# gcorso/disco-diffdock

Measured on AMD Instinct MI355X. Metric: complexes/sec, 20-step 40-sample inference, higher is better.
Workload: dtype f32

## Files before the change

disco_diffdock_amd/csrc/ddk_capi.hip:

```cpp
#include <math.h>
#include <algorithm>
#include <cmath>
#include <string.h>

#include "model.h"
#include "k_conv_common.h"

using namespace ddk;

namespace ddk {


int fail(ddk_ctx* ctx, int code, const std::string& msg) {
  if (ctx) ctx->err = msg;
  return code;
}

int hip_fail(ddk_ctx* ctx, hipError_t e, const char* what) {
  return fail(ctx, DDK_ERR_HIP, std::string(what) + ": " + hipGetErrorString(e));
}

hipError_t ctx_malloc(ddk_ctx* ctx, void** p, size_t bytes) {
  *p = nullptr;
  if (ctx->alloc_limit > 0 && ctx->dev_bytes + (int64_t)bytes > ctx->alloc_limit) { ctx->alloc_refusals++; return hipErrorOutOfMemory; }
// ... 501 lines not shown
      float* b2 = b2x_all.data() + g * b2sz;
      for (int t = 0; t < L.n_tiles; ++t) {
        for (int s_ = 0; s_ < 36; ++s_)
          for (int lane = 0; lane < 64; ++lane) {
            const int row = rmx[(size_t)t * 32 + (lane & 31)], hh = lane >> 5;
            w2[(((size_t)t * 9 + s_ / 4) * 64 + lane) * 4 + (s_ & 3)] = row >= 0 ? W2->data[(size_t)row * ne + hid_of(s_, hh)] * rsx[(size_t)t * 32 + (lane & 31)] : 0.f;
          }
        for (int hh = 0; hh < 2; ++hh)
          for (int r = 0; r < 16; ++r) {
            const int row = rmx[(size_t)t * 32 + d_row(r, hh)];
            b2[((size_t)t * 2 + hh) * 16 + r] = row >= 0 ? B2->data[row] * rsx[(size_t)t * 32 + d_row(r, hh)] : 0.f;
          }
      }
    }
    if ((rc = pack_x3(ctx, L, NG, w1all, w2x_all, b2x_all))) return rc;
  }
  if (!ctx->host_only) {
    std::vector<float> w2rec((size_t)NG * L.n_tiles * W2_TILE_FLOATS);
    for (int g = 0; g < NG; ++g)
      for (int t = 0; t < L.n_tiles; ++t) {
        float* rec = w2rec.data() + ((size_t)g * L.n_tiles + t) * W2_TILE_FLOATS;
        memcpy(rec, w2all.data() + g * w2sz + (size_t)t * 2304, 2304 * sizeof(float));
        memcpy(rec + 2304, b2all.data() + g * b2sz + (size_t)t * 32, 32 * sizeof(float));
        memcpy(rec + 2336, &tiles[t], 2 * sizeof(int32_t));
      }
    float* d1 = dev_upload(ctx, w1all);
    float* db1 = dev_upload(ctx, b1all);
    float* d2 = dev_upload(ctx, w2rec);
    if (mode == 0) { L.wn = dev_upload(ctx, L.h_wn); L.bnp = dev_upload(ctx, L.h_bnp); if (!L.wn || !L.bnp) return fail(ctx, DDK_ERR_NOMEM, "device allocation failed while packing conv weights"); }
    L.bn_mean = dev_upload(ctx, L.h_bn_mean);
    L.bn_scale = dev_upload(ctx, L.h_bn_scale);
    L.bn_bias = dev_upload(ctx, L.h_bn_bias);
    if (!d1 || !db1 || !d2 || !L.bn_mean || !L.bn_scale || !L.bn_bias)
      return fail(ctx, DDK_ERR_NOMEM, "device allocation failed while packing conv weights");
    L.w1p[0] = d1; L.b1p[0] = db1; L.w2r[0] = d2;
    for (int g = 1; g < 4; ++g) {
      L.w1p[g] = d1 + g * w1sz;
      L.b1p[g] = db1 + g * b1sz;
      L.w2r[g] = d2 + (size_t)g * L.n_tiles * W2_TILE_FLOATS;
    }
  }
  return DDK_OK;
}

int build_head_layer(ddk_ctx* ctx, int mode, ConvLayerDev& L) {
  std::vector<int> rowmap;
  std::vector<float> rowscale;
  std::vector<TileDesc> tiles;
  int rc = build_layout(ctx, mode, 3, L, rowmap, rowscale, tiles);
  if (rc) return rc;
  L.n_groups = 1;
  const std::string pre = mode == 2 ? "tor_bond_conv.fc" : "final_conv.fc";
  const int kin = mode == 2 ? NE : 2 * NS;
  const HostTensor* W1 = find_w(ctx, pre + ".0.weight", {kin, kin});
  const HostTensor* B1 = find_w(ctx, pre + ".0.bias", {kin});
  const HostTensor* W2 = find_w(ctx, pre + ".4.weight", {L.W, kin});
  const HostTensor* B2 = find_w(ctx, pre + ".4.bias", {L.W});
  if (!W1 || !B1 || !W2 || !B2) return DDK_ERR_INVALID;
  L.has_weights = true;
  std::vector<float> w1(3 * 9 * 64 * 4, 0.f), b1(3 * 2 * 16, 0.f), w2((size_t)L.n_tiles * 9 * 64 * 4, 0.f), b2((size_t)L.n_tiles * 32, 0.f);
  for (int T = 0; T < 3; ++T) {
    for (int s = 0; s < 36; ++s)
      for (int lane = 0; lane < 64; ++lane) {
        const int hidden = 32 * T + (lane & 31), k = kin_of(s, lane >> 5);
        w1[(((size_t)T * 9 + s / 4) * 64 + lane) * 4 + (s & 3)] = (hidden < kin && k < kin) ? W1->data[(size_t)hidden * kin + k] : 0.f;
      }
    for (int hh = 0; hh < 2; ++hh)
      for (int r = 0; r < 16; ++r) {
        const int hidden = 32 * T + d_row(r, hh);
        b1[(T * 2 + hh) * 16 + r] = hidden < kin ? B1->data[hidden] : 0.f;
      }
  }
  for (int t = 0; t < L.n_tiles; ++t) {
    for (int s = 0; s < 36; ++s)
      for (int lane = 0; lane < 64; ++lane) {
        const int row = rowmap[(size_t)t * 32 + (lane & 31)], hd = hid_of(s, lane >> 5);
        w2[(((size_t)t * 9 + s / 4) * 64 + lane) * 4 + (s & 3)] =
            (row >= 0 && hd < kin) ? W2->data[(size_t)row * kin + hd] * rowscale[(size_t)t * 32 + (lane & 31)] : 0.f;
      }
    for (int hh = 0; hh < 2; ++hh)
      for (int r = 0; r < 16; ++r) {
        const int row = rowmap[(size_t)t * 32 + d_row(r, hh)];
        b2[((size_t)t * 2 + hh) * 16 + r] = row >= 0 ? B2->data[row] * rowscale[(size_t)t * 32 + d_row(r, hh)] : 0.f;
      }
  }
  L.h_w1p.assign(1, w1); L.h_b1p.assign(1, b1); L.h_w2p.assign(1, w2); L.h_b2p.assign(1, b2);
  L.h_bn_mean.assign(XW, 0.f); L.h_bn_scale.assign(XW, 1.f); L.h_bn_bias.assign(XW, 0.f);
  if (ctx->cfg.conv_kernel != 1 && (rc = pack_x3(ctx, L, 1, w1, w2, b2))) return rc;
  if (ctx->host_only) return DDK_OK;
  std::vector<float> w2rec((size_t)L.n_tiles * W2_TILE_FLOATS);
  for (int t = 0; t < L.n_tiles; ++t) {
    float* rec = w2rec.data() + (size_t)t * W2_TILE_FLOATS;
    memcpy(rec, w2.data() + (size_t)t * 2304, 2304 * sizeof(float));
    memcpy(rec + 2304, b2.data() + (size_t)t * 32, 32 * sizeof(float));
    memcpy(rec + 2336, &tiles[t], 2 * sizeof(int32_t));
  }
  L.w1p[0] = dev_upload(ctx, w1); L.b1p[0] = dev_upload(ctx, b1); L.w2r[0] = dev_upload(ctx, w2rec);
  if (!L.w1p[0] || !L.b1p[0] || !L.w2r[0]) return fail(ctx, DDK_ERR_NOMEM, "device allocation failed while packing the head weights");
  return DDK_OK;
}

int model_finalize(ddk_ctx* ctx);
int conf_model_finalize(ddk_ctx* ctx);
void conf_model_destroy(ddk_ctx* ctx);
void model_destroy(ddk_ctx* ctx);

}

extern "C" {

const char* ddk_version(void) { return "ddk 0.8 (gfx950)"; }

int ddk_create(const ddk_config* cfg, ddk_ctx** out) {
  if (!cfg || !out) return DDK_ERR_INVALID;
  ddk_ctx* ctx = new ddk_ctx();
  ctx->cfg = *cfg;
  *out = ctx;
  if (cfg->ns != NS || cfg->nv != NV)
    return fail(ctx, DDK_ERR_INVALID, "only ns=24, nv=6 (DiffDock-S / DisCo-DiffDock-S) is compiled in");
  if (cfg->num_conv_layers < 4 || cfg->num_conv_layers > 16)
    return fail(ctx, DDK_ERR_INVALID, "num_conv_layers must be in [4,16] (the heads and the confidence predictor assume the full 0e+1o+1e+0o irreps)");
  if (cfg->confidence_mode && cfg->all_atoms)
    return fail(ctx, DDK_ERR_INVALID, "confidence_mode selects the COARSE-GRAINED score model's confidence head; the all-atom confidence model is all_atoms = 1 alone (include/ddk.h)");
  if (cfg->sigma_embed_dim != 32 || cfg->distance_embed_dim != 32 || cfg->cross_distance_embed_dim != 32)
    return fail(ctx, DDK_ERR_INVALID, "only 32-wide sigma / distance embeddings are compiled in");
  if (cfg->deterministic && cfg->all_atoms)
    return fail(ctx, DDK_ERR_INVALID, "deterministic scatter is implemented for the score model (not with all_atoms)");
#ifdef DDK_VARIANT_CONV_Y
  if (cfg->conv_kernel < 0 || cfg->conv_kernel > 3) return fail(ctx, DDK_ERR_INVALID, "conv_kernel must be 0, 1, 2 (variant build) or 3");
#else
  if (cfg->conv_kernel < 0 || cfg->conv_kernel > 3 || cfg->conv_kernel == 2)
    return fail(ctx, DDK_ERR_INVALID, "conv_kernel must be 0 (two f16 limbs per operand, three products), 1 (fp32 MFMA) or 3 (three f16 limbs, six products); 2 (round 5's software-pipelined form) lives under tools/variants/ and is not part of libddk.so");
#endif
  if (cfg->device < 0) {
    ctx->host_only = true;
    return DDK_OK;
  }
  hipError_t e = hipSetDevice(cfg->device);
  if (e != hipSuccess) return hip_fail(ctx, e, "hipSetDevice");
  hipDeviceProp_t prop;
  e = hipGetDeviceProperties(&prop, cfg->device);
  if (e != hipSuccess) return hip_fail(ctx, e, "hipGetDeviceProperties");
  ctx->n_cu = prop.multiProcessorCount;
  e = hipStreamCreateWithFlags(&ctx->up_stream, hipStreamNonBlocking);
  if (e != hipSuccess) return hip_fail(ctx, e, "hipStreamCreate (upload stream)");
  e = hipStreamCreateWithFlags(&ctx->head_stream, hipStreamNonBlocking);
  if (e == hipSuccess) e = hipEventCreateWithFlags(&ctx->ev_fork, hipEventDisableTiming);
  if (e == hipSuccess) e = hipEventCreateWithFlags(&ctx->ev_join, hipEventDisableTiming);
  if (e != hipSuccess) return hip_fail(ctx, e, "hipStreamCreate (head stream)");
  e = conv_prepare_device();
  if (e != hipSuccess) return hip_fail(ctx, e, "hipFuncSetAttribute(dynamic LDS)");
  e = graph_prepare_device(&ctx->max_rec);
  if (e != hipSuccess) return hip_fail(ctx, e, "hipFuncSetAttribute(dynamic LDS, graph kernels)");
  ctx->ws.tile_info = (int32_t*)dev_alloc(ctx, 64 * sizeof(int32_t));
  if (!ctx->ws.tile_info) return fail(ctx, DDK_ERR_NOMEM, "hipMalloc failed");
  return DDK_OK;
}

void ddk_destroy(ddk_ctx* ctx) {
  if (!ctx) return;
  if (!ctx->host_only) {
    hipSetDevice(ctx->cfg.device);
    model_destroy(ctx);
    conf_model_destroy(ctx);
    for (auto& r : ctx->prof_recs) { hipEventDestroy(r.a); hipEventDestroy(r.b); }
    if (ctx->prof_edges) hipHostFree(ctx->prof_edges);
    for (auto& c : ctx->chunk_pool) { if (c.free_after) hipEventDestroy(c.free_after); ctx_free(ctx, c.p); }
    for (auto& b : ctx->stage_pool) { if (b.done) hipEventDestroy(b.done); hipHostFree(b.p); }
    if (ctx->up_stream) hipStreamDestroy(ctx->up_stream);
    if (ctx->head_stream) hipStreamDestroy(ctx->head_stream);
    if (ctx->ev_fork) hipEventDestroy(ctx->ev_fork);
    if (ctx->ev_join) hipEventDestroy(ctx->ev_join);
    for (void* p : ctx->dev_allocs) ctx_free(ctx, p);
    if (ctx->ws.xpad) ctx_free(ctx, ctx->ws.xpad);
    if (ctx->ws.sum) ctx_free(ctx, ctx->ws.sum);
    if (ctx->ws.deg) ctx_free(ctx, ctx->ws.deg);
  }
  delete ctx;
}

const char* ddk_last_error(ddk_ctx* ctx) { return ctx ? ctx->err.c_str() : "null context"; }

int ddk_load_weights(ddk_ctx* ctx, const char* name, const float* host_ptr, const int64_t* shape, int32_t ndim) {
  if (!ctx || !name || (!host_ptr && ndim > 0 && shape[0] != 0)) return fail(ctx, DDK_ERR_INVALID, "ddk_load_weights: null argument");
  const std::string n(name);
  if (n.find(".tp.") != std::string::npos) return DDK_OK;
  HostTensor t;
  int64_t numel = 1;
  for (int i = 0; i < ndim; ++i) {
    t.shape.push_back(shape[i]);
    numel *= shape[i];
  }
  t.data.assign(host_ptr, host_ptr + numel);
  ctx->weights[n] = std::move(t);
  ctx->finalized = false;
  return DDK_OK;
}

int ddk_finalize_weights(ddk_ctx* ctx) {
  if (!ctx) return DDK_ERR_INVALID;
  if (!ctx->host_only) hipSetDevice(ctx->cfg.device);
  ctx->conv.clear();
  ctx->conv.resize(ctx->cfg.num_conv_layers);
  for (int l = 0; l < ctx->cfg.num_conv_layers; ++l) {
    int rc = build_conv_layer(ctx, ctx->cfg.all_atoms ? 1 : 0, l, ctx->conv[l]);
    if (rc != DDK_OK) return rc;
  }
  ctx->head[0] = ConvLayerDev(); ctx->head[1] = ConvLayerDev();
  if (!ctx->cfg.all_atoms && ctx->weights.find("final_conv.fc.0.weight") != ctx->weights.end()) {
    int rch = build_head_layer(ctx, 3, ctx->head[1]);
    if (rch == DDK_OK && !ctx->cfg.no_torsion) rch = build_head_layer(ctx, 2, ctx->head[0]);
    if (rch != DDK_OK) return rch;
  }
  int rc = ctx->cfg.all_atoms ? conf_model_finalize(ctx) : model_finalize(ctx);
  if (rc != DDK_OK) return rc;
  ctx->finalized = true;
  return DDK_OK;
}

int ddk_set_score_norm_tables(ddk_ctx* ctx, const double* so3, int32_t n_so3, const double* torus, int32_t n_torus) {
  if (!ctx || !so3 || !torus) return fail(ctx, DDK_ERR_INVALID, "null table");
  if (n_so3 != 1000 || n_torus != 5001) return fail(ctx, DDK_ERR_INVALID, "expected 1000 so3 and 5001 torus entries");
  ctx->so3_table.assign(so3, so3 + n_so3);
  ctx->torus_table.assign(torus, torus + n_torus);
  return DDK_OK;
}

static int check_launchable(ddk_ctx* ctx, int32_t layer) {
  if (!ctx) return DDK_ERR_INVALID;
  if (ctx->host_only) return fail(ctx, DDK_ERR_STATE, "host-only context (device < 0) cannot launch kernels");
  if (!ctx->finalized) return fail(ctx, DDK_ERR_STATE, "weights not finalised");
  if (layer < 0 || layer >= (int)ctx->conv.size()) return fail(ctx, DDK_ERR_INVALID, "layer out of range");
  return DDK_OK;
}

int ddk_tp_forward(ddk_ctx* ctx, int32_t layer, const float* x_dst, const float* sh, const float* w, int64_t E,
                   float* out, void* stream) {
  int rc = check_launchable(ctx, layer);
  if (rc) return rc;
  hipError_t e = launch_tp_forward(ctx->conv[layer], x_dst, sh, w, E, out, (hipStream_t)stream);
  if (e == hipErrorInvalidValue)
    return fail(ctx, DDK_ERR_INVALID, "ddk_tp_forward: the layer's irreps are not one of the four conv-layer shapes of this model family (24x0e [+ 6x1o [+ 6x1e [+ 24x0o]]] -> the next entry)");
  if (e != hipSuccess) return hip_fail(ctx, e, "tp_forward launch");
  return DDK_OK;
}

int ddk_conv_forward(ddk_ctx* ctx, int32_t layer, const float* x, int64_t N, const int32_t* edge_src,
                     const int32_t* edge_dst, const int64_t* go, const float* edge_attr, const float* sh, float* out,
                     void* stream) {
  const bool aa = ctx && ctx->cfg.all_atoms;
  const int conv_k = aa ? layer % 9 : 0;
  if (aa) layer /= 9;
  int rc = check_launchable(ctx, layer);
  if (rc) return rc;
  if (!go || go[0] != 0 || go[1] < go[0] || go[2] < go[1] || go[3] < go[2] || go[4] < go[3])
    return fail(ctx, DDK_ERR_INVALID, "group_offsets must be a non-decreasing prefix starting at 0");
  if (go[4] >= (int64_t)1 << 31 || N * XW >= (int64_t)1 << 40) return fail(ctx, DDK_ERR_INVALID, "graph too large");
  hipStream_t s = (hipStream_t)stream;
  const ConvLayerDev& L = ctx->conv[layer];
  if (!L.has_weights) return fail(ctx, DDK_ERR_STATE, "conv layer has no weights loaded");
  Workspace& ws = ctx->ws;
  if ((rc = ensure(ctx, (void**)&ws.xpad, &ws.xpad_cap, (size_t)N * XW * 4))) return rc;
  if ((rc = ensure(ctx, (void**)&ws.sum, &ws.sum_cap, (size_t)N * XW * 4))) return rc;
  if ((rc = ensure(ctx, (void**)&ws.deg, &ws.deg_cap, (size_t)N * 4))) return rc;
  const int64_t E = go[4];
  CK(launch_pad_rows(x, N, L.din, ws.xpad, s), "pad_rows");
  CK(hipMemsetAsync(ws.sum, 0, (size_t)N * XW * 4, s), "memset sum");
  CK(hipMemsetAsync(ws.deg, 0, (size_t)N * 4, s), "memset deg");
  if (E > 0) {
    CK(launch_conv_setup(ws.tile_info, go, s), "conv_setup");
    CK(launch_count_deg(edge_src, E, ws.deg, s), "count_deg");
    ConvLaunch a;
    a.x = ws.xpad; a.src = edge_src; a.dst = edge_dst; a.edge_attr = edge_attr; a.sh = sh; a.sum = ws.sum;
    a.tile_info = ws.tile_info; a.counter = ws.tile_info + 10; a.gather = 0;
    if (aa) {
      CK(launch_conv_one_group(ws.tile_info + 32, 9, conv_k, E, s), "group table");
      a.mode = 1; a.n_groups = 9; a.n_active = 9; a.n_slots = 1; a.slots = 0; a.gbeg = ws.tile_info + 32; a.gend = ws.tile_info + 41;
    }
    CK(launch_conv_fused(L, a, ctx->n_cu, s), "conv_fused");
  }
  if (aa) {
    CK(launch_node_finalize(ws.sum, ws.deg, nullptr, L.bn_mean + conv_k * XW, L.bn_scale + conv_k * XW, L.bn_bias + conv_k * XW, N, L.dout, L.dout, out, s),
       "node_finalize");
    return DDK_OK;
  }
  if (E > 0)
    CK(launch_node_finalize(ws.sum, ws.deg, ws.xpad, L.bn_mean, L.bn_scale, L.bn_bias, N, L.dout, L.dout, out, s), "node_finalize");
  else
    CK(launch_node_finalize(ws.sum, ws.deg, ws.xpad, nullptr, nullptr, nullptr, N, 0, L.dout, out, s), "node_finalize");
  return DDK_OK;
}

int64_t ddk_debug_export(ddk_ctx* ctx, const char* what, void* buf, int64_t cap_words) {
  if (!ctx || !what) return DDK_ERR_INVALID;
  int l = 0, g = 0;
  char item[32] = {0};
  const void* src = nullptr;
  int64_t n = 0;
  if (sscanf(what, "conv.%d.%31[a-z0-9_].%d", &l, item, &g) >= 2) {
    const bool head = (l == 100 || l == 101) && ctx->head[l - 100].n_tiles > 0;
    if (!head && (l < 0 || l >= (int)ctx->conv.size())) return fail(ctx, DDK_ERR_INVALID, "bad export index");
    ConvLayerDev& L = head ? ctx->head[l - 100] : ctx->conv[l];
    if (g < 0 || g >= L.n_groups) return fail(ctx, DDK_ERR_INVALID, "bad export index");
    const std::string it(item);
    if (it == "w1p") { src = L.h_w1p[g].data(); n = L.h_w1p[g].size(); }
    else if (it == "b1p") { src = L.h_b1p[g].data(); n = L.h_b1p[g].size(); }
// ... 31 lines not shown
```

disco_diffdock_amd/csrc/k_graph.hip:

```cpp
#include <stdlib.h>
#include "model.h"
#include "k_node.h"

namespace ddk {


__device__ __forceinline__ bool cross_within(const float* lp, const float* rp, float c) {
#pragma clang fp contract(off)
  const float dx = rp[0] / c - lp[0] / c, dy = rp[1] / c - lp[1] / c, dz = rp[2] / c - lp[2] / c;
  return dx * dx + dy * dy + dz * dz < 1.0f;
}

__device__ __forceinline__ bool cross_within4(const float4 a, float rx, float ry, float rz) {
#pragma clang fp contract(off)
  const float dx = rx - a.x, dy = ry - a.y, dz = rz - a.z;
  return dx * dx + dy * dy + dz * dz < 1.0f;
}

__device__ __forceinline__ float dist2(const float* a, const float* b) {
#pragma clang fp contract(off)
  const float dx = a[0] - b[0], dy = a[1] - b[1], dz = a[2] - b[2];
  return dx * dx + dy * dy + dz * dz;
}

constexpr int GT = 1024;

__device__ void build_lig_adj(const float* lp, int n_lig, float r2, unsigned (*adj)[MAX_LIG / 32]) {
  const int lane = threadIdx.x & 63, wave = threadIdx.x >> 6, nw = blockDim.x >> 6;
  for (int i = wave; i < n_lig; i += nw) {
    int cnt = 0;
    if (lane < MAX_LIG / 32) adj[i][lane] = 0u;
    for (int j0 = 0; j0 < n_lig; j0 += 64) {
      const int j = j0 + lane;
      const bool in = j < n_lig && dist2(lp + 3 * i, lp + 3 * j) < r2;
      const unsigned long long m = __ballot(in);
      const bool keep = in && cnt + __popcll(m & ((1ull << lane) - 1ull)) < LIG_CAP && j != i;
      const unsigned long long kept = __ballot(keep);
      if (lane == 0) { adj[i][j0 >> 5] = (unsigned)kept; adj[i][(j0 >> 5) + 1] = (unsigned)(kept >> 32); }
      cnt += __popcll(m);
    }
  }
}

__device__ void block_exclusive_scan(int* a, int n, int* tmp) {
  const int tid = threadIdx.x, lane = tid & 63, wave = tid >> 6;
  const int nt = blockDim.x;
  const int per = (n + nt - 1) / nt;
  const int beg = min(tid * per, n), end = min(beg + per, n);
  int s = 0;
  for (int k = beg; k < end; ++k) s += a[k];
  int v = s;
#pragma unroll
  for (int d = 1; d < 64; d *= 2) {
    const int t = __shfl_up(v, d, 64);
    if (lane >= d) v += t;
  }
  if (lane == 63) tmp[wave] = v;
  __syncthreads();
  int base = v - s;
  for (int w = 0; w < wave; ++w) base += tmp[w];
  for (int k = beg; k < end; ++k) { const int t = a[k]; a[k] = base; base += t; }
  __syncthreads();
}

__device__ void propagate_levels(uint8_t* lvl, const GraphArgs& G) {
  constexpr int UC = 8;
  if (G.E_rr <= GT * UC) {
    unsigned e[UC];
#pragma unroll
    for (int u = 0; u < UC; ++u) {
      const int k = threadIdx.x + GT * u;
      e[u] = k < G.E_rr ? (unsigned)G.rr_src[k] | ((unsigned)G.rr_dst[k] << 16) : 0xffffffffu;
    }
    for (int pass = 0; pass < 2; ++pass) {
#pragma unroll
      for (int u = 0; u < UC; ++u) {
        const int r = (int)(e[u] & 0xffffu), d = (int)(e[u] >> 16);
        if (e[u] != 0xffffffffu && lvl[r] == pass && lvl[d] == 3) lvl[d] = (uint8_t)(pass + 1);
      }
      __syncthreads();
    }
    return;
  }
  constexpr int U = 8;
  for (int pass = 0; pass < 2; ++pass) {
    for (int k0 = threadIdx.x; k0 < G.E_rr; k0 += GT * U) {
      int r[U], d[U];
#pragma unroll
      for (int u = 0; u < U; ++u) {
        const int k = k0 + GT * u;
        r[u] = k < G.E_rr ? G.rr_src[k] : -1;
        d[u] = k < G.E_rr ? G.rr_dst[k] : 0;
      }
#pragma unroll
      for (int u = 0; u < U; ++u)
        if (r[u] >= 0 && lvl[r[u]] == pass && lvl[d[u]] == 3) lvl[d[u]] = (uint8_t)(pass + 1);
    }
    __syncthreads();
  }
}

__device__ void level_scan(const uint8_t* lvl, const int32_t* outdeg, int n, int* pre, int (*tmp)[4], int* tot) {
  const int tid = threadIdx.x, lane = tid & 63, wave = tid >> 6;
  const int nt = blockDim.x, nw = nt >> 6;
  const int per = (n + nt - 1) / nt;
  const int beg = min(tid * per, n), end = min(beg + per, n);
  int s0 = 0, s1 = 0, s2 = 0, s3 = 0;
  for (int k = beg; k < end; ++k) {
    const int l = lvl[k], od = outdeg[k];
    s0 += l == 0 ? od : 0; s1 += l == 1 ? od : 0; s2 += l == 2 ? od : 0; s3 += l == 3 ? od : 0;
  }
  int v0 = s0, v1 = s1, v2 = s2, v3 = s3;
#pragma unroll
  for (int d = 1; d < 64; d *= 2) {
    const int t0 = __shfl_up(v0, d, 64), t1 = __shfl_up(v1, d, 64), t2 = __shfl_up(v2, d, 64), t3 = __shfl_up(v3, d, 64);
    if (lane >= d) { v0 += t0; v1 += t1; v2 += t2; v3 += t3; }
  }
  if (lane == 63) { tmp[wave][0] = v0; tmp[wave][1] = v1; tmp[wave][2] = v2; tmp[wave][3] = v3; }
  __syncthreads();
  if (pre != nullptr) {
    int b0 = v0 - s0, b1 = v1 - s1, b2 = v2 - s2, b3 = v3 - s3;
    for (int w = 0; w < wave; ++w) { b0 += tmp[w][0]; b1 += tmp[w][1]; b2 += tmp[w][2]; b3 += tmp[w][3]; }
    for (int k = beg; k < end; ++k) {
      const int l = lvl[k], od = outdeg[k];
      pre[k] = l == 0 ? b0 : (l == 1 ? b1 : (l == 2 ? b2 : b3));
      b0 += l == 0 ? od : 0; b1 += l == 1 ? od : 0; b2 += l == 2 ? od : 0; b3 += l == 3 ? od : 0;
    }
  }
  if (tid < 4) { int t_ = 0; for (int w = 0; w < nw; ++w) t_ += tmp[w][tid]; tot[tid] = t_; }
  __syncthreads();
}

__global__ __launch_bounds__(GT) void graph_count_kernel(GraphArgs G) {
  extern __shared__ float smem[];
  float* lp = smem;
  float* rp = lp + MAX_LIG * 3;
  uint8_t* lvl = reinterpret_cast<uint8_t*>(rp + 3 * G.n_rec + G.n_rec);
  __shared__ unsigned adj[MAX_LIG][MAX_LIG / 32];
  __shared__ float4 lps[MAX_LIG];
  __shared__ int s_cnt[2], lvl_tmp[GT / 64][4], lvl_tot[4];
  const int b = blockIdx.x, tid = threadIdx.x;
  for (int i = tid; i < G.n_lig * 3; i += GT) {
    const float v = G.lig_pos[(size_t)b * G.n_lig * 3 + i];
    lp[i] = v;
    reinterpret_cast<float*>(lps)[4 * (i / 3) + i % 3] = v / G.cross_cutoff;
  }
  for (int i = tid; i < G.n_rec * 3; i += GT) rp[i] = G.rec_pos[i] / G.cross_cutoff;
  if (tid < 2) s_cnt[tid] = 0;
  __syncthreads();
  build_lig_adj(lp, G.n_lig, G.lig_r2, adj);
  __syncthreads();
  int c_ll = 0, c_lr = 0;
  for (int i = tid; i < G.n_lig; i += GT)
    for (int w = 0; w < MAX_LIG / 32; ++w) c_ll += __popc(adj[i][w]);
  for (int j = tid; j < G.n_rec; j += GT) {
    const float rx = rp[3 * j], ry = rp[3 * j + 1], rz = rp[3 * j + 2];
    int cnt = 0;
#pragma unroll 4
    for (int i = 0; i < G.n_lig; ++i) cnt += cross_within4(lps[i], rx, ry, rz) ? 1 : 0;
    c_lr += cnt;
    lvl[j] = (G.prune && cnt == 0) ? 3 : 0;
  }
#pragma unroll
  for (int d = 32; d > 0; d >>= 1) { c_ll += __shfl_down(c_ll, d, 64); c_lr += __shfl_down(c_lr, d, 64); }
  if ((tid & 63) == 0) { atomicAdd(&s_cnt[0], c_ll); atomicAdd(&s_cnt[1], c_lr); }
  __syncthreads();
  if (G.prune) propagate_levels(lvl, G);
  level_scan(lvl, G.rr_outdeg, G.n_rec, nullptr, lvl_tmp, lvl_tot);
  if (tid < 2) G.counts[CNT_STRIDE * b + tid] = s_cnt[tid];
  if (tid < 3) G.counts[CNT_STRIDE * b + 2 + tid] = lvl_tot[tid];
  for (int j = tid; j < G.n_rec; j += GT) G.levels[(size_t)b * G.n_rec + j] = lvl[j];
}

__device__ __forceinline__ void sample_prefix(const GraphArgs& G, int b, int* ex, int* tot) {
  const int lane = threadIdx.x & 63;
#pragma unroll
  for (int k = 0; k < 5; ++k) { tot[k] = 0; ex[k] = 0; }
  for (int b0 = 0; b0 < G.B; b0 += 64) {
    const int bb = b0 + lane;
    int v[5], inc[5];
#pragma unroll
    for (int k = 0; k < 5; ++k) v[k] = bb < G.B ? G.counts[CNT_STRIDE * bb + k] + (k == 0 ? G.M : 0) : 0;
#pragma unroll
    for (int k = 0; k < 5; ++k) {
      int x = v[k];
#pragma unroll
      for (int d = 1; d < 64; d *= 2) { const int t = __shfl_up(x, d, 64); if (lane >= d) x += t; }
      inc[k] = x;
    }
    if (b >= b0 && b < b0 + 64) {
#pragma unroll
      for (int k = 0; k < 5; ++k) ex[k] = tot[k] + __shfl(inc[k] - v[k], b - b0, 64);
    }
#pragma unroll
    for (int k = 0; k < 5; ++k) tot[k] += __shfl(inc[k], 63, 64);
  }
  ex[5] = b * G.E_rr - (ex[2] + ex[3] + ex[4]);
}

__device__ void write_group_tables(const GraphArgs& G, const int* tot) {
  const int ll = tot[0], lr = tot[1], ra = tot[2], rb = tot[3], rc = tot[4];
  int go[5];
  go[0] = 0; go[1] = ll; go[2] = ll + lr; go[3] = go[2] + G.B * G.E_rr; go[4] = go[3] + lr;
  const int seg[4] = {go[2], go[2] + ra, go[2] + ra + rb, go[2] + ra + rb + rc};
  const int n_shared = G.shared_rr ? G.E_rr : 0;
  int bs = 0;
  G.info[I_FB] = 0;
  for (int g = 0; g < 5; ++g) {
    bs += (g == 3 && G.cross_mirror) ? 0 : ((g < 4 ? go[g + 1] - go[g] : n_shared) + 255) / 256;
    G.info[I_FB + 1 + g] = bs;
  }
  for (int g = 0; g < 5; ++g) G.info[I_GO + g] = go[g];
  for (int k = 0; k < 8; ++k) G.info[I_CNT + k] = 0;
  for (int l = 0; l < 4; ++l) G.info[I_SEG + l] = seg[l];
  G.info[I_E] = go[4];
  G.info[I_OVF] = ((int64_t)go[4] + n_shared > G.edge_cap) ? 1 : 0;
  G.info[I_SHARED] = G.shared_rr ? go[4] : -1;
  G.info[I_HEAD] = 0; G.info[I_HEAD + 1] = G.B * G.n_lig; G.info[I_HEAD + 2] = G.B * G.n_lig; G.info[I_HEAD + 3] = G.B * G.n_lig;
  G.info[I_HEAD + 4] = 0; G.info[I_HEAD + 5] = 0;
  G.info[I_EXEC] = go[4];
  G.info[I_EXEC + 1] = go[2];
  G.info[I_EXEC + 7] = lr;
  for (int k = 0; k < N_TAB; ++k) {
    int32_t* tb = G.info + I_TAB + 8 * k;
    int tot = 0;
    for (int g = 0; g < 4; ++g) { tb[g] = go[g]; tb[4 + g] = go[g + 1]; }
    if (k == TAB_A) tb[4 + 2] = seg[1];
    if (k == TAB_B) tb[4 + 2] = seg[2];
    if (k == TAB_C) tb[4 + 2] = seg[3];
    if (k == TAB_SHARED) { tb[2] = go[4]; tb[4 + 2] = go[4] + n_shared; }
    for (int g = 0; g < 4; ++g) tot += tb[4 + g] - tb[g];
    if (k == TAB_SHARED && G.patch_off >= 0 && G.shared_rr) tot += G.info[I_PATCH];
    G.info[I_EXEC + 2 + k] = tot;
  }
  if (G.patch_off >= 0 && G.shared_rr) {
    const int np = G.info[I_PATCH];
    const int32_t* ts = G.info + I_TAB + 8 * TAB_SHARED;
    for (int g = 0; g < 4; ++g) { G.info[I_TABX + g] = ts[g]; G.info[I_TABX + 5 + g] = ts[4 + g]; }
    G.info[I_TABX + 4] = (int)G.patch_off; G.info[I_TABX + 9] = (int)G.patch_off + np;
    G.info[I_FBX] = bs + (np + 255) / 256;
  } else {
    G.info[I_FBX] = bs;
  }
}

__device__ __forceinline__ bool latent_nonzero(const float* lat, int64_t row, int ld) {
  bool nz = false;
  for (int j = 0; j < ld; ++j) nz |= lat[row * ld + j] != 0.0f;
  return nz;
}

__global__ __launch_bounds__(256) void disco_patch_count_kernel(PatchArgs A) {
  extern __shared__ unsigned char mk[];
  __shared__ int red[256];
  const int b = blockIdx.x, tid = threadIdx.x;
  for (int j = tid; j < A.n_rec; j += 256)
    mk[j] = b > 0 && (latent_nonzero(A.rec_latent, (int64_t)b * A.n_rec + j, A.latent_dim) || latent_nonzero(A.rec_latent, j, A.latent_dim));
  __syncthreads();
  int cnt = 0;
  for (int i = tid; i < A.n_rec; i += 256) {
    bool a = mk[i];
    const int k0 = A.rr_start[i], k1 = k0 + A.rr_outdeg[i];
    for (int k = k0; k < k1 && !a; ++k) a = mk[A.rr_dst[k]];
    A.rr_mask[(size_t)b * A.n_rec + i] = a;
    if (a) cnt += k1 - k0;
  }
  red[tid] = cnt;
  __syncthreads();
  for (int d = 128; d > 0; d >>= 1) { if (tid < d) red[tid] += red[tid + d]; __syncthreads(); }
  if (tid == 0) A.patch_cnt[b] = red[0];
}

__global__ void disco_patch_scan_kernel(PatchArgs A) {
  if (threadIdx.x != 0 || blockIdx.x != 0) return;
  int tot = 0;
  for (int b = 0; b < A.B; ++b) { const int c = A.patch_cnt[b]; A.patch_cnt[b] = tot; tot += c; }
  A.patch_cnt[A.B] = tot;
  A.info[I_PATCH] = tot;
}

__global__ __launch_bounds__(256) void disco_patch_fill_kernel(PatchArgs A) {
  extern __shared__ int pre_[];
  __shared__ int scan_tmp[16];
  const int b = blockIdx.x, tid = threadIdx.x;
  for (int i = tid; i < A.n_rec; i += 256) pre_[i] = A.rr_mask[(size_t)b * A.n_rec + i] ? A.rr_outdeg[i] : 0;
  __syncthreads();
  block_exclusive_scan(pre_, A.n_rec, scan_tmp);
  const int rec0 = A.B * A.n_lig + b * A.n_rec;
  const int64_t base = A.patch_off + A.patch_cnt[b];
  for (int i = tid; i < A.n_rec; i += 256) {
    if (!A.rr_mask[(size_t)b * A.n_rec + i]) continue;
    const int k0 = A.rr_start[i], n = A.rr_outdeg[i];
    for (int q = 0; q < n; ++q) {
      const int64_t pos = base + pre_[i] + q;
      A.e_src[pos] = rec0 + i; A.e_dst[pos] = rec0 + A.rr_dst[k0 + q]; A.e_aux[pos] = k0 + q;
    }
  }
}

hipError_t launch_disco_patch(const PatchArgs& a, hipStream_t s) {
  hipLaunchKernelGGL(disco_patch_count_kernel, dim3(a.B), dim3(256), (size_t)a.n_rec, s, a);
  hipLaunchKernelGGL(disco_patch_scan_kernel, dim3(1), dim3(64), 0, s, a);
  hipLaunchKernelGGL(disco_patch_fill_kernel, dim3(a.B), dim3(256), (size_t)a.n_rec * sizeof(int), s, a);
  return hipGetLastError();
}

constexpr int FILL_SLICES = 4;

__global__ __launch_bounds__(GT) void graph_fill_kernel(GraphArgs G) {
  extern __shared__ float smem[];
  float* lp = smem;
  float* rp = lp + MAX_LIG * 3;
  int* c_rl = reinterpret_cast<int*>(rp + 3 * G.n_rec);
  uint8_t* lvl = reinterpret_cast<uint8_t*>(c_rl + G.n_rec);
  unsigned long long* cmask = reinterpret_cast<unsigned long long*>(lvl + ((G.n_rec + 15) & ~15));
  const int LW = (G.n_lig + 63) >> 6;
  __shared__ unsigned adj[MAX_LIG][MAX_LIG / 32];
  __shared__ int bdeg[MAX_LIG], odeg[MAX_LIG], c_lr[MAX_LIG], ll_pre[MAX_LIG], lr_pre[MAX_LIG], scan_tmp[GT / 64], lvl_tmp[GT / 64][4], lvl_tot[4];
  constexpr int BOND_LDS = 1024;
  __shared__ short2 bond_sd[BOND_LDS];
  const int b = blockIdx.x, slice = blockIdx.y, tid = threadIdx.x, lane = tid & 63, wave = tid >> 6;
  const int n_lig = G.n_lig, n_rec = G.n_rec;
  int ex[6], tot[5];
  sample_prefix(G, b, ex, tot);
// ... 207 lines not shown
    float gs[DE];
#pragma unroll
    for (int k = 0; k < DE; ++k) {
      const float t = d - M.offset[k];
      gs[k] = expf(M.coeff * (t * t));
    }
#pragma unroll
    for (int o = 0; o < NS; ++o) h[o] = sigb[o];
#pragma unroll
    for (int k = 0; k < DE; ++k) {
#pragma unroll
      for (int o = 0; o < NS; ++o) h[o] = fmaf(M.w1d_t[k * NS + o], gs[k], h[o]);
    }
    if (g == 0 && aux >= 0) {
      const float4 ba = *reinterpret_cast<const float4*>(A.bond_attr + 4 * (size_t)aux);
#pragma unroll
      for (int o = 0; o < NS; ++o)
        h[o] += M.w1b[o * 4] * ba.x + M.w1b[o * 4 + 1] * ba.y + M.w1b[o * 4 + 2] * ba.z + M.w1b[o * 4 + 3] * ba.w;
    }
  }
  if (A.latent_dim > 0 && (g == 0 || g == 2)) {
    const float* lat = g == 0 ? A.lig_latent : A.rec_latent;
    const int off = g == 0 ? 0 : A.n_lig_total;
    const int ld = A.latent_dim;
    for (int j = 0; j < ld; ++j) {
      const float ls = lat[(size_t)(sn - off) * ld + j], ldv = lat[(size_t)(dn - off) * ld + j];
#pragma unroll
      for (int o = 0; o < NS; ++o) h[o] += M.w1l[o * 2 * ld + j] * ls + M.w1l[o * 2 * ld + ld + j] * ldv;
    }
  }
#pragma unroll
  for (int o = 0; o < NS; ++o) h[o] = fmaxf(h[o], 0.0f);
  float* out = A.e_emb + (size_t)e * NS;
  float* out2 = (g == 1 && A.cross_mirror) ? A.e_emb + (size_t)aux * NS : nullptr;
  const float uncw = (A.latent_dim > 0 && M.unc != nullptr) ? A.unconditional : 0.0f;
  float y[NS];
#pragma unroll
  for (int o = 0; o < NS; ++o) y[o] = M.b2[o];
#pragma unroll
  for (int k = 0; k < NS; ++k) {
#pragma unroll
    for (int o = 0; o < NS; ++o) y[o] = fmaf(M.w2_t[k * NS + o], h[k], y[o]);
  }
  if (uncw != 0.0f) {
#pragma unroll
    for (int o = 0; o < NS; ++o) y[o] += uncw * M.unc[o];
  }
#pragma unroll
  for (int o4 = 0; o4 < NS / 4; ++o4) {
    const float4 rv = make_float4(y[4 * o4], y[4 * o4 + 1], y[4 * o4 + 2], y[4 * o4 + 3]);
    *reinterpret_cast<float4*>(out + 4 * o4) = rv;
    if (out2) *reinterpret_cast<float4*>(out2 + 4 * o4) = rv;
  }
  *reinterpret_cast<float4*>(A.e_sh + 4 * (size_t)e) = shv;
  if (out2) *reinterpret_cast<float4*>(A.e_sh + 4 * (size_t)aux) = shv;
}

__global__ __launch_bounds__(256) void edge_features_kernel(EdgeFeatArgs A) { edge_features_body(A, (int)blockIdx.x, (int)threadIdx.x); }

__global__ __launch_bounds__(PRE_W) void edge_features_node_kernel(EdgeFeatArgs A, NodePreArgs P, NodeEmbedArgs E, int node_blocks) {
  if ((int)blockIdx.x < node_blocks) { node_finalize_pre_body<2>(P, E, (int)blockIdx.x, node_blocks); return; }
  if (threadIdx.x < 256) edge_features_body(A, (int)blockIdx.x - node_blocks, (int)threadIdx.x);
}

__global__ void node_embed_kernel(NodeEmbedArgs A) {
  const int64_t i = (int64_t)blockIdx.x * blockDim.x + threadIdx.x;
  const int64_t n_l = (int64_t)A.B * A.n_lig, n = n_l + (int64_t)A.B * A.n_rec;
  if (i >= n * XW) return;
  const int64_t node = i / XW;
  const int c = (int)(i % XW);
  float v = 0.0f;
  if (c < NS) {
    const bool lig = node < n_l;
    if (lig) v = A.lig_static[(node % A.n_lig) * NS + c] + A.sp.lig_node_sig[c];
    else v = A.rec_static[((node - n_l) % A.n_rec) * NS + c] + A.sp.rec_node_sig[c];
    if (A.latent_dim > 0) {
      const float* lat = lig ? A.lig_latent + node * A.latent_dim : A.rec_latent + (node - n_l) * A.latent_dim;
      const float* w = (lig ? A.lig_w_lat : A.rec_w_lat) + c * A.latent_dim;
      for (int j = 0; j < A.latent_dim; ++j) v += w[j] * lat[j];
      const float* u = lig ? A.lig_unc : A.rec_unc;
      if (u != nullptr) v += A.unconditional * u[c];
    }
  }
  A.x[i] = v;
}

constexpr int RNS_SLICES = 10;
__global__ __launch_bounds__(RNS_SLICES * NS) void rec_node_static_kernel(RecStaticArgs A) {
  __shared__ double part[RNS_SLICES][NS];
  const int o = threadIdx.x % NS, sl = threadIdx.x / NS, j = blockIdx.x;
  const float* xr = A.rec_x + (size_t)j * A.feat_dim;
  double a = 0.0;
  if (sl == 0) {
    const float* emb = A.rec_table + (size_t)(int)xr[0] * NS;
    a = A.b[o];
    for (int k = 0; k < NS; ++k) a += (double)A.w_emb[o * NS + k] * emb[k];
  }
  const int per = (A.lm + RNS_SLICES - 1) / RNS_SLICES, k0 = sl * per, k1 = min(A.lm, k0 + per);
  for (int k = k0; k < k1; ++k) a += (double)A.w_lm_t[(size_t)k * NS + o] * (double)xr[1 + k];
  part[sl][o] = a;
  __syncthreads();
  if (sl == 0) {
#pragma unroll
    for (int q = 1; q < RNS_SLICES; ++q) a += part[q][o];
    A.out[(size_t)j * NS + o] = (float)a;
  }
}

__global__ __launch_bounds__(256) void rec_edge_static_kernel(const int32_t* rr_src, const int32_t* rr_dst, const float* rec_pos, int E, EdgeMlpDev m,
                                                              float* pre1) {
  const int gid = blockIdx.x * blockDim.x + threadIdx.x;
  const int k = gid / (NS / 4), o4 = gid % (NS / 4);
  if (k >= E) return;
  const int a = rr_src[k], b = rr_dst[k];
  const float vx = rec_pos[3 * b] - rec_pos[3 * a], vy = rec_pos[3 * b + 1] - rec_pos[3 * a + 1], vz = rec_pos[3 * b + 2] - rec_pos[3 * a + 2];
  const float dist = sqrtf(vx * vx + vy * vy + vz * vz);
  float gs[DE];
#pragma unroll
  for (int q = 0; q < DE; ++q) { const float t = dist - m.offset[q]; gs[q] = expf(m.coeff * (t * t)); }
  float r[4];
#pragma unroll
  for (int i = 0; i < 4; ++i) {
    const int o = 4 * o4 + i;
    float a2 = 0.0f;
#pragma unroll
    for (int q = 0; q < DE; ++q) a2 += m.w1d[o * DE + q] * gs[q];
    r[i] = a2;
  }
  *reinterpret_cast<float4*>(pre1 + (size_t)k * NS + 4 * o4) = make_float4(r[0], r[1], r[2], r[3]);
}

__global__ void zero_fill_kernel(float4* p, int64_t n4, float* tail, int n_tail) {
  const int64_t i = (int64_t)blockIdx.x * blockDim.x + threadIdx.x;
  if (i < n4) p[i] = make_float4(0.f, 0.f, 0.f, 0.f);
  if (i < n_tail) tail[i] = 0.0f;
}
hipError_t launch_zero_fill(void* p, size_t bytes, hipStream_t s) {
  if (bytes == 0) return hipSuccess;
  if ((reinterpret_cast<uintptr_t>(p) & 15) || (bytes & 3)) return hipMemsetAsync(p, 0, bytes, s);
  const int64_t n4 = (int64_t)(bytes / 16);
  const int n_tail = (int)((bytes % 16) / 4);
  hipLaunchKernelGGL(zero_fill_kernel, dim3((unsigned)((n4 + 255) / 256 + 1)), dim3(256), 0, s, reinterpret_cast<float4*>(p), n4,
                     reinterpret_cast<float*>(p) + 4 * n4, n_tail);
  return hipGetLastError();
}

hipError_t launch_complex_static(const RecStaticArgs& R, const int32_t* rr_src, const int32_t* rr_dst, const float* rec_pos, int E, const EdgeMlpDev& m,
                                 float* pre1, hipStream_t s) {
  if (R.n_rec > 0) hipLaunchKernelGGL(rec_node_static_kernel, dim3(R.n_rec), dim3(RNS_SLICES * NS), 0, s, R);
  if (E > 0) hipLaunchKernelGGL(rec_edge_static_kernel, dim3((E * (NS / 4) + 255) / 256), dim3(256), 0, s, rr_src, rr_dst, rec_pos, E, m, pre1);
  return hipGetLastError();
}

static inline size_t graph_lds_bytes(int n_rec) {
  return (size_t)(MAX_LIG * 3 + n_rec * 3) * 4 + (size_t)n_rec * 4 + (((size_t)n_rec + 15) & ~(size_t)15);
}

static size_t g_graph_dyn[64] = {};
static inline size_t graph_lds_bytes_mirror(int n_rec, int n_lig) { return graph_lds_bytes(n_rec) + (size_t)n_rec * ((n_lig + 63) / 64) * 8; }
int graph_cross_mirror_fits(int n_lig, int n_rec) {
  static const bool off = getenv("DDK_NO_CROSS_MIRROR") != nullptr;
  if (off) return 0;
  int dev = 0;
  if (hipGetDevice(&dev) != hipSuccess || dev < 0 || dev >= 64) return 0;
  return g_graph_dyn[dev] > 0 && graph_lds_bytes_mirror(n_rec, n_lig) <= g_graph_dyn[dev];
}

hipError_t graph_prepare_device(int* max_rec) {
  hipFuncAttributes a1, a2;
  hipError_t e = hipFuncGetAttributes(&a1, reinterpret_cast<const void*>(&graph_count_kernel));
  if (e == hipSuccess) e = hipFuncGetAttributes(&a2, reinterpret_cast<const void*>(&graph_fill_kernel));
  if (e != hipSuccess) return e;
  const size_t st = a1.sharedSizeBytes > a2.sharedSizeBytes ? a1.sharedSizeBytes : a2.sharedSizeBytes;
  const size_t dyn = 160 * 1024 - st;
  e = hipFuncSetAttribute(reinterpret_cast<const void*>(&graph_count_kernel), hipFuncAttributeMaxDynamicSharedMemorySize, (int)(160 * 1024 - a1.sharedSizeBytes));
  if (e == hipSuccess) e = hipFuncSetAttribute(reinterpret_cast<const void*>(&graph_fill_kernel), hipFuncAttributeMaxDynamicSharedMemorySize, (int)(160 * 1024 - a2.sharedSizeBytes));
  if (e != hipSuccess) return e;
  int n = MAX_REC;
  while (n > 1 && graph_lds_bytes(n) > dyn) --n;
  *max_rec = n;
  int dev = 0;
  if (hipGetDevice(&dev) == hipSuccess && dev >= 0 && dev < 64) g_graph_dyn[dev] = 160 * 1024 - a2.sharedSizeBytes;
  return hipSuccess;
}

hipError_t launch_graph(const GraphArgs& G, int64_t edge_cap, hipStream_t s) {
  const size_t lds = graph_lds_bytes(G.n_rec);
  GraphArgs Gc = G;
  Gc.edge_cap = edge_cap;
  hipLaunchKernelGGL(graph_count_kernel, dim3(G.B), dim3(GT), lds, s, Gc);
  hipLaunchKernelGGL(graph_fill_kernel, dim3(G.B, FILL_SLICES), dim3(GT), G.cross_mirror ? graph_lds_bytes_mirror(G.n_rec, G.n_lig) : lds, s, Gc);
  return hipGetLastError();
}

__global__ __launch_bounds__(GT) void det_ranges_kernel(GraphArgs G, int kind, int len_uniform, int32_t* out, int nr) {
  extern __shared__ int nb_s[];
  __shared__ int scan_tmp[GT / 64];
  const int tid = threadIdx.x, lane = tid & 63, wave = tid >> 6;
  int32_t* beg_o = out + nr + 1;
  int32_t* end_o = beg_o + nr;
  int32_t* grp_o = end_o + nr;
  auto put = [&](int r, int beg, int end, int g) {
    if (lane == 0) { beg_o[r] = beg; end_o[r] = end; grp_o[r] = g; nb_s[r] = (end - beg + 255) / 256; }
  };
  if (kind == 6) {
    for (int r = tid; r < nr; r += GT) { beg_o[r] = r * len_uniform; end_o[r] = (r + 1) * len_uniform; grp_o[r] = 0; nb_s[r] = (len_uniform + 255) / 256; }
  } else {
    const int nseg = kind == 5 ? 0 : kind;
    for (int b = wave; b < G.B; b += GT / 64) {
      int ex[6], tot[5];
      sample_prefix(G, b, ex, tot);
      const int g1 = tot[0], g2 = tot[0] + tot[1], g3 = g2 + G.B * G.E_rr;
      const int cnt0 = G.counts[CNT_STRIDE * b] + G.M, cnt1 = G.counts[CNT_STRIDE * b + 1];
      const int ca = G.counts[CNT_STRIDE * b + 2], cb = G.counts[CNT_STRIDE * b + 3], cc = G.counts[CNT_STRIDE * b + 4];
      put(b, ex[0], ex[0] + cnt0, 0);
      put(G.B + b, g1 + ex[1], g1 + ex[1] + cnt1, 1);
      if (kind == 0) continue;
      int r = 2 * G.B;
      const int segbeg[4] = {g2 + ex[2], g2 + tot[2] + ex[3], g2 + tot[2] + tot[3] + ex[4], g2 + tot[2] + tot[3] + tot[4] + ex[5]};
      const int seglen[4] = {ca, cb, cc, G.E_rr - ca - cb - cc};
      for (int l = 0; l < nseg; ++l) { put(r + b, segbeg[l], segbeg[l] + seglen[l], 2); r += G.B; }
      if (kind == 5) {
        const int g4 = g3 + tot[1];
        if (b == 0) put(r, g4, g4 + G.E_rr, 2);
        r += 1;
      }
      put(r + b, g3 + ex[1], g3 + ex[1] + cnt1, 3);
    }
  }
  __syncthreads();
  block_exclusive_scan(nb_s, nr, scan_tmp);
  for (int r = tid; r < nr; r += GT) out[r] = nb_s[r];
  if (tid == 0) out[nr] = nb_s[nr - 1] + (end_o[nr - 1] - beg_o[nr - 1] + 255) / 256;
}

int det_ranges_count(int kind, int B) { return kind == 0 ? 2 * B : (kind == 5 ? 3 * B + 1 : (kind == 6 ? B : (3 + kind) * B)); }

hipError_t launch_det_ranges(const GraphArgs& G, int kind, int len_uniform, int32_t* out, hipStream_t s) {
  const int nr = det_ranges_count(kind, G.B);
  hipLaunchKernelGGL(det_ranges_kernel, dim3(1), dim3(GT), (size_t)(nr + 1) * sizeof(int), s, G, kind, len_uniform, out, nr);
  return hipGetLastError();
}

hipError_t launch_edge_features(const EdgeFeatArgs& A, int64_t edge_cap, hipStream_t s) {
  const unsigned blocks = (unsigned)((edge_cap + 255) / 256 + 5);
  hipLaunchKernelGGL(edge_features_kernel, dim3(blocks), dim3(256), 0, s, A);
  return hipGetLastError();
}

hipError_t launch_edge_features_node(const EdgeFeatArgs& A, int64_t edge_cap, const NodePreArgs& P, const NodeEmbedArgs& E, hipStream_t s) {
  const unsigned blocks = (unsigned)((edge_cap + 255) / 256 + 5);
  const int nb = node_pre_tiles(P);
  hipLaunchKernelGGL(edge_features_node_kernel, dim3(blocks + nb), dim3(PRE_W), 0, s, A, P, E, nb);
  return hipGetLastError();
}

hipError_t launch_node_embed(const NodeEmbedArgs& a, hipStream_t s) {
  const int64_t tot = (int64_t)a.B * (a.n_lig + a.n_rec) * XW;
  hipLaunchKernelGGL(node_embed_kernel, dim3((unsigned)((tot + 255) / 256)), dim3(256), 0, s, a);
  return hipGetLastError();
}

}
```

disco_diffdock_amd/csrc/k_heads.hip:

```cpp
#include "model.h"

namespace ddk {

constexpr int EPB = 32;
__device__ __forceinline__ void edge_embed8(const EdgeMlpDev& m, const float* b1, float d, float (*act)[DE + 1], int el, int p, float* e3) {
#pragma unroll
  for (int q = 0; q < 4; ++q) {
    const float t = d - m.offset[4 * p + q];
    act[el][4 * p + q] = expf(m.coeff * (t * t));
  }
  __syncthreads();
  float h3[3];
#pragma unroll
  for (int q = 0; q < 3; ++q) {
    const int o = 3 * p + q;
    float a = b1[o];
#pragma unroll
    for (int k = 0; k < DE; ++k) a += m.w1d[o * DE + k] * act[el][k];
    h3[q] = fmaxf(a, 0.0f);
  }
  __syncthreads();
#pragma unroll
  for (int q = 0; q < 3; ++q) act[el][3 * p + q] = h3[q];
  __syncthreads();
#pragma unroll
  for (int q = 0; q < 3; ++q) {
    const int o = 3 * p + q;
    float a = m.b2[o];
#pragma unroll
    for (int k = 0; k < NS; ++k) a += m.w2[o * NS + k] * act[el][k];
    e3[q] = a;
  }
  __syncthreads();
}

__global__ __launch_bounds__(256) void heads_pre_kernel(HeadArgs A, int n_tor_blocks) {
  __shared__ float lp[MAX_LIG * 3];
  __shared__ float act[EPB][DE + 1];
  __shared__ int nb[BOND_CAP];
  __shared__ int s_cnt, s_base;
  __shared__ float ctr[3];
  const int tid = threadIdx.x, n = A.n_lig;
  const int el = tid >> 3, p = tid & 7;
  const bool tor = (int)blockIdx.x < n_tor_blocks;
  const int b = tor ? blockIdx.x / A.R : blockIdx.x - n_tor_blocks;
  for (int i = tid; i < n * 3; i += 256) lp[i] = A.lig_pos[(size_t)b * n * 3 + i];
  __syncthreads();
  if (!tor) {
    if (tid < 3) {
      float s = 0.0f;
      for (int i = 0; i < n; ++i) s += lp[3 * i + tid];
      ctr[tid] = s / (float)n;
    }
    __syncthreads();
    for (int a0 = 0; a0 < n; a0 += EPB) {
      const int i = a0 + el;
      const bool live = i < n;
      const int ii = live ? i : n - 1;
      const float vx = lp[3 * ii] - ctr[0], vy = lp[3 * ii + 1] - ctr[1], vz = lp[3 * ii + 2] - ctr[2];
      const float d = sqrtf(vx * vx + vy * vy + vz * vz);
      float e3[3];
      edge_embed8(A.md.center_edge, A.sp.center_edge_sigb, d, act, el, p, e3);
      if (live) {
        const int e = b * n + i;
        float* at = A.h_attr + (size_t)e * NE;
        const float* xr = A.x + ((size_t)b * n + i) * XW;
#pragma unroll
        for (int q = 0; q < 3; ++q) {
          at[3 * p + q] = e3[q];
          at[NS + 3 * p + q] = xr[3 * p + q];
          at[2 * NS + 3 * p + q] = 0.0f;
        }
        if (p == 0) {
          const float inv = 1.7320508075688772f / fmaxf(d, 1e-12f);
          *reinterpret_cast<float4*>(A.h_sh + (size_t)e * 4) = make_float4(1.0f, vx * inv, vy * inv, vz * inv);
          A.h_src[e] = b;
          A.h_dst[e] = b * n + i;
        }
      }
    }
    return;
  }
  const int r = blockIdx.x - b * A.R;
  const int u = A.rot_u[r], v = A.rot_v[r];
  const float cx = (lp[3 * u] + lp[3 * v]) * 0.5f, cy = (lp[3 * u + 1] + lp[3 * v + 1]) * 0.5f, cz = (lp[3 * u + 2] + lp[3 * v + 2]) * 0.5f;
  if (tid < 64) {
    int cnt = 0;
    for (int k0 = 0; k0 < n; k0 += 64) {
      const int k = k0 + tid;
      bool in = false;
      if (k < n) {
        const float dx = lp[3 * k] - cx, dy = lp[3 * k + 1] - cy, dz = lp[3 * k + 2] - cz;
        in = dx * dx + dy * dy + dz * dz < A.lig_r2;
      }
      const unsigned long long mask = __ballot(in);
      const int rank = cnt + __popcll(mask & ((1ull << tid) - 1ull));
      if (in && rank < BOND_CAP) nb[rank] = k;
      cnt += __popcll(mask);
    }
    if (tid == 0) {
      s_cnt = cnt < BOND_CAP ? cnt : BOND_CAP;
      if (A.deterministic) {
        s_base = A.B * n + (int)blockIdx.x * BOND_CAP;
        if (blockIdx.x == 0) A.h_info[3] = A.B * n + n_tor_blocks * BOND_CAP;
      } else {
        s_base = atomicAdd(A.h_info + 3, s_cnt);
      }
      A.h_deg[blockIdx.x] = s_cnt;
    }
  }
  __syncthreads();
  const int ne = s_cnt;
  const bool live = el < ne;
  const int k = ne > 0 ? nb[live ? el : 0] : u;
  const float vx = lp[3 * k] - cx, vy = lp[3 * k + 1] - cy, vz = lp[3 * k + 2] - cz;
  const float d = sqrtf(vx * vx + vy * vy + vz * vz);
  float e3[3];
  edge_embed8(A.md.final_edge, A.md.final_edge_b1, d, act, el, p, e3);
  const int e = s_base + el;
  float* at = A.h_attr + (size_t)e * NE;
  if (!live) {
    if (A.deterministic) {
#pragma unroll
      for (int q = 0; q < 9; ++q) at[9 * p + q] = 0.0f;
      if (p == 0) {
        *reinterpret_cast<float4*>(A.h_sh + (size_t)e * 4) = make_float4(0.f, 0.f, 0.f, 0.f);
        A.h_src[e] = A.B + n_tor_blocks;
        A.h_dst[e] = b * n + u;
      }
    }
    return;
  }
  const float* xk = A.x + ((size_t)b * n + k) * XW;
  const float* xu = A.x + ((size_t)b * n + u) * XW;
  const float* xv = A.x + ((size_t)b * n + v) * XW;
#pragma unroll
  for (int q = 0; q < 3; ++q) {
    const int o = 3 * p + q;
    at[o] = e3[q];
    at[NS + o] = xk[o];
    at[2 * NS + o] = xu[o] + xv[o];
  }
  if (p != 0) return;
  const float inv = 1.7320508075688772f / fmaxf(d, 1e-12f);
  const float s1[3] = {vx * inv, vy * inv, vz * inv};
  float bx = lp[3 * v] - lp[3 * u], by = lp[3 * v + 1] - lp[3 * u + 1], bz = lp[3 * v + 2] - lp[3 * u + 2];
  const float bn = fmaxf(sqrtf(bx * bx + by * by + bz * bz), 1e-12f);
  bx /= bn; by /= bn; bz /= bn;
  const float s3 = 1.7320508075688772f, s5 = 2.2360679774997897f;
  const float y0 = s5 * s3 * bx * bz, y1 = s5 * s3 * bx * by, y2 = s5 * (by * by - 0.5f * (bx * bx + bz * bz)),
              y3 = s5 * s3 * by * bz, y4 = s5 * (s3 * 0.5f) * (bz * bz - bx * bx);
  const float ca = 0.31622776601683794f, cb = 0.18257418583505536f;
  const float T0 = s3 * (-cb * s1[0] * y2 - ca * s1[0] * y4 + ca * s1[1] * y1 + ca * s1[2] * y0);
  const float T1 = s3 * (ca * s1[0] * y1 + 2.0f * cb * s1[1] * y2 + ca * s1[2] * y3);
  const float T2 = s3 * (ca * s1[0] * y0 + ca * s1[1] * y3 - cb * s1[2] * y2 + ca * s1[2] * y4);
  *reinterpret_cast<float4*>(A.h_sh + (size_t)e * 4) = make_float4(1.0f, T0, T1, T2);
  A.h_src[e] = A.B + (int)blockIdx.x;
  A.h_dst[e] = b * n + k;
}

__global__ __launch_bounds__(64) void heads_post_kernel(HeadArgs A, int n_tor_blocks) {
  __shared__ float v48[2 * NS], hid[NS], g12[12];
  const int tid = threadIdx.x;
  if (A.prof_out != nullptr && blockIdx.x == gridDim.x - 1 && tid < PROF_INTS) A.prof_out[tid] = A.exec_info[tid];
  if ((int)blockIdx.x < n_tor_blocks) {
    float* row = A.h_sum + (size_t)(A.B + blockIdx.x) * XW;
    const int ne = A.h_deg[blockIdx.x];
    if (tid < 2 * NS) {
      const float s = row[tid] / (float)(ne > 1 ? ne : 1);
      row[tid] = 0.0f;
      v48[tid] = (s - A.md.tb_bn_mean[tid]) * A.md.tb_bn_scale[tid] + A.md.tb_bn_bias[tid];
    }
    __syncthreads();
    if (tid < NS) {
      float a = 0.0f;
      for (int j = 0; j < 2 * NS; ++j) a += A.md.tf_w0[tid * 2 * NS + j] * v48[j];
      hid[tid] = A.md.tf_w3[tid] * tanhf(a);
    }
    __syncthreads();
    if (tid == 0) {
      float o = 0.0f;
      for (int j = 0; j < NS; ++j) o += hid[j];
      if (A.scale_by_sigma) o *= A.sp.torus_norm_sqrt;
      A.tor_out[blockIdx.x] = o;
    }
    return;
  }
  const int b = blockIdx.x - n_tor_blocks;
  float* row = A.h_sum + (size_t)b * XW;
  if (tid < 12) {
    g12[tid] = (row[tid] / (float)A.n_lig) * A.md.fc_bn_scale[tid / 3];
    row[tid] = 0.0f;
  }
  __syncthreads();
  if (tid < 2) {
    const int o = 3 * tid;
    const float px = g12[o] + g12[6 + o], py = g12[o + 1] + g12[7 + o], pz = g12[o + 2] + g12[8 + o];
    const float nrm = sqrtf(px * px + py * py + pz * pz);
    const float* w0n = tid == 0 ? A.md.tr_w0n : A.md.rot_w0n;
    const float* w3 = tid == 0 ? A.md.tr_w3 : A.md.rot_w3;
    const float* sb = tid == 0 ? A.sp.tr_sigb : A.sp.rot_sigb;
    float s = tid == 0 ? A.md.tr_b3 : A.md.rot_b3;
    for (int k = 0; k < NS; ++k) s += w3[k] * fmaxf(w0n[k] * nrm + sb[k], 0.0f);
    float f = s / nrm;
    if (A.scale_by_sigma) f = tid == 0 ? f / A.sp.tr_sigma : f * A.sp.so3_norm;
    float* out = (tid == 0 ? A.tr_out : A.rot_out) + 3 * (size_t)b;
    out[0] = px * f; out[1] = py * f; out[2] = pz * f;
  }
}

hipError_t launch_heads_pre(const HeadArgs& A, bool torsion, hipStream_t s) {
  const int n_tor = (torsion && A.R > 0) ? A.B * A.R : 0;
  hipLaunchKernelGGL(heads_pre_kernel, dim3(n_tor + A.B), dim3(256), 0, s, A, n_tor);
  return hipGetLastError();
}

hipError_t launch_heads_post(const HeadArgs& A, bool torsion, hipStream_t s) {
  const int n_tor = (torsion && A.R > 0) ? A.B * A.R : 0;
  hipLaunchKernelGGL(heads_post_kernel, dim3(n_tor + A.B), dim3(64), 0, s, A, n_tor);
  return hipGetLastError();
}

}
```

disco_diffdock_amd/csrc/k_se3.hip:

```cpp
#include "model.h"

namespace ddk {


__device__ void axis_angle_to_matrix_dev(float ax, float ay, float az, float* R) {
  const float ang = sqrtf(ax * ax + ay * ay + az * az);
  const float half = 0.5f * ang;
  const float s = fabsf(ang) < 1e-6f ? 0.5f - ang * ang / 48.0f : sinf(half) / ang;
  const float qr = cosf(half), qi = ax * s, qj = ay * s, qk = az * s;
  const float two_s = 2.0f / (qr * qr + qi * qi + qj * qj + qk * qk);
  R[0] = 1 - two_s * (qj * qj + qk * qk); R[1] = two_s * (qi * qj - qk * qr); R[2] = two_s * (qi * qk + qj * qr);
  R[3] = two_s * (qi * qj + qk * qr); R[4] = 1 - two_s * (qi * qi + qk * qk); R[5] = two_s * (qj * qk - qi * qr);
  R[6] = two_s * (qi * qk - qj * qr); R[7] = two_s * (qj * qk + qi * qr); R[8] = 1 - two_s * (qi * qi + qj * qj);
}

__device__ void horn_rotation(const double* S, float* R) {
  double N[4][4] = {
      {S[0] + S[4] + S[8], S[5] - S[7], S[6] - S[2], S[1] - S[3]},
      {S[5] - S[7], S[0] - S[4] - S[8], S[1] + S[3], S[6] + S[2]},
      {S[6] - S[2], S[1] + S[3], -S[0] + S[4] - S[8], S[5] + S[7]},
      {S[1] - S[3], S[6] + S[2], S[5] + S[7], -S[0] - S[4] + S[8]}};
  double V[4][4] = {{1, 0, 0, 0}, {0, 1, 0, 0}, {0, 0, 1, 0}, {0, 0, 0, 1}};
  for (int sweep = 0; sweep < 30; ++sweep) {
    double off = 0, dg = 0;
#pragma unroll
    for (int p = 0; p < 4; ++p) {
      dg += N[p][p] * N[p][p];
#pragma unroll
      for (int q = p + 1; q < 4; ++q) off += N[p][q] * N[p][q];
    }
    if (off <= 1e-32 * dg || off < 1e-300) break;
#pragma unroll
    for (int p = 0; p < 4; ++p)
#pragma unroll
      for (int q = p + 1; q < 4; ++q) {
        const double x = N[p][q];
        if (fabs(x) <= 8.7e-19 * (fabs(N[p][p]) + fabs(N[q][q]))) continue;
        const double d = 0.5 * (N[q][q] - N[p][p]);
        const double r = d + (d >= 0 ? 1.0 : -1.0) * sqrt(d * d + x * x);
        const double inv = rsqrt(r * r + x * x);
        const double c = fabs(r) * inv, s = (r >= 0 ? x : -x) * inv;
        const double app = N[p][p], aqq = N[q][q], cc = c * c, ss = s * s, cs2 = 2.0 * c * s * x;
        N[p][p] = cc * app - cs2 + ss * aqq;
        N[q][q] = ss * app + cs2 + cc * aqq;
        N[p][q] = 0.0; N[q][p] = 0.0;
#pragma unroll
        for (int k = 0; k < 4; ++k) {
          if (k == p || k == q) continue;
          const double a = N[k][p], b = N[k][q];
          const double np_ = c * a - s * b, nq_ = s * a + c * b;
          N[k][p] = np_; N[p][k] = np_; N[k][q] = nq_; N[q][k] = nq_;
        }
#pragma unroll
        for (int k = 0; k < 4; ++k) {
          const double a = V[k][p], b = V[k][q];
          V[k][p] = c * a - s * b; V[k][q] = s * a + c * b;
        }
      }
  }
  double top = N[0][0], w = V[0][0], x = V[1][0], y = V[2][0], z = V[3][0];
#pragma unroll
  for (int k = 1; k < 4; ++k)
    if (N[k][k] > top) { top = N[k][k]; w = V[0][k]; x = V[1][k]; y = V[2][k]; z = V[3][k]; }
  const double nn = w * w + x * x + y * y + z * z, s2 = 2.0 / nn;
  R[0] = (float)(1 - s2 * (y * y + z * z)); R[1] = (float)(s2 * (x * y - z * w)); R[2] = (float)(s2 * (x * z + y * w));
  R[3] = (float)(s2 * (x * y + z * w)); R[4] = (float)(1 - s2 * (x * x + z * z)); R[5] = (float)(s2 * (y * z - x * w));
  R[6] = (float)(s2 * (x * z - y * w)); R[7] = (float)(s2 * (y * z + x * w)); R[8] = (float)(1 - s2 * (x * x + y * y));
}

__device__ void kabsch_block(const float* a, const float* bpts, int n, float* cA, float* cB, double* S, float* Rk, float* tk) {
  const int tid = threadIdx.x;
  if (tid < 3) {
    float sa = 0.0f, sb = 0.0f;
    for (int i = 0; i < n; ++i) { sa += a[3 * i + tid]; sb += bpts[3 * i + tid]; }
    cA[tid] = sa / (float)n; cB[tid] = sb / (float)n;
  }
  __syncthreads();
  if (tid < 9) {
    const int r = tid / 3, c = tid % 3;
    double s = 0.0;
    for (int i = 0; i < n; ++i) s += (double)(a[3 * i + r] - cA[r]) * (double)(bpts[3 * i + c] - cB[c]);
    S[tid] = s;
  }
  __syncthreads();
  if (tid == 0) {
    horn_rotation(S, Rk);
    for (int k = 0; k < 3; ++k) tk[k] = -(Rk[3 * k] * cA[0] + Rk[3 * k + 1] * cA[1] + Rk[3 * k + 2] * cA[2]) + cB[k];
  }
  __syncthreads();
}

__global__ __launch_bounds__(256) void debug_kabsch_kernel(const float* A, const float* Bp, int n, float* R_out, float* t_out) {
  __shared__ float a[MAX_LIG * 3], bb[MAX_LIG * 3], cA[3], cB[3], Rk[9], tk[3];
  __shared__ double S[9];
  const int b = blockIdx.x, tid = threadIdx.x;
  for (int i = tid; i < n * 3; i += 256) { a[i] = A[(size_t)b * n * 3 + i]; bb[i] = Bp[(size_t)b * n * 3 + i]; }
  __syncthreads();
  kabsch_block(a, bb, n, cA, cB, S, Rk, tk);
  if (tid < 9) R_out[9 * b + tid] = Rk[tid];
  if (tid < 3) t_out[3 * b + tid] = tk[tid];
}

__global__ void debug_axis_angle_kernel(const float* aa, int n, float* R_out) {
  const int i = blockIdx.x * blockDim.x + threadIdx.x;
  if (i < n) axis_angle_to_matrix_dev(aa[3 * i], aa[3 * i + 1], aa[3 * i + 2], R_out + 9 * i);
}

hipError_t launch_debug_kabsch(const float* A, const float* Bp, int B, int n, float* R_out, float* t_out, hipStream_t s) {
  hipLaunchKernelGGL(debug_kabsch_kernel, dim3(B), dim3(256), 0, s, A, Bp, n, R_out, t_out);
  return hipGetLastError();
}

hipError_t launch_debug_axis_angle(const float* aa, int n, float* R_out, hipStream_t s) {
  hipLaunchKernelGGL(debug_axis_angle_kernel, dim3((n + 63) / 64), dim3(64), 0, s, aa, n, R_out);
  return hipGetLastError();
}

template <bool POST, bool REC>
__global__ __launch_bounds__(256) void se3_update_kernel(Se3Args A, HeadArgs H) {
  __shared__ float rig[MAX_LIG * 3], flx_a[MAX_LIG * 3], flx2[MAX_LIG * 3];
  __shared__ float upd[6], ctr[3], Rm[9], cA[3], cB[3], Rk[9], tk[3], rot_th[64];
  __shared__ int2 rot_uv[64];
  __shared__ double S[9];
  float* flx = flx_a;
  const int b = blockIdx.x, tid = threadIdx.x, n = A.n_lig, R = A.R;
  if constexpr (POST) {
    __shared__ float v48[64][2 * NS], hid[64][NS], g12[12];
    if (H.prof_out != nullptr && b == (int)gridDim.x - 1 && tid < PROF_INTS) H.prof_out[tid] = H.exec_info[tid];
    if (A.tor != nullptr && R > 0) {
      for (int r0 = 0; r0 < R; r0 += 64) {
        const int chunk = min(64, R - r0);
        for (int i = tid; i < chunk * 2 * NS; i += 256) {
          const int rr = i / (2 * NS), c = i - rr * 2 * NS;
          const int bond = b * R + r0 + rr;
          float* row = H.h_sum + (size_t)(H.B + bond) * XW;
          const int ne = H.h_deg[bond];
          const float sv = row[c] / (float)(ne > 1 ? ne : 1);
          row[c] = 0.0f;
          v48[rr][c] = (sv - H.md.tb_bn_mean[c]) * H.md.tb_bn_scale[c] + H.md.tb_bn_bias[c];
        }
        __syncthreads();
        for (int i = tid; i < chunk * NS; i += 256) {
          const int rr = i / NS, k = i - rr * NS;
          float a = 0.0f;
          for (int j = 0; j < 2 * NS; ++j) a += H.md.tf_w0[k * 2 * NS + j] * v48[rr][j];
          hid[rr][k] = H.md.tf_w3[k] * tanhf(a);
        }
        __syncthreads();
        if (tid < chunk) {
          float o = 0.0f;
          for (int j = 0; j < NS; ++j) o += hid[tid][j];
          if (H.scale_by_sigma) o *= H.sp.torus_norm_sqrt;
          H.tor_out[(size_t)b * R + r0 + tid] = o;
        }
        __syncthreads();
      }
    }
    float* row = H.h_sum + (size_t)b * XW;
    if (tid < 12) {
      g12[tid] = (row[tid] / (float)H.n_lig) * H.md.fc_bn_scale[tid / 3];
      row[tid] = 0.0f;
    }
    __syncthreads();
    if (tid < 2) {
      const int o = 3 * tid;
      const float px = g12[o] + g12[6 + o], py = g12[o + 1] + g12[7 + o], pz = g12[o + 2] + g12[8 + o];
      const float nrm = sqrtf(px * px + py * py + pz * pz);
      const float* w0n = tid == 0 ? H.md.tr_w0n : H.md.rot_w0n;
      const float* w3 = tid == 0 ? H.md.tr_w3 : H.md.rot_w3;
      const float* sb = tid == 0 ? H.sp.tr_sigb : H.sp.rot_sigb;
      float sv = tid == 0 ? H.md.tr_b3 : H.md.rot_b3;
      for (int k = 0; k < NS; ++k) sv += w3[k] * fmaxf(w0n[k] * nrm + sb[k], 0.0f);
      float f = sv / nrm;
      if (H.scale_by_sigma) f = tid == 0 ? f / H.sp.tr_sigma : f * H.sp.so3_norm;
      float* out = (tid == 0 ? H.tr_out : H.rot_out) + 3 * (size_t)b;
      out[0] = px * f; out[1] = py * f; out[2] = pz * f;
    }
    __syncthreads();
  }
  const float* nz = A.noise ? A.noise + (size_t)b * (6 + R) : nullptr;
  for (int i = tid; i < n * 3; i += 256) rig[i] = A.pos[(size_t)b * n * 3 + i];
  if (tid < 6) {
    const int k = tid / 3;
    const float sc = (tid < 3 ? A.tr : A.rot)[3 * b + tid % 3];
    const float u = A.sc[k] * sc + (nz ? A.nc[k] * nz[tid] : 0.0f);
    upd[tid] = u;
    if constexpr (REC) {
      if (A.rec_scores != nullptr) A.rec_scores[(size_t)b * (6 + R) + tid] = sc;
      if (A.rec_perturb != nullptr) A.rec_perturb[(size_t)b * (6 + R) + tid] = u;
    }
  }
  if constexpr (REC) {
    if (A.rec_edges != nullptr && b == 0 && tid < 4) A.rec_edges[tid] = A.info[I_GO + 1 + tid] - A.info[I_GO + tid];
  }
  __syncthreads();
  if (tid < 3) {
    float s = 0.0f;
    for (int i = 0; i < n; ++i) s += rig[3 * i + tid];
    ctr[tid] = s / (float)n;
  }
  if (tid == 32) axis_angle_to_matrix_dev(upd[3], upd[4], upd[5], Rm);
  __syncthreads();
  if (tid < n) {
    const float x = rig[3 * tid] - ctr[0], y = rig[3 * tid + 1] - ctr[1], z = rig[3 * tid + 2] - ctr[2];
    const float rx = Rm[0] * x + Rm[1] * y + Rm[2] * z + upd[0] + ctr[0];
    const float ry = Rm[3] * x + Rm[4] * y + Rm[5] * z + upd[1] + ctr[1];
    const float rz = Rm[6] * x + Rm[7] * y + Rm[8] * z + upd[2] + ctr[2];
    rig[3 * tid] = rx; rig[3 * tid + 1] = ry; rig[3 * tid + 2] = rz;
    flx[3 * tid] = rx; flx[3 * tid + 1] = ry; flx[3 * tid + 2] = rz;
  }
  __syncthreads();
  if (A.tor == nullptr || R == 0) {
    for (int i = tid; i < n * 3; i += 256) {
      A.pos_out[(size_t)b * n * 3 + i] = rig[i];
      if constexpr (REC) if (A.rec_pos != nullptr) A.rec_pos[(size_t)b * n * 3 + i] = rig[i];
    }
    if constexpr (REC)
      for (int r = tid; r < R; r += 256) {
        if (A.rec_scores != nullptr) A.rec_scores[(size_t)b * (6 + R) + 6 + r] = 0.0f;
        if (A.rec_perturb != nullptr) A.rec_perturb[(size_t)b * (6 + R) + 6 + r] = 0.0f;
      }
    return;
  }
  float* cur = flx;
  float* nxt = flx2;
  for (int r0 = 0; r0 < R; r0 += 64) {
    const int chunk = min(64, R - r0);
    if (tid < chunk) {
      const int r = r0 + tid;
      rot_uv[tid] = make_int2(A.rot_u[r], A.rot_v[r]);
      const float ts = A.tor[(size_t)b * R + r];
      const float th = A.sc[2] * ts + (nz ? A.nc[2] * nz[6 + r] : 0.0f);
      rot_th[tid] = th;
      if constexpr (REC) {
        if (A.rec_scores != nullptr) A.rec_scores[(size_t)b * (6 + R) + 6 + r] = ts;
        if (A.rec_perturb != nullptr) A.rec_perturb[(size_t)b * (6 + R) + 6 + r] = th;
      }
    }
    unsigned long long mbits = 0ull;
    if (tid < n)
      for (int k = 0; k < chunk; ++k) mbits |= (unsigned long long)(A.mask_rotate[(size_t)(r0 + k) * n + tid] != 0) << k;
    __syncthreads();
    for (int k = 0; k < chunk; ++k) {
      if (tid < n) {
        const int2 uv = rot_uv[k];
        const float th = rot_th[k];
        const float px = cur[3 * uv.y], py = cur[3 * uv.y + 1], pz = cur[3 * uv.y + 2];
        float x = cur[3 * tid], y = cur[3 * tid + 1], z = cur[3 * tid + 2];
        if ((mbits >> k) & 1ull) {
          const float ax = cur[3 * uv.x] - px, ay = cur[3 * uv.x + 1] - py, az = cur[3 * uv.x + 2] - pz;
          const float nn = sqrtf(ax * ax + ay * ay + az * az);
          float Rl[9];
          axis_angle_to_matrix_dev(ax / nn * th, ay / nn * th, az / nn * th, Rl);
          x -= px; y -= py; z -= pz;
          const float nx = Rl[0] * x + Rl[1] * y + Rl[2] * z + px, ny = Rl[3] * x + Rl[4] * y + Rl[5] * z + py, nz_ = Rl[6] * x + Rl[7] * y + Rl[8] * z + pz;
          x = nx; y = ny; z = nz_;
        }
        nxt[3 * tid] = x; nxt[3 * tid + 1] = y; nxt[3 * tid + 2] = z;
      }
      __syncthreads();
      float* t_ = cur; cur = nxt; nxt = t_;
    }
  }
  flx = cur;
  kabsch_block(flx, rig, n, cA, cB, S, Rk, tk);
  if (tid < n) {
    const float x = flx[3 * tid], y = flx[3 * tid + 1], z = flx[3 * tid + 2];
    float* o = A.pos_out + ((size_t)b * n + tid) * 3;
    const float ox = Rk[0] * x + Rk[1] * y + Rk[2] * z + tk[0];
    const float oy = Rk[3] * x + Rk[4] * y + Rk[5] * z + tk[1];
    const float oz = Rk[6] * x + Rk[7] * y + Rk[8] * z + tk[2];
    o[0] = ox; o[1] = oy; o[2] = oz;
    if constexpr (REC)
      if (A.rec_pos != nullptr) {
        float* q = A.rec_pos + ((size_t)b * n + tid) * 3;
        q[0] = ox; q[1] = oy; q[2] = oz;
      }
  }
}

__global__ __launch_bounds__(256) void randomize_kernel(RandPosArgs A) {
  __shared__ float p[MAX_LIG * 3];
  __shared__ float Rt[9], piv[3], ctr[3];
  __shared__ int skip;
  const int b = blockIdx.x, tid = threadIdx.x, n = A.n_lig, R = A.R;
  for (int i = tid; i < n * 3; i += 256) p[i] = A.pos0[i];
  __syncthreads();
  if (A.tor != nullptr) {
    for (int r = 0; r < R; ++r) {
      if (tid == 0) {
        const float th = A.tor[(size_t)b * R + r];
        skip = th == 0.0f;
        const int u = A.rot_u[r], v = A.rot_v[r];
        const float ax = p[3 * u] - p[3 * v], ay = p[3 * u + 1] - p[3 * v + 1], az = p[3 * u + 2] - p[3 * v + 2];
        const float nn = sqrtf(ax * ax + ay * ay + az * az);
        axis_angle_to_matrix_dev(ax / nn * th, ay / nn * th, az / nn * th, Rt);
        piv[0] = p[3 * v]; piv[1] = p[3 * v + 1]; piv[2] = p[3 * v + 2];
      }
      __syncthreads();
      if (!skip && tid < n && A.mask_rotate[(size_t)r * n + tid]) {
        const float x = p[3 * tid] - piv[0], y = p[3 * tid + 1] - piv[1], z = p[3 * tid + 2] - piv[2];
        p[3 * tid] = Rt[0] * x + Rt[1] * y + Rt[2] * z + piv[0];
        p[3 * tid + 1] = Rt[3] * x + Rt[4] * y + Rt[5] * z + piv[1];
        p[3 * tid + 2] = Rt[6] * x + Rt[7] * y + Rt[8] * z + piv[2];
      }
      __syncthreads();
    }
  }
  if (tid < 3) {
    float s = 0.0f;
    for (int i = 0; i < n; ++i) s += p[3 * i + tid];
    ctr[tid] = s / (float)n;
  }
  __syncthreads();
  if (tid < n) {
    const float* M = A.rot + (size_t)b * 9;
    const float x = p[3 * tid] - ctr[0], y = p[3 * tid + 1] - ctr[1], z = p[3 * tid + 2] - ctr[2];
    float ox = M[0] * x + M[1] * y + M[2] * z, oy = M[3] * x + M[4] * y + M[5] * z, oz = M[6] * x + M[7] * y + M[8] * z;
    if (A.tr != nullptr) { ox += A.tr[3 * b]; oy += A.tr[3 * b + 1]; oz += A.tr[3 * b + 2]; }
    float* o = A.pos_out + ((size_t)b * n + tid) * 3;
    o[0] = ox; o[1] = oy; o[2] = oz;
  }
}

hipError_t launch_randomize(const RandPosArgs& A, hipStream_t s) {
  hipLaunchKernelGGL(randomize_kernel, dim3(A.B), dim3(256), 0, s, A);
  return hipGetLastError();
}

__global__ __launch_bounds__(256) void pose_metrics_kernel(const float* pos, const float* ref, const uint8_t* mask, const int32_t* perms, int n_perms,
                                                           const float* rec_pos, int n_lig, int n_rec, float* out) {
  __shared__ float p[MAX_LIG * 3], rf[MAX_LIG * 3];
  __shared__ unsigned char keep[MAX_LIG];
  __shared__ float red[4][256];
  const int b = blockIdx.x, tid = threadIdx.x;
  for (int i = tid; i < n_lig * 3; i += 256) { p[i] = pos[(size_t)b * n_lig * 3 + i]; rf[i] = ref[i]; }
  for (int i = tid; i < n_lig; i += 256) keep[i] = mask ? (mask[i] != 0) : 1;
  __syncthreads();
  float cnt = 0.f, cx = 0.f, cy = 0.f, cz = 0.f, rx = 0.f, ry = 0.f, rz = 0.f;
  float mcross = INFINITY, mself = INFINITY;
  for (int i = tid; i < n_lig; i += 256)
    if (keep[i]) {
      cnt += 1.f;
      cx += p[3 * i]; cy += p[3 * i + 1]; cz += p[3 * i + 2];
      rx += rf[3 * i]; ry += rf[3 * i + 1]; rz += rf[3 * i + 2];
      for (int j = 0; j < n_lig; ++j)
        if (j != i && keep[j]) {
          const float ex = p[3 * i] - p[3 * j], ey = p[3 * i + 1] - p[3 * j + 1], ez = p[3 * i + 2] - p[3 * j + 2];
          mself = fminf(mself, ex * ex + ey * ey + ez * ez);
        }
    }
  float best = INFINITY;
  const int K = perms ? n_perms : 1;
  for (int k = tid; k < K; k += 256) {
    float s2 = 0.f;
    for (int i = 0; i < n_lig; ++i)
      if (keep[i]) {
        const int j = perms ? perms[(size_t)k * n_lig + i] : i;
        if ((unsigned)j >= (unsigned)n_lig) { s2 = INFINITY; break; }
        const float dx = p[3 * j] - rf[3 * i], dy = p[3 * j + 1] - rf[3 * i + 1], dz = p[3 * j + 2] - rf[3 * i + 2];
        s2 += dx * dx + dy * dy + dz * dz;
      }
    best = fminf(best, s2);
  }
  for (int r = tid; r < n_rec; r += 256) {
    const float qx = rec_pos[3 * r], qy = rec_pos[3 * r + 1], qz = rec_pos[3 * r + 2];
    for (int i = 0; i < n_lig; ++i)
      if (keep[i]) {
        const float ex = qx - p[3 * i], ey = qy - p[3 * i + 1], ez = qz - p[3 * i + 2];
        mcross = fminf(mcross, ex * ex + ey * ey + ez * ez);
      }
  }
  float vals[7] = {cnt, cx, cy, cz, rx, ry, rz};
  float sums[7];
  for (int k = 0; k < 7; ++k) {
    red[0][tid] = vals[k];
    __syncthreads();
    for (int o = 128; o > 0; o >>= 1) { if (tid < o) red[0][tid] += red[0][tid + o]; __syncthreads(); }
    sums[k] = red[0][0];
    __syncthreads();
  }
  red[1][tid] = mcross; red[2][tid] = mself; red[3][tid] = best;
  __syncthreads();
  for (int o = 128; o > 0; o >>= 1) {
    if (tid < o) {
      red[1][tid] = fminf(red[1][tid], red[1][tid + o]); red[2][tid] = fminf(red[2][tid], red[2][tid + o]);
      red[3][tid] = fminf(red[3][tid], red[3][tid + o]);
    }
    __syncthreads();
  }
  if (tid == 0) {
    const float n = fmaxf(sums[0], 1.f);
    const float dx = (sums[1] - sums[4]) / n, dy = (sums[2] - sums[5]) / n, dz = (sums[3] - sums[6]) / n;
    out[4 * b + 0] = sqrtf(red[3][0] / n);
    out[4 * b + 1] = sqrtf(dx * dx + dy * dy + dz * dz);
    out[4 * b + 2] = sqrtf(red[1][0]);
    out[4 * b + 3] = sqrtf(red[2][0]);
  }
}

hipError_t launch_pose_metrics(const float* pos, const float* ref, const uint8_t* mask, const int32_t* perms, int n_perms, const float* rec_pos,
                               int B, int n_lig, int n_rec, float* out, hipStream_t s) {
  hipLaunchKernelGGL(pose_metrics_kernel, dim3(B), dim3(256), 0, s, pos, ref, mask, perms, n_perms, rec_pos, n_lig, n_rec, out);
  return hipGetLastError();
}

__global__ void cfg_combine_kernel(float* score, const float* uncond, float w, int64_t n) {
  const int64_t i = (int64_t)blockIdx.x * blockDim.x + threadIdx.x;
  if (i < n) score[i] = score[i] + w * (score[i] - uncond[i]);
}

hipError_t launch_cfg_combine(float* score, const float* uncond, float weight, int64_t n, hipStream_t s) {
  if (n == 0) return hipSuccess;
  hipLaunchKernelGGL(cfg_combine_kernel, dim3((unsigned)((n + 255) / 256)), dim3(256), 0, s, score, uncond, weight, n);
  return hipGetLastError();
}

hipError_t launch_se3(const Se3Args& A, hipStream_t s, const HeadArgs* post) {
  const bool rec = A.rec_pos != nullptr || A.rec_scores != nullptr || A.rec_perturb != nullptr || A.rec_edges != nullptr;
  HeadArgs H0 = {};
  const HeadArgs& H = post ? *post : H0;
  if (post && rec) hipLaunchKernelGGL((se3_update_kernel<true, true>), dim3(A.B), dim3(256), 0, s, A, H);
  else if (post) hipLaunchKernelGGL((se3_update_kernel<true, false>), dim3(A.B), dim3(256), 0, s, A, H);
  else if (rec) hipLaunchKernelGGL((se3_update_kernel<false, true>), dim3(A.B), dim3(256), 0, s, A, H);
  else hipLaunchKernelGGL((se3_update_kernel<false, false>), dim3(A.B), dim3(256), 0, s, A, H);
  return hipGetLastError();
}

}
```

disco_diffdock_amd/csrc/model.h:

```cpp
#pragma once
#include <stdio.h>
#include <stdlib.h>
#include <thread>

#include "ddk_internal.h"

namespace ddk {

constexpr int SIG = 32;
constexpr int DE = 32;
constexpr int MAX_LIG = 256;
constexpr int MAX_REC = 8192;
constexpr int LIG_CAP = 33;
constexpr int BOND_CAP = 32;
constexpr int LIG_DIMS[16] = {119, 4, 12, 12, 8, 10, 6, 6, 2, 8, 2, 2, 2, 2, 2, 2};
constexpr int REC_DIM = 38;

enum InfoSlot : int {
  I_GO = 5,
  I_CNT = 10,
  I_FB = 18,
  I_E = 24,
  I_OVF = 25,
  I_MISMATCH = 31,
// ... 39 lines not shown
  const float* final_edge_b1;
  const float *lig_w_lat, *rec_w_lat;
  const float *lig_node_unc, *rec_node_unc;
  int latent_dim;
  const float *fc_w0, *fc_b0, *fc_w4, *fc_b4;
  float fc_bn_scale[4];
  const float *tr_w0n, *tr_w3, *rot_w0n, *rot_w3;
  float tr_b3, rot_b3;
  const float *tb_w0, *tb_b0, *tb_w4, *tb_b4;
  const float *tb_bn_scale, *tb_bn_mean, *tb_bn_bias;
  const float *tf_w0, *tf_w3;
  const float *rec_table, *rec_w_emb, *rec_w_lm_t, *rec_b;
};

constexpr int AR_H = 128;
constexpr int AR_NS_MAX = 24;
struct ArMlpDev { const float *w0, *b0, *w4, *b4, *w8; float b8; };
struct ArArgs {
  const float* x;
  ArMlpDev s, r;
  int ar_ns, H;
  int n_lig_total, n_rec_total, n_lig, n_rec;
  float* logits;
};
struct ArDecodeArgs {
  const float* logits;
  const float* uniforms;
  float temperature;
  int n_lig, n_rec, idx, latent_dim;
  float* lig_latent;
  float* rec_latent;
  int32_t* choices;
};
hipError_t launch_ar_logits(const ArArgs& A, hipStream_t s);
hipError_t launch_ar_decode(const ArDecodeArgs& A, int B, hipStream_t s);

struct ModelHost {
  std::vector<float> lig_tables;
  std::vector<int> lig_table_off;
  std::vector<float> lig_w_emb, lig_w_sig, lig_b;
  std::vector<float> rec_table, rec_w_emb, rec_w_esm, rec_w_sig, rec_b;
  std::vector<float> le_w1s, le_b1, re_w1s, re_b1, ce_w1s, ce_b1, cen_w1s, cen_b1;
  std::vector<float> re_w1d;
  std::vector<float> tr_w0s, tr_b0, rot_w0s, rot_b0;
  float rec_coeff = 0.f;
  std::vector<float> rec_offset;
  bool ready = false;
};

struct ConfPredictorDev {
  float *w0 = nullptr, *s0 = nullptr, *t0 = nullptr, *w4 = nullptr, *s4 = nullptr, *t4 = nullptr, *w8 = nullptr, *b8 = nullptr;
  int n_out = 1;
};
int conf_predictor_load(ddk_ctx* ctx, ConfPredictorDev& P);
hipError_t launch_conf_head(const ConfPredictorDev& P, const float* x, int B, int n_lig, float* out, const int32_t* ovf, hipStream_t s);

struct Model {
  ModelDev dev;
  ModelHost host;
  bool confidence_mode = false;
  ConfPredictorDev pred;
  bool has_ar = false;
  ArMlpDev ar_s, ar_r;
  int ar_ns = 0, ar_H = 0;
};


struct GraphArgs {
  const float* lig_pos;
  const float* rec_pos;
  const int32_t* bond_src;
  const int32_t* bond_dst;
  const int32_t* rr_src;
  const int32_t* rr_dst;
  const int32_t* rr_outdeg;
  int B, n_lig, n_rec, M, E_rr;
  float lig_r2;
  float cross_cutoff;
  const int32_t* rr_start;
  int32_t* counts;
  int32_t* offs;
  int32_t* info;
  uint8_t* levels;
  int prune = 0;
  int shared_rr = 0;
  int32_t* e_src;
  int32_t* e_dst;
  int32_t* e_aux;
  int32_t* deg;
  int rec_node_base = -1;
  int64_t patch_off = -1;
  int64_t edge_cap = 0;
  int cross_mirror = 0;
};

int det_ranges_count(int kind, int B);
hipError_t launch_det_ranges(const GraphArgs& G, int kind, int len_uniform, int32_t* out, hipStream_t s);

struct PatchArgs {
  const float* rec_latent;
  const int32_t* rr_start;
  const int32_t* rr_outdeg;
  const int32_t* rr_dst;
  int B, n_lig, n_rec, E_rr, latent_dim;
  int64_t patch_off;
  uint8_t* rr_mask;
  int32_t* patch_cnt;
  int32_t* info;
  int32_t *e_src, *e_dst, *e_aux;
};
hipError_t launch_disco_patch(const PatchArgs& a, hipStream_t s);

struct EdgeFeatArgs {
  const float* lig_pos;
  const float* rec_pos;
  const float* bond_attr;
  const float* rr_pre1;
  const float* rr_sh;
  const int32_t* e_src;
  const int32_t* e_dst;
  const int32_t* e_aux;
  const int32_t* info;
  float* e_emb;
  float* e_sh;
  EdgeMlpDev lig, rec, cross;
  StepParams sp;
  int n_lig_total;
  int rec_node_base = -1;
  int n_rec;
  int n_shared = 0;
  int cross_mirror = 0;
  int g2_live_only = 0;
  int64_t patch_off = -1;
  const float* lig_latent;
  const float* rec_latent;
  float unconditional;
  int latent_dim;
};

struct HeadArgs {
  const float* lig_pos;
  const float* x;
  ModelDev md;
  StepParams sp;
  int B, n_lig, R;
  int scale_by_sigma;
  const int32_t* rot_u;
  const int32_t* rot_v;
  float lig_r2;
  float* tr_out;
  float* rot_out;
  float* tor_out;
  int32_t *h_src, *h_dst, *h_deg, *h_info;
  float *h_attr, *h_sh, *h_sum;
  int32_t* prof_out = nullptr;
  const int32_t* exec_info = nullptr;
  int deterministic;
};

struct Se3Args {
  const float* pos;
  const float* tr;
  const float* rot;
  const float* tor;
  const float* noise;
  float sc[3], nc[3];
  const int32_t* rot_u;
  const int32_t* rot_v;
  const uint8_t* mask_rotate;
  int B, n_lig, R;
  float* pos_out;
  float* rec_pos = nullptr;
  float* rec_scores = nullptr;
  float* rec_perturb = nullptr;
  int32_t* rec_edges = nullptr;
  const int32_t* info = nullptr;
};

struct RandPosArgs {
  const float* pos0;
  const float* tor;
  const float* rot;
  const float* tr;
  const int32_t* rot_u;
  const int32_t* rot_v;
  const uint8_t* mask_rotate;
  int B, n_lig, R;
  float* pos_out;
};
hipError_t launch_randomize(const RandPosArgs& A, hipStream_t s);
hipError_t launch_debug_kabsch(const float* A, const float* Bp, int B, int n, float* R_out, float* t_out, hipStream_t s);
hipError_t launch_debug_axis_angle(const float* aa, int n, float* R_out, hipStream_t s);
hipError_t launch_pose_metrics(const float* pos, const float* ref, const uint8_t* mask, const int32_t* perms, int n_perms, const float* rec_pos,
                               int B, int n_lig, int n_rec, float* out, hipStream_t s);

int conf_model_finalize(ddk_ctx* ctx);
void conf_complex_free(ddk_complex* cx);
void conf_model_destroy(ddk_ctx* ctx);
struct ConfComplex;

hipError_t launch_graph(const GraphArgs& G, int64_t edge_cap, hipStream_t s);
GraphArgs graph_args(const ddk_ctx* ctx, const ddk_complex* cx, int B, const float* lig_pos, float cross_cutoff);
int graph_cross_mirror_fits(int n_lig, int n_rec);
hipError_t launch_edge_features(const EdgeFeatArgs& A, int64_t edge_cap, hipStream_t s);
hipError_t launch_edge_features_node(const EdgeFeatArgs& A, int64_t edge_cap, const NodePreArgs& P, const NodeEmbedArgs& E, hipStream_t s);
struct NodeEmbedArgs {
  const float* lig_static; const float* rec_static; StepParams sp; int B, n_lig, n_rec; float* x;
  const float *lig_latent, *rec_latent, *lig_w_lat, *rec_w_lat, *lig_unc, *rec_unc; float unconditional; int latent_dim;
};
hipError_t launch_node_embed(const NodeEmbedArgs& a, hipStream_t s);
struct RecStaticArgs { const float* rec_x; int n_rec, feat_dim, lm; const float *rec_table, *w_emb, *w_lm_t, *b; float* out; };
hipError_t launch_complex_static(const RecStaticArgs& R, const int32_t* rr_src, const int32_t* rr_dst, const float* rec_pos, int E, const EdgeMlpDev& m,
                                 float* pre1, hipStream_t s);
hipError_t launch_zero_fill(void* p, size_t bytes, hipStream_t s);
hipError_t launch_heads_pre(const HeadArgs& A, bool torsion, hipStream_t s);
hipError_t launch_heads_post(const HeadArgs& A, bool torsion, hipStream_t s);
hipError_t launch_se3(const Se3Args& A, hipStream_t s, const HeadArgs* post = nullptr);
hipError_t launch_cfg_combine(float* score, const float* uncond, float weight, int64_t n, hipStream_t s);

}

struct ddk_complex {
  int n_lig = 0, n_rec = 0, M = 0, R = 0, E_rr = 0, max_batch = 0;
  int32_t *bond_src = nullptr, *bond_dst = nullptr, *rot_u = nullptr, *rot_v = nullptr, *rot_bond = nullptr;
  float* bond_attr = nullptr;
  uint8_t* mask_rotate = nullptr;
  float *rec_pos = nullptr, *lig_node_static = nullptr, *rec_node_static = nullptr;
  int32_t *rr_src = nullptr, *rr_dst = nullptr, *rr_outdeg = nullptr, *rr_start = nullptr;
  float *rr_pre1 = nullptr, *rr_sh = nullptr;
  int64_t edge_cap = 0;
  int32_t *e_src = nullptr, *e_dst = nullptr, *e_aux = nullptr, *deg = nullptr, *counts = nullptr, *offs = nullptr, *info = nullptr;
  uint8_t* levels = nullptr;
  float *e_emb = nullptr, *e_sh = nullptr, *xa = nullptr, *xb = nullptr, *sum = nullptr;
  float* scores = nullptr;
  const float *lig_latent = nullptr, *rec_latent = nullptr;
  float unconditional = 0.0f;
  int64_t patch_off = -1;
  uint8_t* rr_mask = nullptr;
  int32_t* patch_cnt = nullptr;
  bool latent_dirty = true;
  int patch_B = 0;
  float cfg_weight = 0.0f, cfg_start = 1.0f, cfg_end = 0.0f;
  float *zero_lat = nullptr, *scores2 = nullptr;
  float* part = nullptr;
  int32_t* det_rng = nullptr;
  float* sum_rr0 = nullptr;
  int32_t *h_src = nullptr, *h_dst = nullptr, *h_deg = nullptr;
  float *h_attr = nullptr, *h_sh = nullptr, *h_sum = nullptr;
  float* pre = nullptr;
  float* x_last = nullptr;
  int last_B = 0;
  bool sum_clean = false;
  bool keep_rec = false, last_full = false;
  ddk::ConfComplex* conf = nullptr;
  ddk_ctx* owner = nullptr;
  struct Chunk { void* p; size_t cap; };
  std::vector<Chunk> allocs;
  char* chunk = nullptr;
  size_t chunk_cap = 0, chunk_off = 0, reserve_hint = 0;
  bool oom = false;
  int stage_idx = -1;
  size_t stage_off = 0;
  struct CopyRec { void* dst; size_t off, bytes; };
  std::vector<CopyRec> pending;
  hipEvent_t ready = nullptr;
  bool ready_pending = false;
  hipStream_t last_stream = nullptr;
  std::vector<hipStream_t> streams;
  bool used = false;
  struct Canary { char* tail; size_t bytes; };
  std::vector<Canary> canaries;
  std::vector<int32_t> h_rr;
  std::vector<float> h_rec_pos;
};

#define GET(var, name, ...) const HostTensor* var = find_w(ctx, name, {__VA_ARGS__}); if (!var) return DDK_ERR_INVALID
#define CK(x, what) do { hipError_t ck_e = (x); if (ck_e != hipSuccess) return hip_fail(ctx, ck_e, what); } while (0)

namespace ddk {
const HostTensor* find_w(ddk_ctx* ctx, const std::string& name, std::initializer_list<int64_t> shape);
std::vector<float> cols(const HostTensor* t, int c0, int c1);
std::vector<float> transpose_rm(const std::vector<float>& w, int rows, int cols_);

template <typename F>
inline void host_parallel_for(int n, F&& body) {
  unsigned nt = std::thread::hardware_concurrency();
  nt = nt < 1 ? 1 : (nt > 8 ? 8 : nt);
  if (n < 512 || nt == 1) {
    for (int i = 0; i < n; ++i) body(i);
    return;
  }
  std::vector<std::thread> th;
  const int per = (n + (int)nt - 1) / (int)nt;
  for (unsigned t = 0; t < nt; ++t) {
    const int lo = (int)t * per, hi = lo + per < n ? lo + per : n;
    if (lo >= hi) break;
    th.emplace_back([lo, hi, &body]() { for (int i = lo; i < hi; ++i) body(i); });
  }
  for (auto& x : th) x.join();
}


void* cx_new_chunk(ddk_complex* cx, size_t cap);
int cx_stage_begin(ddk_ctx* ctx, ddk_complex* cx, size_t bytes);
bool cx_put(ddk_complex* cx, void* dst, const void* src, size_t bytes);
int cx_stage_flush(ddk_ctx* ctx, ddk_complex* cx);
hipError_t cx_wait_ready(ddk_complex* cx, hipStream_t s);
inline void cx_reserve(ddk_complex* cx, size_t bytes) { cx->reserve_hint = bytes; }
inline bool cx_canary_on() { static const bool on = getenv("DDK_CANARY") != nullptr; return on; }
inline void* cx_alloc(ddk_complex* cx, size_t bytes) {
  const size_t need = (((bytes ? bytes : 4) + 255) & ~(size_t)255) + (cx_canary_on() ? 4096 : 0);
  if (!cx->chunk || cx->chunk_off + need > cx->chunk_cap) {
    size_t cap = need > cx->reserve_hint ? need : cx->reserve_hint;
    if (cap < ((size_t)1 << 20)) cap = (size_t)1 << 20;
    void* p = cx_new_chunk(cx, cap);
    if (!p) { cx->oom = true; return nullptr; }
    cx->chunk = (char*)p; cx->chunk_off = 0; cx->reserve_hint = 0;
  }
  void* r = cx->chunk + cx->chunk_off;
  cx->chunk_off += need;
  if (cx_canary_on()) {
    char* tail = (char*)r + (need - 4096);
    if (hipMemset(tail, 0xA5, 4096) != hipSuccess) { cx->oom = true; return nullptr; }
    cx->canaries.push_back({tail, bytes});
  }
  {
    static const bool trace = getenv("DDK_TRACE_ALLOC") != nullptr;
    if (trace && bytes >= 4096) fprintf(stderr, "[ddk alloc] cx %p ctx %p  %p .. %p  (%zu B, chunk %p + %zu of %zu)\n", (void*)cx, (void*)cx->owner, r, (void*)((char*)r + bytes), bytes,
                                        (void*)cx->chunk, cx->chunk_off - need, cx->chunk_cap);
  }
  return r;
}
template <typename T>
inline T* cx_upload(ddk_complex* cx, const T* src, size_t n) {
  T* p = (T*)cx_alloc(cx, n * sizeof(T));
  if (!p || (n && src && !cx_put(cx, p, src, n * sizeof(T)))) return nullptr;
  return p;
}
}
```

disco_diffdock_amd/csrc/model.hip:

```cpp
#include <math.h>
#include <string.h>

#include <algorithm>
#include <thread>

#include "model.h"

namespace ddk {

std::vector<float> cols(const HostTensor* t, int c0, int c1) {
  const int rows = (int)t->shape[0], nc = (int)t->shape[1];
  std::vector<float> o((size_t)rows * (c1 - c0));
  for (int r = 0; r < rows; ++r)
    for (int c = c0; c < c1; ++c) o[(size_t)r * (c1 - c0) + (c - c0)] = t->data[(size_t)r * nc + c];
  return o;
}

static bool smearing(ddk_ctx* ctx, const char* name, float stop, EdgeMlpDev& m, std::vector<float>* host_off, float* host_coeff) {
  std::vector<float> off(DE);
  auto it = ctx->weights.find(std::string(name) + "_distance_expansion.offset");
  if (it != ctx->weights.end() && it->second.data.size() == (size_t)DE) off = it->second.data;
  else for (int k = 0; k < DE; ++k) off[k] = stop * (float)k / (float)(DE - 1);
  const double d = (double)(off[1] - off[0]);
  m.coeff = (float)(-0.5 / (d * d));
// ... 251 lines not shown
  {
    float idx = (log10f(sp.rot_sigma) - (float)log10(0.01)) / (float)(log10(2.0) - log10(0.01)) * 1000.0f;
    long i = lrintf(idx);
    i = i < 0 ? 0 : (i > 999 ? 999 : i);
    sp.so3_norm = (float)ctx->so3_table[i];
  }
  {
    float s = logf(sp.tor_sigma / (float)M_PI);
    s = (s - (float)log(3e-3)) / (float)(log(2.0) - log(3e-3)) * 5000.0f;
    s = s < 0.f ? 0.f : (s > 5000.f ? 5000.f : s);
    const long i = lrintf(s);
    sp.torus_norm_sqrt = sqrtf((float)ctx->torus_table[i]);
  }
  return DDK_OK;
}

constexpr size_t CHUNK_POOL_MAX_CHUNKS = 1024;
constexpr size_t CHUNK_POOL_MAX_BYTES = (size_t)96 << 30;

size_t pool_evict_idle(ddk_ctx* ctx, bool wait) {
  size_t freed = 0;
  for (size_t i = 0; i < ctx->chunk_pool.size();) {
    ddk_ctx::PoolChunk& c = ctx->chunk_pool[i];
    const bool idle = !c.free_after || hipEventQuery(c.free_after) == hipSuccess;
    if (!idle && !wait) { ++i; continue; }
    if (!idle) hipEventSynchronize(c.free_after);
    if (c.free_after) hipEventDestroy(c.free_after);
    ctx_free(ctx, c.p);
    freed += c.cap;
    ctx->chunk_pool_bytes -= c.cap;
    ctx->pool_frees++;
    ctx->chunk_pool.erase(ctx->chunk_pool.begin() + i);
  }
  return freed;
}

void* cx_new_chunk(ddk_complex* cx, size_t cap) {
  ddk_ctx* ctx = cx->owner;
  {
    size_t c2 = (size_t)1 << 20;
    while (c2 < cap) c2 = (c2 & (c2 - 1)) ? (c2 / 3) * 4 : c2 + c2 / 2;
    cap = c2;
  }
  int best = -1;
  for (int i = 0; i < (int)ctx->chunk_pool.size(); ++i) {
    const auto& c = ctx->chunk_pool[i];
    if (c.free_after && hipEventQuery(c.free_after) != hipSuccess) continue;
    if (c.cap >= cap && c.cap <= 2 * cap && (best < 0 || c.cap < ctx->chunk_pool[best].cap)) best = i;
  }
  void* p = nullptr;
  if (best >= 0) {
    ddk_ctx::PoolChunk c = ctx->chunk_pool[best];
    ctx->chunk_pool.erase(ctx->chunk_pool.begin() + best);
    ctx->chunk_pool_bytes -= c.cap;
    if (c.free_after) hipEventDestroy(c.free_after);
    p = c.p; cap = c.cap;
    ctx->pool_reuses++;
  } else {
    if (ctx_malloc(ctx, &p, cap) != hipSuccess) {
      if (pool_evict_idle(ctx, false) == 0 || ctx_malloc(ctx, &p, cap) != hipSuccess)
        if (pool_evict_idle(ctx, true) == 0 || ctx_malloc(ctx, &p, cap) != hipSuccess) {
          ctx->err = "out of device memory: a complex asked for a chunk of " + std::to_string(cap) + " B (context holds " + std::to_string(ctx->dev_bytes) + " B" +
                     (ctx->alloc_limit > 0 ? ", debug limit " + std::to_string(ctx->alloc_limit) + " B" : std::string()) + "); retry with a smaller batch";
          return nullptr;
        }
    }
    ctx->pool_mallocs++;
  }
  ctx->pool_bytes_out += (int64_t)cap;
  if (ctx->pool_bytes_out > ctx->pool_bytes_out_peak) ctx->pool_bytes_out_peak = ctx->pool_bytes_out;
  cx->allocs.push_back({p, cap});
  cx->chunk_cap = cap;
  return p;
}

int cx_stage_begin(ddk_ctx* ctx, ddk_complex* cx, size_t bytes) {
  bytes = (bytes + 4095) & ~(size_t)4095;
  int idx = -1;
  for (int i = 0; i < (int)ctx->stage_pool.size(); ++i) {
    auto& b = ctx->stage_pool[i];
    if (b.in_flight && hipEventQuery(b.done) == hipSuccess) b.in_flight = false;
    if (!b.in_flight && b.cap >= bytes && (idx < 0 || b.cap < ctx->stage_pool[idx].cap)) idx = i;
  }
  if (idx < 0) {
    ddk_ctx::StageBuf b;
    b.cap = bytes < ((size_t)8 << 20) ? ((size_t)8 << 20) : bytes;
    if (hipHostMalloc((void**)&b.p, b.cap) != hipSuccess) return fail(ctx, DDK_ERR_NOMEM, "hipHostMalloc failed (staging buffer)");
    if (hipEventCreateWithFlags(&b.done, hipEventDisableTiming) != hipSuccess) return fail(ctx, DDK_ERR_HIP, "event create failed");
    ctx->stage_pool.push_back(b);
    idx = (int)ctx->stage_pool.size() - 1;
  }
  ctx->stage_pool[idx].in_flight = true;
  cx->stage_idx = idx; cx->stage_off = 0; cx->pending.clear();
  return DDK_OK;
}

bool cx_put(ddk_complex* cx, void* dst, const void* src, size_t bytes) {
  if (!dst || !bytes) return dst != nullptr;
  ddk_ctx* ctx = cx->owner;
  if (cx->stage_idx >= 0) {
    auto& b = ctx->stage_pool[cx->stage_idx];
    const size_t off = (cx->stage_off + 255) & ~(size_t)255;
    if (off + bytes <= b.cap) {
      memcpy(b.p + off, src, bytes);
      cx->stage_off = off + bytes;
      if (!cx->pending.empty()) {
        auto& l = cx->pending.back();
        const size_t gap = off - l.off;
        if ((char*)l.dst + gap == (char*)dst && gap >= l.bytes && gap - l.bytes < 256) { l.bytes = gap + bytes; return true; }
      }
      cx->pending.push_back({dst, off, bytes});
      return true;
    }
  }
  if (hipMemcpyAsync(dst, src, bytes, hipMemcpyHostToDevice, ctx->up_stream) != hipSuccess) return false;
  return hipStreamSynchronize(ctx->up_stream) == hipSuccess;
}

int cx_stage_flush(ddk_ctx* ctx, ddk_complex* cx) {
  hipError_t e = hipSuccess;
  if (cx->stage_idx >= 0) {
    auto& b = ctx->stage_pool[cx->stage_idx];
    for (const auto& r : cx->pending)
      if (e == hipSuccess) e = hipMemcpyAsync(r.dst, b.p + r.off, r.bytes, hipMemcpyHostToDevice, ctx->up_stream);
    if (e == hipSuccess) e = hipEventRecord(b.done, ctx->up_stream);
    cx->pending.clear();
    cx->stage_idx = -1;
  }
  if (e == hipSuccess && !cx->ready) e = hipEventCreateWithFlags(&cx->ready, hipEventDisableTiming);
  if (e == hipSuccess) e = hipEventRecord(cx->ready, ctx->up_stream);
  if (e != hipSuccess) return hip_fail(ctx, e, "complex upload");
  cx->ready_pending = true;
  return DDK_OK;
}

hipError_t cx_wait_ready(ddk_complex* cx, hipStream_t s) {
  cx->last_stream = s; cx->used = true;
  if (std::find(cx->streams.begin(), cx->streams.end(), s) == cx->streams.end()) cx->streams.push_back(s);
  if (!cx->ready_pending) return hipSuccess;
  if (hipEventQuery(cx->ready) == hipSuccess) { cx->ready_pending = false; return hipSuccess; }
  return hipStreamWaitEvent(s, cx->ready, 0);
}

GraphArgs graph_args(const ddk_ctx* ctx, const ddk_complex* cx, int B, const float* lig_pos, float cross_cutoff) {
  GraphArgs G;
  G.lig_pos = lig_pos; G.rec_pos = cx->rec_pos; G.bond_src = cx->bond_src; G.bond_dst = cx->bond_dst;
  G.rr_src = cx->rr_src; G.rr_dst = cx->rr_dst; G.rr_outdeg = cx->rr_outdeg; G.rr_start = cx->rr_start;
  G.B = B; G.n_lig = cx->n_lig; G.n_rec = cx->n_rec; G.M = cx->M; G.E_rr = cx->E_rr;
  G.lig_r2 = ctx->cfg.lig_max_radius * ctx->cfg.lig_max_radius; G.cross_cutoff = cross_cutoff; G.counts = cx->counts; G.offs = cx->offs; G.info = cx->info; G.levels = cx->levels;
  return G;
}

static hipError_t build_graph(ddk_ctx* ctx, ddk_complex* cx, int B, const float* lig_pos, float cross_cutoff, bool prune, bool shared_rr,
                              hipStream_t s, int64_t patch_off = -1, int cross_mirror = 0) {
  GraphArgs G = graph_args(ctx, cx, B, lig_pos, cross_cutoff);
  G.cross_mirror = cross_mirror; G.prune = prune ? 1 : 0; G.shared_rr = shared_rr ? 1 : 0; G.patch_off = patch_off;
  G.e_src = cx->e_src; G.e_dst = cx->e_dst; G.e_aux = cx->e_aux; G.deg = cx->deg;
  return launch_graph(G, cx->edge_cap, s);
}

static int score_forward_impl(ddk_ctx* ctx, ddk_complex* cx, int B, const float* lig_pos, const StepParams& sp,
                              float* tr_out, float* rot_out, float* tor_out, hipStream_t s, HeadArgs* defer_post = nullptr) {
  const ddk_config& c = ctx->cfg;
  Model* M = (Model*)ctx->model;
  const int n_lig = cx->n_lig, n_rec = cx->n_rec;
  const int64_t N = (int64_t)B * (n_lig + n_rec);
  const bool patched = c.latent_dim > 0 && ctx->layer0_dedup && !c.deterministic && cx->patch_off >= 0 && cx->pre != nullptr &&
                       ctx->conv[0].wn != nullptr && c.num_conv_layers > 1;
  const bool dedup = ((c.latent_dim == 0 && ctx->layer0_dedup) || patched) && B > 1 && cx->E_rr > 0;
  if (c.latent_dim > 0 && (!cx->lig_latent || !cx->rec_latent))
    return fail(ctx, DDK_ERR_STATE, "latent-conditioned model: call ddk_set_latents before the forward");
  if (dedup && patched && (cx->latent_dirty || cx->patch_B != B)) {
    PatchArgs P;
    P.rec_latent = cx->rec_latent; P.rr_start = cx->rr_start; P.rr_outdeg = cx->rr_outdeg; P.rr_dst = cx->rr_dst;
    P.B = B; P.n_lig = n_lig; P.n_rec = n_rec; P.E_rr = cx->E_rr; P.latent_dim = c.latent_dim; P.patch_off = cx->patch_off;
    P.rr_mask = cx->rr_mask; P.patch_cnt = cx->patch_cnt; P.info = cx->info; P.e_src = cx->e_src; P.e_dst = cx->e_dst; P.e_aux = cx->e_aux;
    CK(launch_disco_patch(P, s), "layer-0 patch group");
    cx->latent_dirty = false; cx->patch_B = B;
  }
  const bool prune = ctx->prune && !cx->keep_rec && cx->E_rr > 0;
  const int mirror = graph_cross_mirror_fits(n_lig, n_rec);
  CK(build_graph(ctx, cx, B, lig_pos, sp.cross_cutoff, prune, dedup, s, (dedup && patched) ? cx->patch_off : -1, mirror), "graph build");
  EdgeFeatArgs F;
  F.cross_mirror = mirror;
  F.lig_pos = lig_pos; F.rec_pos = cx->rec_pos; F.bond_attr = cx->bond_attr; F.rr_pre1 = cx->rr_pre1; F.rr_sh = cx->rr_sh;
  F.e_src = cx->e_src; F.e_dst = cx->e_dst; F.e_aux = cx->e_aux; F.info = cx->info; F.e_emb = cx->e_emb; F.e_sh = cx->e_sh;
  F.lig = M->dev.lig_edge; F.rec = M->dev.rec_edge; F.cross = M->dev.cross_edge; F.sp = sp;
  F.n_lig_total = B * n_lig; F.n_rec = n_rec; F.n_shared = dedup ? cx->E_rr : 0;
  F.g2_live_only = (dedup && prune && c.num_conv_layers == 5) ? 1 : 0;
  F.patch_off = (dedup && patched) ? cx->patch_off : -1;
  F.latent_dim = c.latent_dim; F.lig_latent = cx->lig_latent; F.rec_latent = cx->rec_latent; F.unconditional = cx->unconditional;
  const int64_t cap_b = (int64_t)B * ((int64_t)cx->M + (int64_t)n_lig * LIG_CAP + 2LL * n_lig * n_rec + cx->E_rr) + cx->E_rr;
  const int64_t feat_cap = (cap_b < cx->edge_cap ? cap_b : cx->edge_cap) + (F.patch_off >= 0 ? (int64_t)B * cx->E_rr + 256 : 0);
  float* xin = cx->xa;
  float* xout = cx->xb;
  NodeEmbedArgs NE_;
  NE_.lig_static = cx->lig_node_static; NE_.rec_static = cx->rec_node_static; NE_.sp = sp; NE_.B = B; NE_.n_lig = n_lig; NE_.n_rec = n_rec;
  NE_.x = xin; NE_.lig_latent = cx->lig_latent; NE_.rec_latent = cx->rec_latent; NE_.lig_w_lat = M->dev.lig_w_lat; NE_.rec_w_lat = M->dev.rec_w_lat;
  NE_.lig_unc = M->dev.lig_node_unc; NE_.rec_unc = M->dev.rec_node_unc; NE_.unconditional = cx->unconditional; NE_.latent_dim = c.latent_dim;
  const bool split = ctx->conv[0].wn != nullptr && cx->pre != nullptr;
  if (split) {
    NodePreArgs PA = {};
    PA.x_out = xin; PA.n_lig_total = B * n_lig; PA.n_rec_total = B * n_rec; PA.n_rec = n_rec;
    PA.wn = ctx->conv[0].wn; PA.bnp = ctx->conv[0].bnp; PA.pre = cx->pre; PA.n_slots = 1; PA.lig_roles = 15; PA.rec_roles = 15;
    CK(launch_edge_features_node(F, feat_cap, PA, NE_, s), "edge features + node embed + node_pre");
  } else {
    CK(launch_edge_features(F, feat_cap, s), "edge features");
    CK(launch_node_embed(NE_, s), "node embed");
  }
  if (!cx->sum_clean) {
    CK(hipMemsetAsync(cx->sum, 0, (size_t)cx->max_batch * (n_lig + n_rec) * XW * sizeof(float) * (c.deterministic ? 2 : 1), s), "memset sum");
    CK(hipMemsetAsync(cx->sum_rr0, 0, (size_t)n_rec * XW * sizeof(float), s), "memset sum_rr0");
  }
  cx->sum_clean = false;
  bool rr0_dirty = false;
  const int NL = c.num_conv_layers;
  int32_t* prof_slot = nullptr;
  if (ctx->prof && ctx->prof_slots + 1 <= ctx->prof_cap) prof_slot = ctx->prof_edges + (size_t)PROF_INTS * ctx->prof_slots;
  for (int l = 0; l < NL; ++l) {
    const ConvLayerDev& L = ctx->conv[l];
    ConvLaunch a;
    a.x = xin; a.src = cx->e_src; a.dst = cx->e_dst; a.edge_attr = cx->e_emb; a.sh = cx->e_sh; a.sum = cx->sum;
    a.tile_info = cx->info; a.counter = cx->info + I_CNT + (l % 8); a.gather = 1;
    a.pre = split ? cx->pre : nullptr;
    const bool lig_only = (l == NL - 1 && !cx->keep_rec);
    const bool shared0 = dedup && l == 0;
    int tab = TAB_ALL;
    if (shared0) tab = TAB_SHARED;
    else if (prune && l == NL - 2) tab = TAB_A;
    else if (prune && l == NL - 3) tab = TAB_B;
    else if (prune && l == NL - 4) tab = TAB_C;
    a.gbeg = cx->info + I_TAB + 8 * tab; a.gend = a.gbeg + 4;
    a.n_groups = 4; a.n_active = lig_only ? 2 : 4; a.n_slots = 1; a.slots = 0;
    if (shared0 && patched) {
      a.gbeg = cx->info + I_TABX; a.gend = a.gbeg + 5; a.n_groups = 5; a.n_active = 5; a.wmap = 0x23210ull;
    }
    if (c.deterministic) {
      a.n_slots = 2; a.slots = (0u) | (1u << 2) | (0u << 4) | (1u << 6);
      a.part = cx->part; a.edge_bound = cap_b;
      const int kind = lig_only ? 0 : (shared0 ? 5 : (tab == TAB_A ? 1 : (tab == TAB_B ? 2 : (tab == TAB_C ? 3 : 4))));
      GraphArgs Gd = {};
      Gd.counts = cx->counts; Gd.B = B; Gd.M = cx->M; Gd.E_rr = cx->E_rr;
      CK(launch_det_ranges(Gd, kind, 0, cx->det_rng, s), "deterministic ranges");
      a.det_rng = cx->det_rng; a.det_nr = det_ranges_count(kind, B);
    }
    if (shared0) {
      rr0_dirty = true;
      a.sum_g2 = cx->sum_rr0; a.g2_node_off = B * n_lig;
    }
    if (l >= 8) CK(hipMemsetAsync(cx->info + I_CNT + (l % 8), 0, sizeof(int32_t), s), "counter reset");
    ddk_ctx::ProfRec pr;
    if (prof_slot) {
      CK(hipEventCreate(&pr.a), "event"); CK(hipEventCreate(&pr.b), "event");
      pr.layer = l; pr.slot = ctx->prof_slots; pr.tab = tab; pr.lig_only = lig_only; pr.r01_skipped = shared0 ? (patched ? -1 : (int64_t)(B - 1) * cx->E_rr) : 0;
      CK(hipEventRecord(pr.a, s), "event record");
    }
    a.use_y = ctx->cfg.conv_kernel == 2;
    if (ctx->conv_trace != nullptr && ctx->conv_trace_layer == l) { a.trace = ctx->conv_trace; a.trace_coarse = ctx->conv_trace_coarse; }
    CK(launch_conv_fused(L, a, ctx->n_cu, s), "conv_fused");
    if (prof_slot) {
      CK(hipEventRecord(pr.b, s), "event record");
      ctx->prof_recs.push_back(pr);
    }
    const bool clear_rr0 = rr0_dirty && !shared0;
    if (split && l + 1 < NL) {
      NodePreArgs PA = {};
      PA.sum = cx->sum; PA.deg = cx->deg; PA.x_in = xin; PA.bn_mean = L.bn_mean; PA.bn_scale = L.bn_scale; PA.bn_bias = L.bn_bias;
      PA.dout = L.dout; PA.x_out = xout; PA.sum_rr0 = shared0 ? cx->sum_rr0 : nullptr; PA.n_lig_total = B * n_lig; PA.n_rec_total = B * n_rec;
      PA.rr0_mask = (shared0 && patched) ? cx->rr_mask : nullptr;
      PA.n_rec = n_rec; PA.zero_extra = clear_rr0 ? cx->sum_rr0 : nullptr; PA.n_extra = clear_rr0 ? (int64_t)n_rec * XW : 0;
      PA.wn = ctx->conv[l + 1].wn; PA.bnp = ctx->conv[l + 1].bnp; PA.pre = cx->pre; PA.n_slots = c.deterministic ? 2 : 1;
      const bool next_lig_only = (l + 1 == NL - 1) && !cx->keep_rec;
      PA.lig_roles = next_lig_only ? 0x7 : 0xF; PA.rec_roles = next_lig_only ? 0x4 : 0xF;
      PA.levels = prune ? cx->levels : nullptr; PA.max_level = l == NL - 2 ? 0 : (l == NL - 3 ? 1 : (l == NL - 4 ? 2 : 3));
      CK(launch_node_finalize_pre(PA, true, s), "node_finalize_pre");
    } else
    CK(launch_node_finalize(cx->sum, cx->deg, xin, L.bn_mean, L.bn_scale, L.bn_bias, lig_only ? (int64_t)B * n_lig : N, L.dout, XW, xout, s,
                            shared0 ? cx->sum_rr0 : nullptr, (int64_t)B * n_lig, n_rec, 1, clear_rr0 ? cx->sum_rr0 : nullptr,
                            clear_rr0 ? (int64_t)n_rec * XW : 0, c.deterministic ? 2 : 1, (shared0 && patched) ? cx->rr_mask : nullptr), "node_finalize");
    if (clear_rr0) rr0_dirty = false;
    float* t = xin; xin = xout; xout = t;
  }
  cx->x_last = xin;
  cx->last_B = B;
  cx->last_full = cx->keep_rec;
  cx->sum_clean = !rr0_dirty;
  if (M->confidence_mode) return DDK_OK;
  const bool torsion = !c.no_torsion && tor_out != nullptr && cx->R > 0;
  HeadArgs Hd;
  Hd.lig_pos = lig_pos; Hd.x = xin; Hd.md = M->dev; Hd.sp = sp; Hd.B = B; Hd.n_lig = n_lig; Hd.R = cx->R;
  Hd.scale_by_sigma = c.scale_by_sigma; Hd.rot_u = cx->rot_u; Hd.rot_v = cx->rot_v; Hd.lig_r2 = c.lig_max_radius * c.lig_max_radius;
  Hd.tr_out = tr_out; Hd.rot_out = rot_out; Hd.tor_out = tor_out;
  Hd.h_src = cx->h_src; Hd.h_dst = cx->h_dst; Hd.h_deg = cx->h_deg; Hd.h_info = cx->info + I_HEAD; Hd.h_attr = cx->h_attr; Hd.h_sh = cx->h_sh;
  Hd.h_sum = cx->h_sum; Hd.deterministic = c.deterministic;
  if (prof_slot) {
    Hd.prof_out = prof_slot; Hd.exec_info = cx->info + I_EXEC;
    ctx->prof_slots += 1;
  }
  CK(launch_heads_pre(Hd, torsion, s), "heads_pre");
  int32_t* head_rng = nullptr;
  if (c.deterministic) {
    head_rng = cx->det_rng + (4 * (7 * (size_t)cx->max_batch + 1) + 8);
    GraphArgs Gd = {};
    Gd.B = B;
    CK(launch_det_ranges(Gd, 6, n_lig, head_rng, s), "deterministic ranges (head)");
  }
  if (torsion) {
    CK(hipEventRecord(ctx->ev_fork, s), "head fork");
    CK(hipStreamWaitEvent(ctx->head_stream, ctx->ev_fork, 0), "head fork");
  }
  for (int hd = 1; hd >= (torsion ? 0 : 1); --hd) {
    ConvLaunch a;
    a.x = xin; a.src = cx->h_src; a.dst = cx->h_dst; a.edge_attr = cx->h_attr; a.sh = cx->h_sh; a.sum = cx->h_sum;
    a.tile_info = cx->info; a.counter = cx->info + I_HEAD + 4 + hd; a.gather = 0; a.pre = nullptr;
    a.n_groups = 1; a.n_active = 1; a.n_slots = 1; a.slots = 0;
    a.gbeg = cx->info + I_HEAD + (hd == 1 ? 0 : 2); a.gend = a.gbeg + 1;
    if (c.deterministic) {
      const int64_t eh = (int64_t)B * (n_lig + (int64_t)cx->R * BOND_CAP);
      a.part = cx->part + (hd == 1 ? 0 : ((size_t)B + 2) * CONV_WAVES * 2 * XW); a.edge_bound = eh;
      if (hd == 1) { a.det_rng = head_rng; a.det_nr = B; }
    }
    CK(launch_conv_fused(ctx->head[hd], a, ctx->n_cu, (hd == 1 && torsion) ? ctx->head_stream : s), "conv_fused (head)");
  }
  if (torsion) {
    CK(hipEventRecord(ctx->ev_join, ctx->head_stream), "head join");
    CK(hipStreamWaitEvent(s, ctx->ev_join, 0), "head join");
  }
  if (defer_post) *defer_post = Hd;
  else CK(launch_heads_post(Hd, torsion, s), "heads_post");
  return DDK_OK;
}

}

using namespace ddk;

static int check_model(ddk_ctx* ctx, ddk_complex* cx, int B) {
  if (!ctx) return DDK_ERR_INVALID;
  if (ctx->host_only) return fail(ctx, DDK_ERR_STATE, "host-only context (device < 0) cannot launch kernels");
  if (!ctx->finalized || !ctx->model || !((Model*)ctx->model)->host.ready)
    return fail(ctx, DDK_ERR_STATE, "score model weights not loaded / finalised");
  if (!cx) return fail(ctx, DDK_ERR_INVALID, "null complex");
  if (B < 1 || B > cx->max_batch) return fail(ctx, DDK_ERR_INVALID, "batch size exceeds the complex's max_batch");
  return DDK_OK;
}

extern "C" {

int ddk_complex_create(ddk_ctx* ctx, const ddk_complex_desc* d, int32_t max_batch, ddk_complex** out) {
  if (!ctx || !d || !out) return DDK_ERR_INVALID;
  if (ctx->host_only) return fail(ctx, DDK_ERR_STATE, "host-only context (device < 0) cannot hold device data");
  if (!ctx->finalized) return fail(ctx, DDK_ERR_STATE, "ddk_finalize_weights has not run");
  const ddk_config& c = ctx->cfg;
  const bool has_model = ctx->model != nullptr;
  static const ModelHost no_model;
  const ModelHost& H = has_model ? ((Model*)ctx->model)->host : no_model;
  if (d->n_lig < 1 || d->n_lig > MAX_LIG) return fail(ctx, DDK_ERR_INVALID, "n_lig must be in [1, 256]");
  if (d->n_rec < 1 || d->n_rec > ctx->max_rec)
    return fail(ctx, DDK_ERR_INVALID, "n_rec must be in [1, " + std::to_string(ctx->max_rec) + "]: the graph kernels keep a sample's receptor (17 B per residue) in LDS");
  if (has_model && d->rec_feat_dim != 1 + c.lm_embedding_dim) return fail(ctx, DDK_ERR_INVALID, "receptor feature width != 1 + lm_embedding_dim");
  if (max_batch < 1) return fail(ctx, DDK_ERR_INVALID, "max_batch < 1");
  hipSetDevice(c.device);
  ddk_complex* cx = new ddk_complex();
  cx->owner = ctx;
  *out = cx;
  cx->n_lig = d->n_lig; cx->n_rec = d->n_rec; cx->M = d->n_bond_edges; cx->R = d->n_rot; cx->E_rr = d->n_rec_edges;
  cx->max_batch = max_batch;
  const int n_lig = d->n_lig, n_rec = d->n_rec, M = d->n_bond_edges, lm = c.lm_embedding_dim;
  {
    const size_t E0 = (size_t)d->n_rec_edges, Bm0 = (size_t)max_batch, R0 = (size_t)(d->n_rot > 0 ? d->n_rot : 1);
    const size_t cap0 = Bm0 * ((size_t)M + (size_t)n_lig * LIG_CAP + 2 * (size_t)n_lig * n_rec + E0) + E0 + 64, N0 = Bm0 * (size_t)(n_lig + n_rec);
    size_t need = (size_t)M * 24 + R0 * 8 + R0 * n_lig + (size_t)n_rec * 12 + (size_t)(n_lig + n_rec) * NS * 4 + E0 * (8 + NS * 4 + 16) + (size_t)n_rec * 4 +
                  (size_t)n_rec * d->rec_feat_dim * 4;
    need += cap0 * (12 + NS * 4 + 16) + N0 * 4 + N0 * PRE_W * 4 + (c.deterministic ? N0 * XW * 4 + (cap0 / 32 + 128 + 8 * (7 * Bm0 + 8)) * 2 * XW * 4 + 64 * (7 * Bm0 + 8) : 0) + Bm0 * ((size_t)n_lig + R0 * BOND_CAP + 2) * (8 + NE * 4 + 16) + Bm0 * (1 + R0) * (XW * 4 + 4) + 8 * 256 + Bm0 * 2 * CNT_STRIDE * 4 + INFO_INTS * 4 + (size_t)n_rec * 4 + Bm0 * n_rec + 3 * N0 * XW * 4 + (size_t)n_rec * XW * 4 + Bm0 * n_lig * 12 + 2 * Bm0 * (6 + R0) * 4;
    if (c.latent_dim > 0) need += N0 * c.latent_dim * 4 + Bm0 * E0 * (12 + NS * 4 + 16) + Bm0 * n_rec + (Bm0 + 1) * 4 + 3 * 256;
    cx_reserve(cx, need + 64 * 256);
    const size_t staged = (size_t)M * 24 + R0 * 8 + R0 * n_lig + (size_t)n_rec * 12 + (size_t)n_lig * NS * 4 + E0 * (8 + 16) +
                          (size_t)n_rec * 8 + (size_t)n_rec * d->rec_feat_dim * 4 + 24 * 256;
    int rc0 = cx_stage_begin(ctx, cx, staged);
    if (rc0) return rc0;
  }
  std::vector<int32_t> ru, rv;
  for (int m = 0; m < M; ++m) {
    const int a = d->bond_index[m], b = d->bond_index[M + m];
    if (a < 0 || a >= n_lig || b < 0 || b >= n_lig) return fail(ctx, DDK_ERR_INVALID, "bond index out of range");
    if (d->edge_mask[m]) { ru.push_back(a); rv.push_back(b); }
  }
  if ((int)ru.size() != d->n_rot) return fail(ctx, DDK_ERR_INVALID, "edge_mask.sum() != n_rot");
  for (int r = 0; r < d->n_rot; ++r)
    if (d->mask_rotate[(size_t)r * n_lig + ru[r]] || !d->mask_rotate[(size_t)r * n_lig + rv[r]])
      return fail(ctx, DDK_ERR_INVALID, "mask_rotate orientation: u must be fixed and v rotating for every rotatable bond");
  cx->bond_src = cx_upload(cx, d->bond_index, (size_t)M);
  cx->bond_dst = cx_upload(cx, d->bond_index + M, (size_t)M);
  cx->bond_attr = cx_upload(cx, d->bond_attr, (size_t)M * 4);
  cx->rot_u = cx_upload(cx, ru.data(), ru.size());
  cx->rot_v = cx_upload(cx, rv.data(), rv.size());
  cx->mask_rotate = cx_upload(cx, d->mask_rotate, (size_t)d->n_rot * n_lig);
  cx->rec_pos = cx_upload(cx, d->rec_pos, (size_t)n_rec * 3);
  std::vector<float> ls((size_t)n_lig * NS);
  for (int i = 0; has_model && i < n_lig; ++i) {
    float emb[NS] = {0};
    for (int f = 0; f < 16; ++f) {
      const int v = d->lig_x[(size_t)i * 16 + f];
      if (v < 0 || v >= LIG_DIMS[f]) return fail(ctx, DDK_ERR_INVALID, "ligand categorical feature out of range");
      const float* row = H.lig_tables.data() + (size_t)(H.lig_table_off[f] + v) * NS;
      for (int k = 0; k < NS; ++k) emb[k] += row[k];
    }
    for (int o = 0; o < NS; ++o) {
      double a = H.lig_b[o];
      for (int k = 0; k < NS; ++k) a += (double)H.lig_w_emb[(size_t)o * NS + k] * emb[k];
      ls[(size_t)i * NS + o] = (float)a;
    }
  }
  for (int j = 0; has_model && j < n_rec; ++j) {
    const int res = (int)d->rec_x[(size_t)j * d->rec_feat_dim];
    if (res < 0 || res >= REC_DIM) return fail(ctx, DDK_ERR_INVALID, "residue id out of range");
  }
  float* rec_x_dev = has_model ? cx_upload(cx, d->rec_x, (size_t)n_rec * d->rec_feat_dim) : nullptr;
  cx->lig_node_static = cx_upload(cx, ls.data(), ls.size());
  cx->rec_node_static = cx_upload<float>(cx, nullptr, (size_t)n_rec * NS);
  const int E = d->n_rec_edges;
  std::vector<int32_t> outdeg(n_rec, 0);
  std::vector<float> sh((size_t)E * 4);
  for (int k = 0; k < E; ++k) {
    const int a = d->rec_edge_index[k], b = d->rec_edge_index[E + k];
    if (a < 0 || a >= n_rec || b < 0 || b >= n_rec) return fail(ctx, DDK_ERR_INVALID, "receptor edge index out of range");
    if (k > 0 && a < d->rec_edge_index[k - 1]) return fail(ctx, DDK_ERR_INVALID, "receptor edges must be grouped by source (process_mols.py:337-353 order)");
    outdeg[a]++;
    const float vx = d->rec_pos[3 * b] - d->rec_pos[3 * a], vy = d->rec_pos[3 * b + 1] - d->rec_pos[3 * a + 1],
                vz = d->rec_pos[3 * b + 2] - d->rec_pos[3 * a + 2];
    const float dist = sqrtf(vx * vx + vy * vy + vz * vz);
    const float inv = 1.7320508075688772f / fmaxf(dist, 1e-12f);
    sh[4 * (size_t)k] = 1.0f; sh[4 * (size_t)k + 1] = vx * inv; sh[4 * (size_t)k + 2] = vy * inv; sh[4 * (size_t)k + 3] = vz * inv;
  }
  cx->h_rr.assign(d->rec_edge_index, d->rec_edge_index + 2 * (size_t)E);
  cx->h_rec_pos.assign(d->rec_pos, d->rec_pos + 3 * (size_t)n_rec);
  cx->rr_src = cx_upload(cx, d->rec_edge_index, (size_t)E);
  cx->rr_dst = cx_upload(cx, d->rec_edge_index + E, (size_t)E);
  cx->rr_outdeg = cx_upload(cx, outdeg.data(), outdeg.size());
  std::vector<int32_t> rstart(n_rec, 0);
  for (int j = 1; j < n_rec; ++j) rstart[j] = rstart[j - 1] + outdeg[j - 1];
  cx->rr_start = cx_upload(cx, rstart.data(), rstart.size());
  cx->rr_pre1 = cx_upload<float>(cx, nullptr, (size_t)E * NS);
  cx->rr_sh = cx_upload(cx, sh.data(), sh.size());
  const int64_t Bm = max_batch;
  cx->edge_cap = Bm * ((int64_t)M + (int64_t)n_lig * LIG_CAP + 2LL * n_lig * n_rec + E) + E + 64;
  if (cx->edge_cap >= ((int64_t)1 << 31)) return fail(ctx, DDK_ERR_INVALID, "edge capacity exceeds int32 (reduce max_batch)");
  const int64_t N = Bm * (n_lig + n_rec);
  const int64_t patch_cap = (has_model && c.latent_dim > 0 && E > 0) ? Bm * (int64_t)E : 0;
  if (cx->edge_cap + patch_cap >= ((int64_t)1 << 31)) return fail(ctx, DDK_ERR_INVALID, "edge capacity exceeds int32 (reduce max_batch)");
  const int64_t e_alloc = cx->edge_cap + patch_cap;
  cx->e_src = cx_upload<int32_t>(cx, nullptr, e_alloc);
  cx->e_dst = cx_upload<int32_t>(cx, nullptr, e_alloc);
  cx->e_aux = cx_upload<int32_t>(cx, nullptr, e_alloc);
  cx->e_emb = cx_upload<float>(cx, nullptr, e_alloc * NS);
  cx->e_sh = cx_upload<float>(cx, nullptr, e_alloc * 4);
  if (patch_cap > 0) {
    cx->patch_off = cx->edge_cap;
    cx->rr_mask = cx_upload<uint8_t>(cx, nullptr, Bm * n_rec);
    cx->patch_cnt = cx_upload<int32_t>(cx, nullptr, Bm + 1);
  }
  cx->deg = cx_upload<int32_t>(cx, nullptr, N);
  cx->counts = cx_upload<int32_t>(cx, nullptr, Bm * CNT_STRIDE);
  cx->offs = cx_upload<int32_t>(cx, nullptr, Bm * CNT_STRIDE);
  cx->info = cx_upload<int32_t>(cx, nullptr, INFO_INTS);
  cx->levels = cx_upload<uint8_t>(cx, nullptr, Bm * n_rec);
  cx->xa = cx_upload<float>(cx, nullptr, N * XW);
  cx->xb = cx_upload<float>(cx, nullptr, N * XW);
  const int det = c.deterministic ? 1 : 0;
  cx->sum = cx_upload<float>(cx, nullptr, N * XW * (det ? 2 : 1));
  if (det) {
    cx->part = cx_upload<float>(cx, nullptr, (cx->edge_cap / CONV_BLOCK_EDGES + 16 + 7 * Bm + 8) * CONV_WAVES * 2 * XW);
    cx->det_rng = cx_upload<int32_t>(cx, nullptr, 2 * (4 * (7 * Bm + 1) + 8));
  }
  cx->sum_rr0 = cx_upload<float>(cx, nullptr, (int64_t)n_rec * XW);
  if (has_model) cx->pre = cx_upload<float>(cx, nullptr, N * PRE_W);
  if (has_model) {
    const int64_t Eh = Bm * ((int64_t)n_lig + (int64_t)(d->n_rot > 0 ? d->n_rot : 0) * BOND_CAP) + 64, Nh = Bm * (1 + (int64_t)(d->n_rot > 0 ? d->n_rot : 0)) + 1;
    cx->h_src = cx_upload<int32_t>(cx, nullptr, Eh);
    cx->h_dst = cx_upload<int32_t>(cx, nullptr, Eh);
    cx->h_attr = cx_upload<float>(cx, nullptr, Eh * NE);
    cx->h_sh = cx_upload<float>(cx, nullptr, Eh * 4);
    cx->h_deg = cx_upload<int32_t>(cx, nullptr, Nh);
    cx->h_sum = cx_upload<float>(cx, nullptr, Nh * XW);
    if (cx->h_sum) launch_zero_fill(cx->h_sum, (size_t)Nh * XW * sizeof(float), ctx->up_stream);
  }
  cx->scores = cx_upload<float>(cx, nullptr, Bm * (6 + (d->n_rot > 0 ? d->n_rot : 1)));
  cx->scores2 = cx_upload<float>(cx, nullptr, Bm * (6 + (d->n_rot > 0 ? d->n_rot : 1)));
  if (c.latent_dim > 0) {
    cx->zero_lat = cx_upload<float>(cx, nullptr, N * c.latent_dim);
    if (cx->zero_lat) launch_zero_fill(cx->zero_lat, (size_t)N * c.latent_dim * sizeof(float), ctx->up_stream);
  }
  if (cx->oom || !cx->bond_src || !cx->rr_sh || !cx->scores)
    return fail(ctx, DDK_ERR_NOMEM, "ddk_complex_create (max_batch " + std::to_string(max_batch) + ", " + std::to_string(n_rec) + " residues): " +
                (ctx->err.rfind("out of device memory", 0) == 0 ? ctx->err : std::string("device allocation failed")));
  hipMemsetAsync(cx->info, 0, INFO_INTS * sizeof(int32_t), ctx->up_stream);
  if (cx->sum && cx->sum_rr0) {
    launch_zero_fill(cx->sum, (size_t)N * XW * sizeof(float) * (det ? 2 : 1), ctx->up_stream);
    launch_zero_fill(cx->sum_rr0, (size_t)n_rec * XW * sizeof(float), ctx->up_stream);
    cx->sum_clean = true;
  }
  int rcf = cx_stage_flush(ctx, cx);
  if (rcf || !has_model) return rcf;
  {
    const ModelDev& MD = ((Model*)ctx->model)->dev;
    RecStaticArgs RS;
    RS.rec_x = rec_x_dev; RS.n_rec = n_rec; RS.feat_dim = d->rec_feat_dim; RS.lm = lm; RS.rec_table = MD.rec_table; RS.w_emb = MD.rec_w_emb; RS.w_lm_t = MD.rec_w_lm_t;
    RS.b = MD.rec_b; RS.out = cx->rec_node_static;
    hipError_t e = launch_complex_static(RS, cx->rr_src, cx->rr_dst, cx->rec_pos, E, MD.rec_edge, cx->rr_pre1, ctx->up_stream);
    if (e == hipSuccess) e = hipEventRecord(cx->ready, ctx->up_stream);
    if (e != hipSuccess) return hip_fail(ctx, e, "static precompute");
  }
  return DDK_OK;
}

void ddk_complex_destroy(ddk_ctx* ctx, ddk_complex* cx) {
  if (!cx) return;
  if (!ctx) ctx = cx->owner;
  hipSetDevice(ctx->cfg.device);
  if (!cx->canaries.empty()) {
    hipDeviceSynchronize();
    std::vector<unsigned char> h(4096);
    for (size_t i = 0; i < cx->canaries.size(); ++i) {
      if (hipMemcpy(h.data(), cx->canaries[i].tail, 4096, hipMemcpyDeviceToHost) != hipSuccess) continue;
      size_t bad = 0, first = 4096;
      for (size_t k = 0; k < 4096; ++k) if (h[k] != 0xA5) { ++bad; if (first == 4096) first = k; }
      if (bad) fprintf(stderr, "[ddk canary] cx %p (n_lig %d n_rec %d all_atoms %d): allocation #%zu of %zu B overrun: %zu bytes changed, first at +%zu\n", (void*)cx, cx->n_lig, cx->n_rec,
                       ctx->cfg.all_atoms, i, cx->canaries[i].bytes, bad, first);
    }
  }
  if (cx->stage_idx >= 0) { ctx->stage_pool[cx->stage_idx].in_flight = false; cx->stage_idx = -1; }
  bool joined = true;
  for (hipStream_t o : cx->streams) {
    if (o == cx->last_stream) continue;
    hipEvent_t ev = nullptr;
    bool ok = hipEventCreateWithFlags(&ev, hipEventDisableTiming) == hipSuccess;
    if (ok) ok = hipEventRecord(ev, o) == hipSuccess && hipStreamWaitEvent(cx->last_stream, ev, 0) == hipSuccess;
    if (ev) hipEventDestroy(ev);
    joined = joined && ok;
  }
  if (!joined) hipDeviceSynchronize();
  for (auto& a : cx->allocs) {
    if (!a.p) continue;
    ddk_ctx::PoolChunk c;
    c.p = a.p; c.cap = a.cap;
    ctx->pool_bytes_out -= (int64_t)a.cap;
    bool ok = hipEventCreateWithFlags(&c.free_after, hipEventDisableTiming) == hipSuccess;
    if (ok) ok = hipEventRecord(c.free_after, cx->used ? cx->last_stream : ctx->up_stream) == hipSuccess;
    if (!ok || ctx->chunk_pool_bytes + c.cap > CHUNK_POOL_MAX_BYTES || ctx->chunk_pool.size() >= CHUNK_POOL_MAX_CHUNKS) {
      if (ok) hipEventSynchronize(c.free_after); else hipDeviceSynchronize();
      if (c.free_after) hipEventDestroy(c.free_after);
      ctx_free(ctx, a.p);
      ctx->pool_frees++;
      continue;
    }
    ctx->chunk_pool.push_back(c);
    ctx->chunk_pool_bytes += c.cap;
  }
  if (cx->ready) hipEventDestroy(cx->ready);
  conf_complex_free(cx);
  delete cx;
}

int ddk_score_confidence(ddk_ctx* ctx, ddk_complex* cx, int32_t B, const float* lig_pos, float t_tr, float t_rot, float t_tor, float* out,
                         void* stream) {
  int rc = check_model(ctx, cx, B);
  if (rc) return rc;
  Model* M = (Model*)ctx->model;
  if (!M->confidence_mode) return fail(ctx, DDK_ERR_STATE, "ddk_score_confidence needs a context created with confidence_mode = 1");
  if (!lig_pos || !out) return fail(ctx, DDK_ERR_INVALID, "ddk_score_confidence: null argument");
  { hipError_t we = cx_wait_ready(cx, (hipStream_t)stream); if (we != hipSuccess) return hip_fail(ctx, we, "wait for the complex upload"); }
  StepParams sp;
  if ((rc = make_step_params(ctx, t_tr, t_rot, t_tor, sp))) return rc;
  if ((rc = score_forward_impl(ctx, cx, B, lig_pos, sp, nullptr, nullptr, nullptr, (hipStream_t)stream))) return rc;
  hipError_t e = launch_conf_head(M->pred, cx->x_last, B, cx->n_lig, out, nullptr, (hipStream_t)stream);
  return e == hipSuccess ? DDK_OK : hip_fail(ctx, e, "confidence head");
}

int ddk_score_forward(ddk_ctx* ctx, ddk_complex* cx, int32_t B, const float* lig_pos, float t_tr, float t_rot, float t_tor,
                      float* tr_out, float* rot_out, float* tor_out, void* stream) {
  int rc = check_model(ctx, cx, B);
  if (rc) return rc;
  if (((Model*)ctx->model)->confidence_mode) return fail(ctx, DDK_ERR_STATE, "a confidence_mode context has no score heads (ddk_score_confidence)");
  { hipError_t we = cx_wait_ready(cx, (hipStream_t)stream); if (we != hipSuccess) return hip_fail(ctx, we, "wait for the complex upload"); }
  StepParams sp;
  if ((rc = make_step_params(ctx, t_tr, t_rot, t_tor, sp))) return rc;
  return score_forward_impl(ctx, cx, B, lig_pos, sp, tr_out, rot_out, tor_out, (hipStream_t)stream);
}

int ddk_build_graph(ddk_ctx* ctx, ddk_complex* cx, int32_t B, const float* lig_pos, float t_tr, int32_t* edge_src_out,
                    int32_t* edge_dst_out, int64_t cap, int32_t* group_offsets_out, void* stream) {
  int rc = check_model(ctx, cx, B);
  if (rc) return rc;
  { hipError_t we = cx_wait_ready(cx, (hipStream_t)stream); if (we != hipSuccess) return hip_fail(ctx, we, "wait for the complex upload"); }
  if (!lig_pos || !edge_src_out || !edge_dst_out || !group_offsets_out) return fail(ctx, DDK_ERR_INVALID, "ddk_build_graph: null argument");
  const int64_t cap_b = (int64_t)B * ((int64_t)cx->M + (int64_t)cx->n_lig * LIG_CAP + 2LL * cx->n_lig * cx->n_rec + cx->E_rr);
  const int64_t need = cap_b < cx->edge_cap ? cap_b : cx->edge_cap;
  if (cap < need) return fail(ctx, DDK_ERR_INVALID, "ddk_build_graph: cap " + std::to_string(cap) + " is below the worst case " + std::to_string(need) + " of this batch");
  StepParams sp;
  if ((rc = make_step_params(ctx, t_tr, t_tr, t_tr, sp))) return rc;
  hipStream_t s = (hipStream_t)stream;
  hipError_t e = build_graph(ctx, cx, B, lig_pos, sp.cross_cutoff, false, false, s);
  if (e == hipSuccess) e = hipMemcpyAsync(edge_src_out, cx->e_src, (size_t)need * sizeof(int32_t), hipMemcpyDeviceToDevice, s);
  if (e == hipSuccess) e = hipMemcpyAsync(edge_dst_out, cx->e_dst, (size_t)need * sizeof(int32_t), hipMemcpyDeviceToDevice, s);
  if (e == hipSuccess) e = hipMemcpyAsync(group_offsets_out, cx->info + I_GO, 5 * sizeof(int32_t), hipMemcpyDeviceToDevice, s);
  if (e != hipSuccess) return hip_fail(ctx, e, "ddk_build_graph");
  return DDK_OK;
}

int ddk_se3_update(ddk_ctx* ctx, ddk_complex* cx, int32_t B, const float* pos, const float* tr, const float* rot,
                   const float* tor, float* pos_out, void* stream) {
  if (!ctx) return DDK_ERR_INVALID;
  if (ctx->host_only) return fail(ctx, DDK_ERR_STATE, "host-only context (device < 0) cannot launch kernels");
  if (!cx || B < 1) return fail(ctx, DDK_ERR_INVALID, "bad complex / batch");
  { hipError_t we = cx_wait_ready(cx, (hipStream_t)stream); if (we != hipSuccess) return hip_fail(ctx, we, "wait for the complex upload"); }
  Se3Args A;
  A.pos = pos; A.tr = tr; A.rot = rot; A.tor = tor; A.noise = nullptr;
  for (int k = 0; k < 3; ++k) { A.sc[k] = 1.0f; A.nc[k] = 0.0f; }
  A.rot_u = cx->rot_u; A.rot_v = cx->rot_v; A.mask_rotate = cx->mask_rotate; A.B = B; A.n_lig = cx->n_lig; A.R = cx->R;
  A.pos_out = pos_out;
  hipError_t e = launch_se3(A, (hipStream_t)stream);
  if (e != hipSuccess) return hip_fail(ctx, e, "se3_update launch");
  return DDK_OK;
}

int ddk_randomize_position(ddk_ctx* ctx, ddk_complex* cx, int32_t B, const float* pos0, const float* tor, const float* rot,
                           const float* tr, float* pos_out, void* stream) {
  if (!ctx) return DDK_ERR_INVALID;
  if (ctx->host_only) return fail(ctx, DDK_ERR_STATE, "host-only context (device < 0) cannot launch kernels");
  if (!cx || B < 1 || !pos0 || !rot || !pos_out) return fail(ctx, DDK_ERR_INVALID, "ddk_randomize_position: bad complex / batch / null argument");
  { hipError_t we = cx_wait_ready(cx, (hipStream_t)stream); if (we != hipSuccess) return hip_fail(ctx, we, "wait for the complex upload"); }
  RandPosArgs A;
  A.pos0 = pos0; A.tor = tor; A.rot = rot; A.tr = tr;
  A.rot_u = cx->rot_u; A.rot_v = cx->rot_v; A.mask_rotate = cx->mask_rotate; A.B = B; A.n_lig = cx->n_lig; A.R = cx->R;
  A.pos_out = pos_out;
  hipError_t e = launch_randomize(A, (hipStream_t)stream);
  if (e != hipSuccess) return hip_fail(ctx, e, "randomize_position launch");
  return DDK_OK;
}

int ddk_pose_metrics(ddk_ctx* ctx, ddk_complex* cx, int32_t B, const float* pos, const float* ref_pos, const uint8_t* atom_mask,
                     const int32_t* perms, int32_t n_perms, const float* rec_atom_pos, int32_t n_rec_atoms, float* out, void* stream) {
  if (!ctx) return DDK_ERR_INVALID;
  if (ctx->host_only) return fail(ctx, DDK_ERR_STATE, "host-only context (device < 0) cannot launch kernels");
  if (!cx || B < 1 || !pos || !ref_pos || !out) return fail(ctx, DDK_ERR_INVALID, "ddk_pose_metrics: bad complex / batch / null argument");
  if ((perms != nullptr) != (n_perms > 0) || (rec_atom_pos != nullptr) != (n_rec_atoms > 0))
    return fail(ctx, DDK_ERR_INVALID, "ddk_pose_metrics: perms / n_perms and rec_atom_pos / n_rec_atoms come in pairs");
  { hipError_t we = cx_wait_ready(cx, (hipStream_t)stream); if (we != hipSuccess) return hip_fail(ctx, we, "wait for the complex upload"); }
  hipError_t e = launch_pose_metrics(pos, ref_pos, atom_mask, perms, n_perms, rec_atom_pos ? rec_atom_pos : cx->rec_pos, B, cx->n_lig,
                                     rec_atom_pos ? n_rec_atoms : cx->n_rec, out, (hipStream_t)stream);
  if (e != hipSuccess) return hip_fail(ctx, e, "pose_metrics launch");
  return DDK_OK;
}

}

static int sample_impl(ddk_ctx* ctx, ddk_complex* cx, int32_t B, int32_t steps, const float* t, const float* score_coeff, const float* noise_coeff,
                       const float* noise, float* pos, const ddk_trajectory& rec, void* stream, const char* what) {
  int rc = check_model(ctx, cx, B);
  if (rc) return rc;
  if (((Model*)ctx->model)->confidence_mode) return fail(ctx, DDK_ERR_STATE, "a confidence_mode context has no score heads (ddk_score_confidence)");
  { hipError_t we = cx_wait_ready(cx, (hipStream_t)stream); if (we != hipSuccess) return hip_fail(ctx, we, "wait for the complex upload"); }
  if (steps < 1 || !t || !score_coeff || !noise_coeff || !pos) return fail(ctx, DDK_ERR_INVALID, std::string(what) + ": null argument");
  hipStream_t s = (hipStream_t)stream;
  const int R = cx->R;
  const size_t pos_row = (size_t)B * cx->n_lig * 3, sc_row = (size_t)B * (6 + R);
  if (rec.pos) {
    hipError_t e0 = hipMemcpyAsync(rec.pos, pos, pos_row * sizeof(float), hipMemcpyDeviceToDevice, s);
    if (e0 != hipSuccess) return hip_fail(ctx, e0, "trajectory start-pose copy");
  }
  float* tr = cx->scores;
  float* rot = tr + (size_t)B * 3;
  float* tor = rot + (size_t)B * 3;
  const bool torsion = !ctx->cfg.no_torsion && R > 0;
  std::vector<StepParams> sps(steps);
  for (int k = 0; k < steps; ++k)
    if ((rc = make_step_params(ctx, t[3 * k], t[3 * k + 1], t[3 * k + 2], sps[k]))) return rc;
  const size_t n_sc = (size_t)B * (6 + (torsion ? R : 0));
  for (int k = 0; k < steps; ++k) {
    const bool guided = cx->cfg_weight != 0.0f && ctx->cfg.latent_dim > 0 && t[3 * k] <= cx->cfg_start && t[3 * k] >= cx->cfg_end;
    HeadArgs post;
    if ((rc = score_forward_impl(ctx, cx, B, pos, sps[k], tr, rot, torsion ? tor : nullptr, s, guided ? nullptr : &post))) return rc;
    if (guided) {
      const float* ll = cx->lig_latent; const float* rl = cx->rec_latent; const float un = cx->unconditional;
      cx->lig_latent = cx->zero_lat; cx->rec_latent = cx->zero_lat + (size_t)B * cx->n_lig * ctx->cfg.latent_dim; cx->unconditional = 1.0f;
      float* tr2 = cx->scores2;
      float* rot2 = tr2 + (size_t)B * 3;
      float* tor2 = rot2 + (size_t)B * 3;
      rc = score_forward_impl(ctx, cx, B, pos, sps[k], tr2, rot2, torsion ? tor2 : nullptr, s);
      cx->lig_latent = ll; cx->rec_latent = rl; cx->unconditional = un;
      if (rc) return rc;
      hipError_t e2 = launch_cfg_combine(cx->scores, cx->scores2, cx->cfg_weight, (int64_t)n_sc, s);
      if (e2 != hipSuccess) return hip_fail(ctx, e2, "cfg_combine launch");
    }
    Se3Args A;
    A.pos = pos; A.tr = tr; A.rot = rot; A.tor = torsion ? tor : nullptr;
    A.noise = noise ? noise + (size_t)k * B * (6 + R) : nullptr;
    for (int j = 0; j < 3; ++j) { A.sc[j] = score_coeff[3 * k + j]; A.nc[j] = noise_coeff[3 * k + j]; }
    A.rot_u = cx->rot_u; A.rot_v = cx->rot_v; A.mask_rotate = cx->mask_rotate; A.B = B; A.n_lig = cx->n_lig; A.R = R;
    A.pos_out = pos;
    if (rec.pos) A.rec_pos = rec.pos + (size_t)(k + 1) * pos_row;
    if (rec.scores) A.rec_scores = rec.scores + (size_t)k * sc_row;
    if (rec.perturb) A.rec_perturb = rec.perturb + (size_t)k * sc_row;
    if (rec.edge_counts) { A.rec_edges = rec.edge_counts + 4 * (size_t)k; A.info = cx->info; }
    hipError_t e = launch_se3(A, s, guided ? nullptr : &post);
    if (e != hipSuccess) return hip_fail(ctx, e, "se3_update launch");
  }
  return DDK_OK;
}

extern "C" {

int ddk_sample(ddk_ctx* ctx, ddk_complex* cx, int32_t B, int32_t steps, const float* t, const float* score_coeff,
               const float* noise_coeff, const float* noise, float* pos, void* stream) {
  return sample_impl(ctx, cx, B, steps, t, score_coeff, noise_coeff, noise, pos, ddk_trajectory{}, stream, "ddk_sample");
}

int ddk_sample_trajectory(ddk_ctx* ctx, ddk_complex* cx, int32_t B, int32_t steps, const float* t, const float* score_coeff,
                          const float* noise_coeff, const float* noise, float* pos, const ddk_trajectory* rec, void* stream) {
  return sample_impl(ctx, cx, B, steps, t, score_coeff, noise_coeff, noise, pos, rec ? *rec : ddk_trajectory{}, stream, "ddk_sample_trajectory");
}

int ddk_last_graph_stats(ddk_ctx* ctx, ddk_complex* cx, int64_t* out, void* stream) {
  if (!ctx || !cx || !out) return DDK_ERR_INVALID;
  int32_t info[INFO_INTS];
  hipError_t e = hipMemcpyAsync(info, cx->info, sizeof(info), hipMemcpyDeviceToHost, (hipStream_t)stream);
  if (e == hipSuccess) e = hipStreamSynchronize((hipStream_t)stream);
  if (e != hipSuccess) return hip_fail(ctx, e, "graph stats readback");
  for (int g = 0; g < 4; ++g) out[g] = info[I_GO + 1 + g] - info[I_GO + g];
  out[4] = info[I_SHARED] >= 0 ? cx->E_rr : 0;
  out[5] = info[I_E];
  out[6] = info[I_OVF];
  out[7] = cx->edge_cap;
  out[8] = info[I_SEG + 1] - info[I_SEG]; out[9] = info[I_SEG + 2] - info[I_SEG]; out[10] = info[I_SEG + 3] - info[I_SEG];
  out[11] = info[I_MISMATCH];
  return DDK_OK;
}

int ddk_last_node_features(ddk_ctx* ctx, ddk_complex* cx, int32_t B, float* lig_out, float* rec_out, void* stream) {
  if (!ctx || !cx || !cx->x_last || B != cx->last_B) return fail(ctx, DDK_ERR_STATE, "no forward with this batch size has run");
  if (rec_out && !cx->last_full)
    return fail(ctx, DDK_ERR_STATE, "receptor rows of the last conv layer were not evaluated: call ddk_set_keep_receptor_features(on) before the forward");
  hipStream_t s = (hipStream_t)stream;
  const size_t nl = (size_t)B * cx->n_lig * XW, nr = (size_t)B * cx->n_rec * XW;
  hipError_t e = hipSuccess;
  if (lig_out) e = hipMemcpyAsync(lig_out, cx->x_last, nl * sizeof(float), hipMemcpyDeviceToDevice, s);
  if (e == hipSuccess && rec_out) e = hipMemcpyAsync(rec_out, cx->x_last + nl, nr * sizeof(float), hipMemcpyDeviceToDevice, s);
  if (e != hipSuccess) return hip_fail(ctx, e, "node feature copy");
  return DDK_OK;
}

int ddk_set_latents(ddk_ctx* ctx, ddk_complex* cx, const float* lig_latent, const float* rec_latent, float unconditional) {
  if (!ctx || !cx) return DDK_ERR_INVALID;
  if ((lig_latent == nullptr) != (rec_latent == nullptr)) return fail(ctx, DDK_ERR_INVALID, "ddk_set_latents: pass both latent arrays or neither");
  cx->lig_latent = lig_latent; cx->rec_latent = rec_latent; cx->unconditional = unconditional;
  cx->latent_dirty = true;
  return DDK_OK;
}

int ddk_set_keep_receptor_features(ddk_ctx* ctx, ddk_complex* cx, int32_t on) {
  if (!ctx || !cx) return DDK_ERR_INVALID;
  cx->keep_rec = on != 0;
  return DDK_OK;
}

int ddk_ar_logits(ddk_ctx* ctx, ddk_complex* cx, int32_t B, float* logits_out, void* stream) {
  int rc = check_model(ctx, cx, B);
  if (rc) return rc;
  Model* M = (Model*)ctx->model;
  if (!M->has_ar) return fail(ctx, DDK_ERR_STATE, "no AR predictor weights in this context (latent_s_predictor.* / latent_r_predictor.*)");
  if (!logits_out) return fail(ctx, DDK_ERR_INVALID, "ddk_ar_logits: null argument");
  if (!cx->x_last || cx->last_B != B || !cx->last_full)
    return fail(ctx, DDK_ERR_STATE, "ddk_ar_logits needs a forward of this batch size with ddk_set_keep_receptor_features(on) first");
  { hipError_t we = cx_wait_ready(cx, (hipStream_t)stream); if (we != hipSuccess) return hip_fail(ctx, we, "wait for the complex upload"); }
  ArArgs A;
  A.x = cx->x_last; A.s = M->ar_s; A.r = M->ar_r; A.ar_ns = M->ar_ns; A.H = M->ar_H;
  A.n_lig_total = B * cx->n_lig; A.n_rec_total = B * cx->n_rec; A.n_lig = cx->n_lig; A.n_rec = cx->n_rec; A.logits = logits_out;
  hipError_t e = launch_ar_logits(A, (hipStream_t)stream);
  return e == hipSuccess ? DDK_OK : hip_fail(ctx, e, "ar_logits launch");
}

int ddk_ar_decode(ddk_ctx* ctx, ddk_complex* cx, int32_t B, const float* logits, float temperature, const float* uniforms,
                  int32_t decoding_idx, int32_t latent_dim, float* lig_latent, float* rec_latent, int32_t* choices, void* stream) {
  if (!ctx) return DDK_ERR_INVALID;
  if (ctx->host_only) return fail(ctx, DDK_ERR_STATE, "host-only context (device < 0) cannot launch kernels");
  if (!cx || B < 1 || !logits || !lig_latent || !rec_latent || latent_dim < 1 || decoding_idx < 0 || decoding_idx >= latent_dim)
    return fail(ctx, DDK_ERR_INVALID, "ddk_ar_decode: bad argument");
  if (temperature < 100.0f && !uniforms) return fail(ctx, DDK_ERR_INVALID, "ddk_ar_decode: uniforms are required below temperature 100");
  { hipError_t we = cx_wait_ready(cx, (hipStream_t)stream); if (we != hipSuccess) return hip_fail(ctx, we, "wait for the complex upload"); }
  ArDecodeArgs A;
  A.logits = logits; A.uniforms = uniforms; A.temperature = temperature; A.n_lig = cx->n_lig; A.n_rec = cx->n_rec; A.idx = decoding_idx;
  A.latent_dim = latent_dim; A.lig_latent = lig_latent; A.rec_latent = rec_latent; A.choices = choices;
  cx->latent_dirty = true;
  hipError_t e = launch_ar_decode(A, B, (hipStream_t)stream);
  return e == hipSuccess ? DDK_OK : hip_fail(ctx, e, "ar_decode launch");
}

int ddk_set_receptive_field_pruning(ddk_ctx* ctx, int32_t on) {
  if (!ctx) return DDK_ERR_INVALID;
  ctx->prune = on != 0;
  return DDK_OK;
}

int ddk_set_guidance(ddk_ctx* ctx, ddk_complex* cx, float weight, float cfg_start, float cfg_end) {
  if (!ctx || !cx) return DDK_ERR_INVALID;
  if (weight != 0.0f && ctx->cfg.latent_dim <= 0) return fail(ctx, DDK_ERR_INVALID, "classifier-free guidance needs a latent-conditioned model");
  cx->cfg_weight = weight; cx->cfg_start = cfg_start; cx->cfg_end = cfg_end;
  return DDK_OK;
}

int ddk_profile_enable(ddk_ctx* ctx, int32_t on) {
  if (!ctx) return DDK_ERR_INVALID;
  if (ctx->host_only) return fail(ctx, DDK_ERR_STATE, "host-only context");
  for (auto& r : ctx->prof_recs) { hipEventDestroy(r.a); hipEventDestroy(r.b); }
  ctx->prof_recs.clear();
  ctx->prof_slots = 0;
  if (on && !ctx->prof_edges) {
    ctx->prof_cap = 32768;
    if (hipHostMalloc((void**)&ctx->prof_edges, (size_t)ctx->prof_cap * PROF_INTS * sizeof(int32_t)) != hipSuccess)
      return fail(ctx, DDK_ERR_NOMEM, "hipHostMalloc failed");
  }
  ctx->prof = on != 0;
  return DDK_OK;
}

int ddk_profile_read(ddk_ctx* ctx, double* out, int32_t n) {
  if (!ctx || !out) return DDK_ERR_INVALID;
  const int L = ctx->cfg.num_conv_layers;
  if (n < 5 * L) return fail(ctx, DDK_ERR_INVALID, "profile buffer too small");
  for (int i = 0; i < 5 * L; ++i) out[i] = 0.0;
  hipError_t e = hipDeviceSynchronize();
  if (e != hipSuccess) return hip_fail(ctx, e, "profile sync");
  for (auto& r : ctx->prof_recs) {
    float ms = 0.f;
    e = hipEventElapsedTime(&ms, r.a, r.b);
    if (e != hipSuccess) return hip_fail(ctx, e, "hipEventElapsedTime");
    const int32_t* pe = ctx->prof_edges + (size_t)PROF_INTS * r.slot;
    const double E = pe[0], E01 = pe[1];
    out[5 * r.layer] += ms;
    out[5 * r.layer + 1] += 1.0;
    out[5 * r.layer + 2] += r.lig_only ? E01 : (double)pe[2 + r.tab];
    out[5 * r.layer + 3] += r.lig_only ? E01 : (r.r01_skipped < 0 ? (double)pe[2 + r.tab] : E - (double)r.r01_skipped);
    out[5 * r.layer + 4] += E;
  }
  return DDK_OK;
}

int ddk_profile_read_forwards(ddk_ctx* ctx, double* out, int32_t max_forwards) {
  if (!ctx || !out || max_forwards < 0) return DDK_ERR_INVALID;
  hipError_t e = hipDeviceSynchronize();
  if (e != hipSuccess) return hip_fail(ctx, e, "profile sync");
  const int nf = ctx->prof_slots < max_forwards ? ctx->prof_slots : max_forwards;
  for (int i = 0; i < 4 * nf; ++i) out[i] = 0.0;
  for (auto& r : ctx->prof_recs) {
    if (r.slot >= nf) continue;
    float ms = 0.f;
    e = hipEventElapsedTime(&ms, r.a, r.b);
    if (e != hipSuccess) return hip_fail(ctx, e, "hipEventElapsedTime");
// ... 78 lines not shown
```

Measured before the change: 48.42.

## Fuse next-step graph count into SE3 update and overlap head geometry on side stream

```diff
diff --git a/disco_diffdock_amd/csrc/ddk_capi.hip b/disco_diffdock_amd/csrc/ddk_capi.hip
--- a/disco_diffdock_amd/csrc/ddk_capi.hip
+++ b/disco_diffdock_amd/csrc/ddk_capi.hip
@@ -677,6 +677,8 @@
   if (e != hipSuccess) return hip_fail(ctx, e, "hipFuncSetAttribute(dynamic LDS)");
   e = graph_prepare_device(&ctx->max_rec);
   if (e != hipSuccess) return hip_fail(ctx, e, "hipFuncSetAttribute(dynamic LDS, graph kernels)");
+  e = se3_prepare_device();
+  if (e != hipSuccess) return hip_fail(ctx, e, "hipFuncSetAttribute(dynamic LDS, update + count kernel)");
   ctx->ws.tile_info = (int32_t*)dev_alloc(ctx, 64 * sizeof(int32_t));
   if (!ctx->ws.tile_info) return fail(ctx, DDK_ERR_NOMEM, "hipMalloc failed");
   return DDK_OK;
diff --git a/disco_diffdock_amd/csrc/k_graph.hip b/disco_diffdock_amd/csrc/k_graph.hip
--- a/disco_diffdock_amd/csrc/k_graph.hip
+++ b/disco_diffdock_amd/csrc/k_graph.hip
@@ -1,175 +1,13 @@
 #include <stdlib.h>
 #include "model.h"
 #include "k_node.h"
+#include "k_graph_count.h"
 
 namespace ddk {
 
 
-__device__ __forceinline__ bool cross_within(const float* lp, const float* rp, float c) {
-#pragma clang fp contract(off)
-  const float dx = rp[0] / c - lp[0] / c, dy = rp[1] / c - lp[1] / c, dz = rp[2] / c - lp[2] / c;
-  return dx * dx + dy * dy + dz * dz < 1.0f;
-}
-
-__device__ __forceinline__ bool cross_within4(const float4 a, float rx, float ry, float rz) {
-#pragma clang fp contract(off)
-  const float dx = rx - a.x, dy = ry - a.y, dz = rz - a.z;
-  return dx * dx + dy * dy + dz * dz < 1.0f;
-}
-
-__device__ __forceinline__ float dist2(const float* a, const float* b) {
-#pragma clang fp contract(off)
-  const float dx = a[0] - b[0], dy = a[1] - b[1], dz = a[2] - b[2];
-  return dx * dx + dy * dy + dz * dz;
-}
-
-constexpr int GT = 1024;
-
-__device__ void build_lig_adj(const float* lp, int n_lig, float r2, unsigned (*adj)[MAX_LIG / 32]) {
-  const int lane = threadIdx.x & 63, wave = threadIdx.x >> 6, nw = blockDim.x >> 6;
-  for (int i = wave; i < n_lig; i += nw) {
-    int cnt = 0;
-    if (lane < MAX_LIG / 32) adj[i][lane] = 0u;
-    for (int j0 = 0; j0 < n_lig; j0 += 64) {
-      const int j = j0 + lane;
-      const bool in = j < n_lig && dist2(lp + 3 * i, lp + 3 * j) < r2;
-      const unsigned long long m = __ballot(in);
-      const bool keep = in && cnt + __popcll(m & ((1ull << lane) - 1ull)) < LIG_CAP && j != i;
-      const unsigned long long kept = __ballot(keep);
-      if (lane == 0) { adj[i][j0 >> 5] = (unsigned)kept; adj[i][(j0 >> 5) + 1] = (unsigned)(kept >> 32); }
-      cnt += __popcll(m);
-    }
-  }
-}
-
-__device__ void block_exclusive_scan(int* a, int n, int* tmp) {
-  const int tid = threadIdx.x, lane = tid & 63, wave = tid >> 6;
-  const int nt = blockDim.x;
-  const int per = (n + nt - 1) / nt;
-  const int beg = min(tid * per, n), end = min(beg + per, n);
-  int s = 0;
-  for (int k = beg; k < end; ++k) s += a[k];
-  int v = s;
-#pragma unroll
-  for (int d = 1; d < 64; d *= 2) {
-    const int t = __shfl_up(v, d, 64);
-    if (lane >= d) v += t;
-  }
-  if (lane == 63) tmp[wave] = v;
-  __syncthreads();
-  int base = v - s;
-  for (int w = 0; w < wave; ++w) base += tmp[w];
-  for (int k = beg; k < end; ++k) { const int t = a[k]; a[k] = base; base += t; }
-  __syncthreads();
-}
-
-__device__ void propagate_levels(uint8_t* lvl, const GraphArgs& G) {
-  constexpr int UC = 8;
-  if (G.E_rr <= GT * UC) {
-    unsigned e[UC];
-#pragma unroll
-    for (int u = 0; u < UC; ++u) {
-      const int k = threadIdx.x + GT * u;
-      e[u] = k < G.E_rr ? (unsigned)G.rr_src[k] | ((unsigned)G.rr_dst[k] << 16) : 0xffffffffu;
-    }
-    for (int pass = 0; pass < 2; ++pass) {
-#pragma unroll
-      for (int u = 0; u < UC; ++u) {
-        const int r = (int)(e[u] & 0xffffu), d = (int)(e[u] >> 16);
-        if (e[u] != 0xffffffffu && lvl[r] == pass && lvl[d] == 3) lvl[d] = (uint8_t)(pass + 1);
-      }
-      __syncthreads();
-    }
-    return;
-  }
-  constexpr int U = 8;
-  for (int pass = 0; pass < 2; ++pass) {
-    for (int k0 = threadIdx.x; k0 < G.E_rr; k0 += GT * U) {
-      int r[U], d[U];
-#pragma unroll
-      for (int u = 0; u < U; ++u) {
-        const int k = k0 + GT * u;
-        r[u] = k < G.E_rr ? G.rr_src[k] : -1;
-        d[u] = k < G.E_rr ? G.rr_dst[k] : 0;
-      }
-#pragma unroll
-      for (int u = 0; u < U; ++u)
-        if (r[u] >= 0 && lvl[r[u]] == pass && lvl[d[u]] == 3) lvl[d[u]] = (uint8_t)(pass + 1);
-    }
-    __syncthreads();
-  }
-}
-
-__device__ void level_scan(const uint8_t* lvl, const int32_t* outdeg, int n, int* pre, int (*tmp)[4], int* tot) {
-  const int tid = threadIdx.x, lane = tid & 63, wave = tid >> 6;
-  const int nt = blockDim.x, nw = nt >> 6;
-  const int per = (n + nt - 1) / nt;
-  const int beg = min(tid * per, n), end = min(beg + per, n);
-  int s0 = 0, s1 = 0, s2 = 0, s3 = 0;
-  for (int k = beg; k < end; ++k) {
-    const int l = lvl[k], od = outdeg[k];
-    s0 += l == 0 ? od : 0; s1 += l == 1 ? od : 0; s2 += l == 2 ? od : 0; s3 += l == 3 ? od : 0;
-  }
-  int v0 = s0, v1 = s1, v2 = s2, v3 = s3;
-#pragma unroll
-  for (int d = 1; d < 64; d *= 2) {
-    const int t0 = __shfl_up(v0, d, 64), t1 = __shfl_up(v1, d, 64), t2 = __shfl_up(v2, d, 64), t3 = __shfl_up(v3, d, 64);
-    if (lane >= d) { v0 += t0; v1 += t1; v2 += t2; v3 += t3; }
-  }
-  if (lane == 63) { tmp[wave][0] = v0; tmp[wave][1] = v1; tmp[wave][2] = v2; tmp[wave][3] = v3; }
-  __syncthreads();
-  if (pre != nullptr) {
-    int b0 = v0 - s0, b1 = v1 - s1, b2 = v2 - s2, b3 = v3 - s3;
-    for (int w = 0; w < wave; ++w) { b0 += tmp[w][0]; b1 += tmp[w][1]; b2 += tmp[w][2]; b3 += tmp[w][3]; }
-    for (int k = beg; k < end; ++k) {
-      const int l = lvl[k], od = outdeg[k];
-      pre[k] = l == 0 ? b0 : (l == 1 ? b1 : (l == 2 ? b2 : b3));
-      b0 += l == 0 ? od : 0; b1 += l == 1 ? od : 0; b2 += l == 2 ? od : 0; b3 += l == 3 ? od : 0;
-    }
-  }
-  if (tid < 4) { int t_ = 0; for (int w = 0; w < nw; ++w) t_ += tmp[w][tid]; tot[tid] = t_; }
-  __syncthreads();
-}
-
 __global__ __launch_bounds__(GT) void graph_count_kernel(GraphArgs G) {
-  extern __shared__ float smem[];
-  float* lp = smem;
-  float* rp = lp + MAX_LIG * 3;
-  uint8_t* lvl = reinterpret_cast<uint8_t*>(rp + 3 * G.n_rec + G.n_rec);
-  __shared__ unsigned adj[MAX_LIG][MAX_LIG / 32];
-  __shared__ float4 lps[MAX_LIG];
-  __shared__ int s_cnt[2], lvl_tmp[GT / 64][4], lvl_tot[4];
-  const int b = blockIdx.x, tid = threadIdx.x;
-  for (int i = tid; i < G.n_lig * 3; i += GT) {
-    const float v = G.lig_pos[(size_t)b * G.n_lig * 3 + i];
-    lp[i] = v;
-    reinterpret_cast<float*>(lps)[4 * (i / 3) + i % 3] = v / G.cross_cutoff;
-  }
-  for (int i = tid; i < G.n_rec * 3; i += GT) rp[i] = G.rec_pos[i] / G.cross_cutoff;
-  if (tid < 2) s_cnt[tid] = 0;
-  __syncthreads();
-  build_lig_adj(lp, G.n_lig, G.lig_r2, adj);
-  __syncthreads();
-  int c_ll = 0, c_lr = 0;
-  for (int i = tid; i < G.n_lig; i += GT)
-    for (int w = 0; w < MAX_LIG / 32; ++w) c_ll += __popc(adj[i][w]);
-  for (int j = tid; j < G.n_rec; j += GT) {
-    const float rx = rp[3 * j], ry = rp[3 * j + 1], rz = rp[3 * j + 2];
-    int cnt = 0;
-#pragma unroll 4
-    for (int i = 0; i < G.n_lig; ++i) cnt += cross_within4(lps[i], rx, ry, rz) ? 1 : 0;
-    c_lr += cnt;
-    lvl[j] = (G.prune && cnt == 0) ? 3 : 0;
-  }
-#pragma unroll
-  for (int d = 32; d > 0; d >>= 1) { c_ll += __shfl_down(c_ll, d, 64); c_lr += __shfl_down(c_lr, d, 64); }
-  if ((tid & 63) == 0) { atomicAdd(&s_cnt[0], c_ll); atomicAdd(&s_cnt[1], c_lr); }
-  __syncthreads();
-  if (G.prune) propagate_levels(lvl, G);
-  level_scan(lvl, G.rr_outdeg, G.n_rec, nullptr, lvl_tmp, lvl_tot);
-  if (tid < 2) G.counts[CNT_STRIDE * b + tid] = s_cnt[tid];
-  if (tid < 3) G.counts[CNT_STRIDE * b + 2 + tid] = lvl_tot[tid];
-  for (int j = tid; j < G.n_rec; j += GT) G.levels[(size_t)b * G.n_rec + j] = lvl[j];
+  graph_count_body(G, (int)blockIdx.x, G.lig_pos + (size_t)blockIdx.x * G.n_lig * 3);
 }
 
 __device__ __forceinline__ void sample_prefix(const GraphArgs& G, int b, int* ex, int* tot) {
@@ -683,9 +521,6 @@
   return hipGetLastError();
 }
 
-static inline size_t graph_lds_bytes(int n_rec) {
-  return (size_t)(MAX_LIG * 3 + n_rec * 3) * 4 + (size_t)n_rec * 4 + (((size_t)n_rec + 15) & ~(size_t)15);
-}
 
 static size_t g_graph_dyn[64] = {};
 static inline size_t graph_lds_bytes_mirror(int n_rec, int n_lig) { return graph_lds_bytes(n_rec) + (size_t)n_rec * ((n_lig + 63) / 64) * 8; }
@@ -715,11 +550,11 @@
   return hipSuccess;
 }
 
-hipError_t launch_graph(const GraphArgs& G, int64_t edge_cap, hipStream_t s) {
+hipError_t launch_graph(const GraphArgs& G, int64_t edge_cap, hipStream_t s, bool counted) {
   const size_t lds = graph_lds_bytes(G.n_rec);
   GraphArgs Gc = G;
   Gc.edge_cap = edge_cap;
-  hipLaunchKernelGGL(graph_count_kernel, dim3(G.B), dim3(GT), lds, s, Gc);
+  if (!counted) hipLaunchKernelGGL(graph_count_kernel, dim3(G.B), dim3(GT), lds, s, Gc);
   hipLaunchKernelGGL(graph_fill_kernel, dim3(G.B, FILL_SLICES), dim3(GT), G.cross_mirror ? graph_lds_bytes_mirror(G.n_rec, G.n_lig) : lds, s, Gc);
   return hipGetLastError();
 }
diff --git a/disco_diffdock_amd/csrc/k_graph_count.h b/disco_diffdock_amd/csrc/k_graph_count.h
--- /dev/null
+++ b/disco_diffdock_amd/csrc/k_graph_count.h
@@ -0,0 +1,177 @@
+#pragma once
+#include "model.h"
+
+namespace ddk {
+
+__device__ __forceinline__ bool cross_within(const float* lp, const float* rp, float c) {
+#pragma clang fp contract(off)
+  const float dx = rp[0] / c - lp[0] / c, dy = rp[1] / c - lp[1] / c, dz = rp[2] / c - lp[2] / c;
+  return dx * dx + dy * dy + dz * dz < 1.0f;
+}
+
+__device__ __forceinline__ bool cross_within4(const float4 a, float rx, float ry, float rz) {
+#pragma clang fp contract(off)
+  const float dx = rx - a.x, dy = ry - a.y, dz = rz - a.z;
+  return dx * dx + dy * dy + dz * dz < 1.0f;
+}
+
+__device__ __forceinline__ float dist2(const float* a, const float* b) {
+#pragma clang fp contract(off)
+  const float dx = a[0] - b[0], dy = a[1] - b[1], dz = a[2] - b[2];
+  return dx * dx + dy * dy + dz * dz;
+}
+
+constexpr int GT = 1024;
+
+__device__ void build_lig_adj(const float* lp, int n_lig, float r2, unsigned (*adj)[MAX_LIG / 32]) {
+  const int lane = threadIdx.x & 63, wave = threadIdx.x >> 6, nw = blockDim.x >> 6;
+  for (int i = wave; i < n_lig; i += nw) {
+    int cnt = 0;
+    if (lane < MAX_LIG / 32) adj[i][lane] = 0u;
+    for (int j0 = 0; j0 < n_lig; j0 += 64) {
+      const int j = j0 + lane;
+      const bool in = j < n_lig && dist2(lp + 3 * i, lp + 3 * j) < r2;
+      const unsigned long long m = __ballot(in);
+      const bool keep = in && cnt + __popcll(m & ((1ull << lane) - 1ull)) < LIG_CAP && j != i;
+      const unsigned long long kept = __ballot(keep);
+      if (lane == 0) { adj[i][j0 >> 5] = (unsigned)kept; adj[i][(j0 >> 5) + 1] = (unsigned)(kept >> 32); }
+      cnt += __popcll(m);
+    }
+  }
+}
+
+__device__ void block_exclusive_scan(int* a, int n, int* tmp) {
+  const int tid = threadIdx.x, lane = tid & 63, wave = tid >> 6;
+  const int nt = blockDim.x;
+  const int per = (n + nt - 1) / nt;
+  const int beg = min(tid * per, n), end = min(beg + per, n);
+  int s = 0;
+  for (int k = beg; k < end; ++k) s += a[k];
+  int v = s;
+#pragma unroll
+  for (int d = 1; d < 64; d *= 2) {
+    const int t = __shfl_up(v, d, 64);
+    if (lane >= d) v += t;
+  }
+  if (lane == 63) tmp[wave] = v;
+  __syncthreads();
+  int base = v - s;
+  for (int w = 0; w < wave; ++w) base += tmp[w];
+  for (int k = beg; k < end; ++k) { const int t = a[k]; a[k] = base; base += t; }
+  __syncthreads();
+}
+
+__device__ void propagate_levels(uint8_t* lvl, const GraphArgs& G) {
+  constexpr int UC = 8;
+  if (G.E_rr <= GT * UC) {
+    unsigned e[UC];
+#pragma unroll
+    for (int u = 0; u < UC; ++u) {
+      const int k = threadIdx.x + GT * u;
+      e[u] = k < G.E_rr ? (unsigned)G.rr_src[k] | ((unsigned)G.rr_dst[k] << 16) : 0xffffffffu;
+    }
+    for (int pass = 0; pass < 2; ++pass) {
+#pragma unroll
+      for (int u = 0; u < UC; ++u) {
+        const int r = (int)(e[u] & 0xffffu), d = (int)(e[u] >> 16);
+        if (e[u] != 0xffffffffu && lvl[r] == pass && lvl[d] == 3) lvl[d] = (uint8_t)(pass + 1);
+      }
+      __syncthreads();
+    }
+    return;
+  }
+  constexpr int U = 8;
+  for (int pass = 0; pass < 2; ++pass) {
+    for (int k0 = threadIdx.x; k0 < G.E_rr; k0 += GT * U) {
+      int r[U], d[U];
+#pragma unroll
+      for (int u = 0; u < U; ++u) {
+        const int k = k0 + GT * u;
+        r[u] = k < G.E_rr ? G.rr_src[k] : -1;
+        d[u] = k < G.E_rr ? G.rr_dst[k] : 0;
+      }
+#pragma unroll
+      for (int u = 0; u < U; ++u)
+        if (r[u] >= 0 && lvl[r[u]] == pass && lvl[d[u]] == 3) lvl[d[u]] = (uint8_t)(pass + 1);
+    }
+    __syncthreads();
+  }
+}
+
+__device__ void level_scan(const uint8_t* lvl, const int32_t* outdeg, int n, int* pre, int (*tmp)[4], int* tot) {
+  const int tid = threadIdx.x, lane = tid & 63, wave = tid >> 6;
+  const int nt = blockDim.x, nw = nt >> 6;
+  const int per = (n + nt - 1) / nt;
+  const int beg = min(tid * per, n), end = min(beg + per, n);
+  int s0 = 0, s1 = 0, s2 = 0, s3 = 0;
+  for (int k = beg; k < end; ++k) {
+    const int l = lvl[k], od = outdeg[k];
+    s0 += l == 0 ? od : 0; s1 += l == 1 ? od : 0; s2 += l == 2 ? od : 0; s3 += l == 3 ? od : 0;
+  }
+  int v0 = s0, v1 = s1, v2 = s2, v3 = s3;
+#pragma unroll
+  for (int d = 1; d < 64; d *= 2) {
+    const int t0 = __shfl_up(v0, d, 64), t1 = __shfl_up(v1, d, 64), t2 = __shfl_up(v2, d, 64), t3 = __shfl_up(v3, d, 64);
+    if (lane >= d) { v0 += t0; v1 += t1; v2 += t2; v3 += t3; }
+  }
+  if (lane == 63) { tmp[wave][0] = v0; tmp[wave][1] = v1; tmp[wave][2] = v2; tmp[wave][3] = v3; }
+  __syncthreads();
+  if (pre != nullptr) {
+    int b0 = v0 - s0, b1 = v1 - s1, b2 = v2 - s2, b3 = v3 - s3;
+    for (int w = 0; w < wave; ++w) { b0 += tmp[w][0]; b1 += tmp[w][1]; b2 += tmp[w][2]; b3 += tmp[w][3]; }
+    for (int k = beg; k < end; ++k) {
+      const int l = lvl[k], od = outdeg[k];
+      pre[k] = l == 0 ? b0 : (l == 1 ? b1 : (l == 2 ? b2 : b3));
+      b0 += l == 0 ? od : 0; b1 += l == 1 ? od : 0; b2 += l == 2 ? od : 0; b3 += l == 3 ? od : 0;
+    }
+  }
+  if (tid < 4) { int t_ = 0; for (int w = 0; w < nw; ++w) t_ += tmp[w][tid]; tot[tid] = t_; }
+  __syncthreads();
+}
+
+__device__ __forceinline__ void graph_count_body(const GraphArgs& G, const int b, const float* pose) {
+  extern __shared__ float smem[];
+  float* lp = smem;
+  float* rp = lp + MAX_LIG * 3;
+  uint8_t* lvl = reinterpret_cast<uint8_t*>(rp + 3 * G.n_rec + G.n_rec);
+  __shared__ unsigned adj[MAX_LIG][MAX_LIG / 32];
+  __shared__ float4 lps[MAX_LIG];
+  __shared__ int s_cnt[2], lvl_tmp[GT / 64][4], lvl_tot[4];
+  const int tid = threadIdx.x;
+  for (int i = tid; i < G.n_lig * 3; i += GT) {
+    const float v = pose[i];
+    lp[i] = v;
+    reinterpret_cast<float*>(lps)[4 * (i / 3) + i % 3] = v / G.cross_cutoff;
+  }
+  for (int i = tid; i < G.n_rec * 3; i += GT) rp[i] = G.rec_pos[i] / G.cross_cutoff;
+  if (tid < 2) s_cnt[tid] = 0;
+  __syncthreads();
+  build_lig_adj(lp, G.n_lig, G.lig_r2, adj);
+  __syncthreads();
+  int c_ll = 0, c_lr = 0;
+  for (int i = tid; i < G.n_lig; i += GT)
+    for (int w = 0; w < MAX_LIG / 32; ++w) c_ll += __popc(adj[i][w]);
+  for (int j = tid; j < G.n_rec; j += GT) {
+    const float rx = rp[3 * j], ry = rp[3 * j + 1], rz = rp[3 * j + 2];
+    int cnt = 0;
+#pragma unroll 4
+    for (int i = 0; i < G.n_lig; ++i) cnt += cross_within4(lps[i], rx, ry, rz) ? 1 : 0;
+    c_lr += cnt;
+    lvl[j] = (G.prune && cnt == 0) ? 3 : 0;
+  }
+#pragma unroll
+  for (int d = 32; d > 0; d >>= 1) { c_ll += __shfl_down(c_ll, d, 64); c_lr += __shfl_down(c_lr, d, 64); }
+  if ((tid & 63) == 0) { atomicAdd(&s_cnt[0], c_ll); atomicAdd(&s_cnt[1], c_lr); }
+  __syncthreads();
+  if (G.prune) propagate_levels(lvl, G);
+  level_scan(lvl, G.rr_outdeg, G.n_rec, nullptr, lvl_tmp, lvl_tot);
+  if (tid < 2) G.counts[CNT_STRIDE * b + tid] = s_cnt[tid];
+  if (tid < 3) G.counts[CNT_STRIDE * b + 2 + tid] = lvl_tot[tid];
+  for (int j = tid; j < G.n_rec; j += GT) G.levels[(size_t)b * G.n_rec + j] = lvl[j];
+}
+
+static inline size_t graph_lds_bytes(int n_rec) {
+  return (size_t)(MAX_LIG * 3 + n_rec * 3) * 4 + (size_t)n_rec * 4 + (((size_t)n_rec + 15) & ~(size_t)15);
+}
+
+}
diff --git a/disco_diffdock_amd/csrc/k_heads.hip b/disco_diffdock_amd/csrc/k_heads.hip
--- a/disco_diffdock_amd/csrc/k_heads.hip
+++ b/disco_diffdock_amd/csrc/k_heads.hip
@@ -34,7 +34,7 @@
   __syncthreads();
 }
 
-__global__ __launch_bounds__(256) void heads_pre_kernel(HeadArgs A, int n_tor_blocks) {
+__global__ __launch_bounds__(256) void heads_geom_kernel(HeadArgs A, int n_tor_blocks) {
   __shared__ float lp[MAX_LIG * 3];
   __shared__ float act[EPB][DE + 1];
   __shared__ int nb[BOND_CAP];
@@ -64,11 +64,9 @@
       if (live) {
         const int e = b * n + i;
         float* at = A.h_attr + (size_t)e * NE;
-        const float* xr = A.x + ((size_t)b * n + i) * XW;
 #pragma unroll
         for (int q = 0; q < 3; ++q) {
           at[3 * p + q] = e3[q];
-          at[NS + 3 * p + q] = xr[3 * p + q];
           at[2 * NS + 3 * p + q] = 0.0f;
         }
         if (p == 0) {
@@ -107,6 +105,7 @@
         s_base = atomicAdd(A.h_info + 3, s_cnt);
       }
       A.h_deg[blockIdx.x] = s_cnt;
+      A.h_base[blockIdx.x] = s_base;
     }
   }
   __syncthreads();
@@ -131,16 +130,8 @@
     }
     return;
   }
-  const float* xk = A.x + ((size_t)b * n + k) * XW;
-  const float* xu = A.x + ((size_t)b * n + u) * XW;
-  const float* xv = A.x + ((size_t)b * n + v) * XW;
-#pragma unroll
-  for (int q = 0; q < 3; ++q) {
-    const int o = 3 * p + q;
-    at[o] = e3[q];
-    at[NS + o] = xk[o];
-    at[2 * NS + o] = xu[o] + xv[o];
-  }
+#pragma unroll
+  for (int q = 0; q < 3; ++q) at[3 * p + q] = e3[q];
   if (p != 0) return;
   const float inv = 1.7320508075688772f / fmaxf(d, 1e-12f);
   const float s1[3] = {vx * inv, vy * inv, vz * inv};
@@ -159,6 +150,91 @@
   A.h_dst[e] = b * n + k;
 }
 
+constexpr int RT = 1024;
+constexpr int ROW_BONDS = 32;
+template <bool FIN>
+__global__ __launch_bounds__(RT) void heads_rows_kernel(HeadArgs A, RowsFinArgs F, int n_tor_blocks) {
+  __shared__ float xs[MAX_LIG][NS];
+  __shared__ short kk[ROW_BONDS * BOND_CAP];
+  __shared__ int ebase[ROW_BONDS];
+  __shared__ int2 ruv[ROW_BONDS];
+  const int tid = threadIdx.x, b = blockIdx.x, n = A.n_lig;
+  const int R = n_tor_blocks > 0 ? A.R : 0;
+  auto stage = [&](int r0) {
+    for (int i = tid; i < ROW_BONDS * BOND_CAP; i += RT) {
+      const int rr = i / BOND_CAP, el = i - rr * BOND_CAP, r = r0 + rr;
+      short k = -1;
+      if (r < R) {
+        const int bond = b * R + r, base = A.h_base[bond];
+        if (el < A.h_deg[bond]) k = (short)(A.h_dst[base + el] - b * n);
+        if (el == 0) { ebase[rr] = base; ruv[rr] = make_int2(A.rot_u[r], A.rot_v[r]); }
+      }
+      kk[i] = k;
+    }
+  };
+  if (R > 0) stage(0);
+  if constexpr (FIN) {
+    if (F.zero_extra != nullptr)
+      for (int64_t i = (int64_t)b * RT + tid; i < F.n_extra; i += (int64_t)gridDim.x * RT) F.zero_extra[i] = 0.0f;
+    constexpr int U = 4;
+    const int tot = n * XW;
+    for (int i0 = tid; i0 < tot; i0 += RT * U) {
+      float sv[U], xi[U];
+      int dg[U];
+#pragma unroll
+      for (int u = 0; u < U; ++u) {
+        const int i = i0 + RT * u;
+        sv[u] = 0.0f; xi[u] = 0.0f; dg[u] = 1;
+        if (i < tot) {
+          const int rl = i / XW, c = i - rl * XW;
+          const int64_t r = (int64_t)b * n + rl;
+          if (c < F.dout) {
+            dg[u] = F.deg[r];
+            for (int sl = 0; sl < F.n_slots; ++sl) sv[u] += F.sum[(r * F.n_slots + sl) * XW + c];
+          }
+          xi[u] = F.x_in[r * XW + c];
+        }
+      }
+#pragma unroll
+      for (int u = 0; u < U; ++u) {
+        const int i = i0 + RT * u;
+        if (i >= tot) continue;
+        const int rl = i / XW, c = i - rl * XW;
+        const int64_t r = (int64_t)b * n + rl;
+        float v = 0.0f;
+        if (c < F.dout) {
+          for (int sl = 0; sl < F.n_slots; ++sl) F.sum[(r * F.n_slots + sl) * XW + c] = 0.0f;
+          v = sv[u] / (float)(dg[u] > 1 ? dg[u] : 1);
+          v = (v - F.bn_mean[c]) * F.bn_scale[c] + F.bn_bias[c];
+        }
+        v += xi[u];
+        F.x_out[r * XW + c] = v;
+        if (c < NS) xs[rl][c] = v;
+      }
+    }
+  } else {
+    for (int i = tid; i < n * NS; i += RT) { const int rl = i / NS, c = i - rl * NS; xs[rl][c] = A.x[((size_t)b * n + rl) * XW + c]; }
+  }
+  __syncthreads();
+  for (int i = tid; i < n * NS; i += RT) {
+    const int rl = i / NS, c = i - rl * NS;
+    A.h_attr[((size_t)b * n + rl) * NE + NS + c] = xs[rl][c];
+  }
+  for (int r0 = 0; r0 < R; r0 += ROW_BONDS) {
+    if (r0 > 0) { __syncthreads(); stage(r0); __syncthreads(); }
+    const int nb = min(ROW_BONDS, R - r0);
+    for (int i = tid; i < nb * BOND_CAP * NS; i += RT) {
+      const int sl = i / NS, c = i - sl * NS, rr = sl / BOND_CAP;
+      const int k = kk[sl];
+      if (k < 0) continue;
+      const int u = ruv[rr].x, v = ruv[rr].y;
+      float* at = A.h_attr + (size_t)(ebase[rr] + (sl - rr * BOND_CAP)) * NE;
+      at[NS + c] = xs[k][c];
+      at[2 * NS + c] = xs[u][c] + xs[v][c];
+    }
+  }
+}
+
 __global__ __launch_bounds__(64) void heads_post_kernel(HeadArgs A, int n_tor_blocks) {
   __shared__ float v48[2 * NS], hid[NS], g12[12];
   const int tid = threadIdx.x;
@@ -209,9 +285,16 @@
   }
 }
 
-hipError_t launch_heads_pre(const HeadArgs& A, bool torsion, hipStream_t s) {
+hipError_t launch_heads_geom(const HeadArgs& A, bool torsion, hipStream_t s) {
   const int n_tor = (torsion && A.R > 0) ? A.B * A.R : 0;
-  hipLaunchKernelGGL(heads_pre_kernel, dim3(n_tor + A.B), dim3(256), 0, s, A, n_tor);
+  hipLaunchKernelGGL(heads_geom_kernel, dim3(n_tor + A.B), dim3(256), 0, s, A, n_tor);
+  return hipGetLastError();
+}
+
+hipError_t launch_heads_rows(const HeadArgs& A, bool torsion, hipStream_t s, const RowsFinArgs* fin) {
+  const int n_tor = (torsion && A.R > 0) ? A.B * A.R : 0;
+  if (fin) hipLaunchKernelGGL(heads_rows_kernel<true>, dim3(A.B), dim3(RT), 0, s, A, *fin, n_tor);
+  else hipLaunchKernelGGL(heads_rows_kernel<false>, dim3(A.B), dim3(RT), 0, s, A, RowsFinArgs{}, n_tor);
   return hipGetLastError();
 }
 
diff --git a/disco_diffdock_amd/csrc/k_se3.hip b/disco_diffdock_amd/csrc/k_se3.hip
--- a/disco_diffdock_amd/csrc/k_se3.hip
+++ b/disco_diffdock_amd/csrc/k_se3.hip
@@ -1,4 +1,5 @@
 #include "model.h"
+#include "k_graph_count.h"
 
 namespace ddk {
 
@@ -116,21 +117,21 @@
   return hipGetLastError();
 }
 
-template <bool POST, bool REC>
-__global__ __launch_bounds__(256) void se3_update_kernel(Se3Args A, HeadArgs H) {
+template <bool POST, bool REC, int NT>
+__device__ __forceinline__ const float* se3_update_body(const Se3Args& A, const HeadArgs& H, const int b) {
   __shared__ float rig[MAX_LIG * 3], flx_a[MAX_LIG * 3], flx2[MAX_LIG * 3];
   __shared__ float upd[6], ctr[3], Rm[9], cA[3], cB[3], Rk[9], tk[3], rot_th[64];
   __shared__ int2 rot_uv[64];
   __shared__ double S[9];
   float* flx = flx_a;
-  const int b = blockIdx.x, tid = threadIdx.x, n = A.n_lig, R = A.R;
+  const int tid = threadIdx.x, n = A.n_lig, R = A.R;
   if constexpr (POST) {
     __shared__ float v48[64][2 * NS], hid[64][NS], g12[12];
     if (H.prof_out != nullptr && b == (int)gridDim.x - 1 && tid < PROF_INTS) H.prof_out[tid] = H.exec_info[tid];
     if (A.tor != nullptr && R > 0) {
       for (int r0 = 0; r0 < R; r0 += 64) {
         const int chunk = min(64, R - r0);
-        for (int i = tid; i < chunk * 2 * NS; i += 256) {
+        for (int i = tid; i < chunk * 2 * NS; i += NT) {
           const int rr = i / (2 * NS), c = i - rr * 2 * NS;
           const int bond = b * R + r0 + rr;
           float* row = H.h_sum + (size_t)(H.B + bond) * XW;
@@ -140,7 +141,7 @@
           v48[rr][c] = (sv - H.md.tb_bn_mean[c]) * H.md.tb_bn_scale[c] + H.md.tb_bn_bias[c];
         }
         __syncthreads();
-        for (int i = tid; i < chunk * NS; i += 256) {
+        for (int i = tid; i < chunk * NS; i += NT) {
           const int rr = i / NS, k = i - rr * NS;
           float a = 0.0f;
           for (int j = 0; j < 2 * NS; ++j) a += H.md.tf_w0[k * 2 * NS + j] * v48[rr][j];
@@ -179,7 +180,7 @@
     __syncthreads();
   }
   const float* nz = A.noise ? A.noise + (size_t)b * (6 + R) : nullptr;
-  for (int i = tid; i < n * 3; i += 256) rig[i] = A.pos[(size_t)b * n * 3 + i];
+  for (int i = tid; i < n * 3; i += NT) rig[i] = A.pos[(size_t)b * n * 3 + i];
   if (tid < 6) {
     const int k = tid / 3;
     const float sc = (tid < 3 ? A.tr : A.rot)[3 * b + tid % 3];
@@ -211,16 +212,16 @@
   }
   __syncthreads();
   if (A.tor == nullptr || R == 0) {
-    for (int i = tid; i < n * 3; i += 256) {
+    for (int i = tid; i < n * 3; i += NT) {
       A.pos_out[(size_t)b * n * 3 + i] = rig[i];
       if constexpr (REC) if (A.rec_pos != nullptr) A.rec_pos[(size_t)b * n * 3 + i] = rig[i];
     }
     if constexpr (REC)
-      for (int r = tid; r < R; r += 256) {
+      for (int r = tid; r < R; r += NT) {
         if (A.rec_scores != nullptr) A.rec_scores[(size_t)b * (6 + R) + 6 + r] = 0.0f;
         if (A.rec_perturb != nullptr) A.rec_perturb[(size_t)b * (6 + R) + 6 + r] = 0.0f;
       }
-    return;
+    return rig;
   }
   float* cur = flx;
   float* nxt = flx2;
@@ -271,12 +272,26 @@
     const float oy = Rk[3] * x + Rk[4] * y + Rk[5] * z + tk[1];
     const float oz = Rk[6] * x + Rk[7] * y + Rk[8] * z + tk[2];
     o[0] = ox; o[1] = oy; o[2] = oz;
+    rig[3 * tid] = ox; rig[3 * tid + 1] = oy; rig[3 * tid + 2] = oz;
     if constexpr (REC)
       if (A.rec_pos != nullptr) {
         float* q = A.rec_pos + ((size_t)b * n + tid) * 3;
         q[0] = ox; q[1] = oy; q[2] = oz;
       }
   }
+  return rig;
+}
+
+template <bool POST, bool REC>
+__global__ __launch_bounds__(256) void se3_update_kernel(Se3Args A, HeadArgs H) {
+  se3_update_body<POST, REC, 256>(A, H, (int)blockIdx.x);
+}
+
+template <bool REC>
+__global__ __launch_bounds__(GT) void se3_update_count_kernel(Se3Args A, HeadArgs H, GraphArgs G) {
+  const float* pose = se3_update_body<true, REC, GT>(A, H, (int)blockIdx.x);
+  __syncthreads();
+  graph_count_body(G, (int)blockIdx.x, pose);
 }
 
 __global__ __launch_bounds__(256) void randomize_kernel(RandPosArgs A) {
@@ -427,4 +442,36 @@
   return hipGetLastError();
 }
 
-}
+static size_t g_se3_count_dyn[64] = {};
+
+hipError_t se3_prepare_device() {
+  hipFuncAttributes a1, a2;
+  hipError_t e = hipFuncGetAttributes(&a1, reinterpret_cast<const void*>(&se3_update_count_kernel<false>));
+  if (e == hipSuccess) e = hipFuncGetAttributes(&a2, reinterpret_cast<const void*>(&se3_update_count_kernel<true>));
+  if (e != hipSuccess) return e;
+  const size_t st = a1.sharedSizeBytes > a2.sharedSizeBytes ? a1.sharedSizeBytes : a2.sharedSizeBytes;
+  if (st >= 160 * 1024) return hipSuccess;
+  const int dyn = (int)(160 * 1024 - st);
+  e = hipFuncSetAttribute(reinterpret_cast<const void*>(&se3_update_count_kernel<false>), hipFuncAttributeMaxDynamicSharedMemorySize, dyn);
+  if (e == hipSuccess) e = hipFuncSetAttribute(reinterpret_cast<const void*>(&se3_update_count_kernel<true>), hipFuncAttributeMaxDynamicSharedMemorySize, dyn);
+  if (e != hipSuccess) return e;
+  int dev = 0;
+  if (hipGetDevice(&dev) == hipSuccess && dev >= 0 && dev < 64) g_se3_count_dyn[dev] = (size_t)dyn;
+  return hipSuccess;
+}
+
+int se3_count_fits(int n_rec) {
+  int dev = 0;
+  if (hipGetDevice(&dev) != hipSuccess || dev < 0 || dev >= 64) return 0;
+  return g_se3_count_dyn[dev] > 0 && graph_lds_bytes(n_rec) <= g_se3_count_dyn[dev];
+}
+
+hipError_t launch_se3_count(const Se3Args& A, const HeadArgs& post, const GraphArgs& G, hipStream_t s) {
+  const bool rec = A.rec_pos != nullptr || A.rec_scores != nullptr || A.rec_perturb != nullptr || A.rec_edges != nullptr;
+  const size_t lds = graph_lds_bytes(G.n_rec);
+  if (rec) hipLaunchKernelGGL((se3_update_count_kernel<true>), dim3(A.B), dim3(GT), lds, s, A, post, G);
+  else hipLaunchKernelGGL((se3_update_count_kernel<false>), dim3(A.B), dim3(GT), lds, s, A, post, G);
+  return hipGetLastError();
+}
+
+}
diff --git a/disco_diffdock_amd/csrc/model.h b/disco_diffdock_amd/csrc/model.h
--- a/disco_diffdock_amd/csrc/model.h
+++ b/disco_diffdock_amd/csrc/model.h
@@ -215,10 +215,16 @@
   float* rot_out;
   float* tor_out;
   int32_t *h_src, *h_dst, *h_deg, *h_info;
+  int32_t* h_base;
   float *h_attr, *h_sh, *h_sum;
   int32_t* prof_out = nullptr;
   const int32_t* exec_info = nullptr;
   int deterministic;
+};
+
+struct RowsFinArgs {
+  float* sum; const int32_t* deg; const float* x_in; const float *bn_mean, *bn_scale, *bn_bias;
+  int dout, n_slots; float* x_out; float* zero_extra; int64_t n_extra;
 };
 
 struct Se3Args {
@@ -262,7 +268,7 @@
 void conf_model_destroy(ddk_ctx* ctx);
 struct ConfComplex;
 
-hipError_t launch_graph(const GraphArgs& G, int64_t edge_cap, hipStream_t s);
+hipError_t launch_graph(const GraphArgs& G, int64_t edge_cap, hipStream_t s, bool counted = false);
 GraphArgs graph_args(const ddk_ctx* ctx, const ddk_complex* cx, int B, const float* lig_pos, float cross_cutoff);
 int graph_cross_mirror_fits(int n_lig, int n_rec);
 hipError_t launch_edge_features(const EdgeFeatArgs& A, int64_t edge_cap, hipStream_t s);
@@ -276,9 +282,13 @@
 hipError_t launch_complex_static(const RecStaticArgs& R, const int32_t* rr_src, const int32_t* rr_dst, const float* rec_pos, int E, const EdgeMlpDev& m,
                                  float* pre1, hipStream_t s);
 hipError_t launch_zero_fill(void* p, size_t bytes, hipStream_t s);
-hipError_t launch_heads_pre(const HeadArgs& A, bool torsion, hipStream_t s);
+hipError_t launch_heads_geom(const HeadArgs& A, bool torsion, hipStream_t s);
+hipError_t launch_heads_rows(const HeadArgs& A, bool torsion, hipStream_t s, const RowsFinArgs* fin = nullptr);
 hipError_t launch_heads_post(const HeadArgs& A, bool torsion, hipStream_t s);
 hipError_t launch_se3(const Se3Args& A, hipStream_t s, const HeadArgs* post = nullptr);
+hipError_t launch_se3_count(const Se3Args& A, const HeadArgs& post, const GraphArgs& G, hipStream_t s);
+int se3_count_fits(int n_rec);
+hipError_t se3_prepare_device();
 hipError_t launch_cfg_combine(float* score, const float* uncond, float weight, int64_t n, hipStream_t s);
 
 }
@@ -308,7 +318,7 @@
   float* part = nullptr;
   int32_t* det_rng = nullptr;
   float* sum_rr0 = nullptr;
-  int32_t *h_src = nullptr, *h_dst = nullptr, *h_deg = nullptr;
+  int32_t *h_src = nullptr, *h_dst = nullptr, *h_deg = nullptr, *h_base = nullptr;
   float *h_attr = nullptr, *h_sh = nullptr, *h_sum = nullptr;
   float* pre = nullptr;
   float* x_last = nullptr;
diff --git a/disco_diffdock_amd/csrc/model.hip b/disco_diffdock_amd/csrc/model.hip
--- a/disco_diffdock_amd/csrc/model.hip
+++ b/disco_diffdock_amd/csrc/model.hip
@@ -427,15 +427,17 @@
 }
 
 static hipError_t build_graph(ddk_ctx* ctx, ddk_complex* cx, int B, const float* lig_pos, float cross_cutoff, bool prune, bool shared_rr,
-                              hipStream_t s, int64_t patch_off = -1, int cross_mirror = 0) {
+                              hipStream_t s, int64_t patch_off = -1, int cross_mirror = 0, bool counted = false) {
   GraphArgs G = graph_args(ctx, cx, B, lig_pos, cross_cutoff);
   G.cross_mirror = cross_mirror; G.prune = prune ? 1 : 0; G.shared_rr = shared_rr ? 1 : 0; G.patch_off = patch_off;
   G.e_src = cx->e_src; G.e_dst = cx->e_dst; G.e_aux = cx->e_aux; G.deg = cx->deg;
-  return launch_graph(G, cx->edge_cap, s);
-}
+  return launch_graph(G, cx->edge_cap, s, counted);
+}
+
+static bool forward_prunes(const ddk_ctx* ctx, const ddk_complex* cx) { return ctx->prune && !cx->keep_rec && cx->E_rr > 0; }
 
 static int score_forward_impl(ddk_ctx* ctx, ddk_complex* cx, int B, const float* lig_pos, const StepParams& sp,
-                              float* tr_out, float* rot_out, float* tor_out, hipStream_t s, HeadArgs* defer_post = nullptr) {
+                              float* tr_out, float* rot_out, float* tor_out, hipStream_t s, HeadArgs* defer_post = nullptr, bool graph_counted = false) {
   const ddk_config& c = ctx->cfg;
   Model* M = (Model*)ctx->model;
   const int n_lig = cx->n_lig, n_rec = cx->n_rec;
@@ -453,9 +455,24 @@
     CK(launch_disco_patch(P, s), "layer-0 patch group");
     cx->latent_dirty = false; cx->patch_B = B;
   }
-  const bool prune = ctx->prune && !cx->keep_rec && cx->E_rr > 0;
+  const bool prune = forward_prunes(ctx, cx);
   const int mirror = graph_cross_mirror_fits(n_lig, n_rec);
-  CK(build_graph(ctx, cx, B, lig_pos, sp.cross_cutoff, prune, dedup, s, (dedup && patched) ? cx->patch_off : -1, mirror), "graph build");
+  CK(build_graph(ctx, cx, B, lig_pos, sp.cross_cutoff, prune, dedup, s, (dedup && patched) ? cx->patch_off : -1, mirror, graph_counted), "graph build");
+  const bool heads = !M->confidence_mode;
+  const bool torsion = !c.no_torsion && tor_out != nullptr && cx->R > 0;
+  HeadArgs Hd;
+  Hd.lig_pos = lig_pos; Hd.x = nullptr; Hd.md = M->dev; Hd.sp = sp; Hd.B = B; Hd.n_lig = n_lig; Hd.R = cx->R;
+  Hd.scale_by_sigma = c.scale_by_sigma; Hd.rot_u = cx->rot_u; Hd.rot_v = cx->rot_v; Hd.lig_r2 = c.lig_max_radius * c.lig_max_radius;
+  Hd.tr_out = tr_out; Hd.rot_out = rot_out; Hd.tor_out = tor_out;
+  Hd.h_src = cx->h_src; Hd.h_dst = cx->h_dst; Hd.h_deg = cx->h_deg; Hd.h_base = cx->h_base; Hd.h_info = cx->info + I_HEAD; Hd.h_attr = cx->h_attr; Hd.h_sh = cx->h_sh;
+  Hd.h_sum = cx->h_sum; Hd.deterministic = c.deterministic;
+  bool rows_done = false;
+  if (heads) {
+    CK(hipEventRecord(ctx->ev_fork, s), "head geometry fork");
+    CK(hipStreamWaitEvent(ctx->head_stream, ctx->ev_fork, 0), "head geometry fork");
+    CK(launch_heads_geom(Hd, torsion, ctx->head_stream), "heads_geom");
+    CK(hipEventRecord(ctx->ev_join, ctx->head_stream), "head geometry join");
+  }
   EdgeFeatArgs F;
   F.cross_mirror = mirror;
   F.lig_pos = lig_pos; F.rec_pos = cx->rec_pos; F.bond_attr = cx->bond_attr; F.rr_pre1 = cx->rr_pre1; F.rr_sh = cx->rr_sh;
@@ -549,6 +566,15 @@
       PA.lig_roles = next_lig_only ? 0x7 : 0xF; PA.rec_roles = next_lig_only ? 0x4 : 0xF;
       PA.levels = prune ? cx->levels : nullptr; PA.max_level = l == NL - 2 ? 0 : (l == NL - 3 ? 1 : (l == NL - 4 ? 2 : 3));
       CK(launch_node_finalize_pre(PA, true, s), "node_finalize_pre");
+    } else if (heads && lig_only && split) {
+      RowsFinArgs RF;
+      RF.sum = cx->sum; RF.deg = cx->deg; RF.x_in = xin; RF.bn_mean = L.bn_mean; RF.bn_scale = L.bn_scale; RF.bn_bias = L.bn_bias;
+      RF.dout = L.dout; RF.n_slots = c.deterministic ? 2 : 1; RF.x_out = xout;
+      RF.zero_extra = clear_rr0 ? cx->sum_rr0 : nullptr; RF.n_extra = clear_rr0 ? (int64_t)n_rec * XW : 0;
+      CK(hipStreamWaitEvent(s, ctx->ev_join, 0), "head geometry join");
+      Hd.x = xout;
+      CK(launch_heads_rows(Hd, torsion, s, &RF), "node_finalize + heads_rows");
+      rows_done = true;
     } else
     CK(launch_node_finalize(cx->sum, cx->deg, xin, L.bn_mean, L.bn_scale, L.bn_bias, lig_only ? (int64_t)B * n_lig : N, L.dout, XW, xout, s,
                             shared0 ? cx->sum_rr0 : nullptr, (int64_t)B * n_lig, n_rec, 1, clear_rr0 ? cx->sum_rr0 : nullptr,
@@ -560,19 +586,16 @@
   cx->last_B = B;
   cx->last_full = cx->keep_rec;
   cx->sum_clean = !rr0_dirty;
-  if (M->confidence_mode) return DDK_OK;
-  const bool torsion = !c.no_torsion && tor_out != nullptr && cx->R > 0;
-  HeadArgs Hd;
-  Hd.lig_pos = lig_pos; Hd.x = xin; Hd.md = M->dev; Hd.sp = sp; Hd.B = B; Hd.n_lig = n_lig; Hd.R = cx->R;
-  Hd.scale_by_sigma = c.scale_by_sigma; Hd.rot_u = cx->rot_u; Hd.rot_v = cx->rot_v; Hd.lig_r2 = c.lig_max_radius * c.lig_max_radius;
-  Hd.tr_out = tr_out; Hd.rot_out = rot_out; Hd.tor_out = tor_out;
-  Hd.h_src = cx->h_src; Hd.h_dst = cx->h_dst; Hd.h_deg = cx->h_deg; Hd.h_info = cx->info + I_HEAD; Hd.h_attr = cx->h_attr; Hd.h_sh = cx->h_sh;
-  Hd.h_sum = cx->h_sum; Hd.deterministic = c.deterministic;
+  if (!heads) return DDK_OK;
   if (prof_slot) {
     Hd.prof_out = prof_slot; Hd.exec_info = cx->info + I_EXEC;
     ctx->prof_slots += 1;
   }
-  CK(launch_heads_pre(Hd, torsion, s), "heads_pre");
+  if (!rows_done) {
+    CK(hipStreamWaitEvent(s, ctx->ev_join, 0), "head geometry join");
+    Hd.x = xin;
+    CK(launch_heads_rows(Hd, torsion, s), "heads_rows");
+  }
   int32_t* head_rng = nullptr;
   if (c.deterministic) {
     head_rng = cx->det_rng + (4 * (7 * (size_t)cx->max_batch + 1) + 8);
@@ -757,6 +780,7 @@
     cx->h_attr = cx_upload<float>(cx, nullptr, Eh * NE);
     cx->h_sh = cx_upload<float>(cx, nullptr, Eh * 4);
     cx->h_deg = cx_upload<int32_t>(cx, nullptr, Nh);
+    cx->h_base = cx_upload<int32_t>(cx, nullptr, Nh);
     cx->h_sum = cx_upload<float>(cx, nullptr, Nh * XW);
     if (cx->h_sum) launch_zero_fill(cx->h_sum, (size_t)Nh * XW * sizeof(float), ctx->up_stream);
   }
@@ -952,10 +976,13 @@
   for (int k = 0; k < steps; ++k)
     if ((rc = make_step_params(ctx, t[3 * k], t[3 * k + 1], t[3 * k + 2], sps[k]))) return rc;
   const size_t n_sc = (size_t)B * (6 + (torsion ? R : 0));
+  const bool fuse_count = se3_count_fits(cx->n_rec) != 0;
+  bool counted = false;
   for (int k = 0; k < steps; ++k) {
     const bool guided = cx->cfg_weight != 0.0f && ctx->cfg.latent_dim > 0 && t[3 * k] <= cx->cfg_start && t[3 * k] >= cx->cfg_end;
     HeadArgs post;
-    if ((rc = score_forward_impl(ctx, cx, B, pos, sps[k], tr, rot, torsion ? tor : nullptr, s, guided ? nullptr : &post))) return rc;
+    if ((rc = score_forward_impl(ctx, cx, B, pos, sps[k], tr, rot, torsion ? tor : nullptr, s, guided ? nullptr : &post, counted))) return rc;
+    counted = false;
     if (guided) {
       const float* ll = cx->lig_latent; const float* rl = cx->rec_latent; const float un = cx->unconditional;
       cx->lig_latent = cx->zero_lat; cx->rec_latent = cx->zero_lat + (size_t)B * cx->n_lig * ctx->cfg.latent_dim; cx->unconditional = 1.0f;
@@ -978,7 +1005,15 @@
     if (rec.scores) A.rec_scores = rec.scores + (size_t)k * sc_row;
     if (rec.perturb) A.rec_perturb = rec.perturb + (size_t)k * sc_row;
     if (rec.edge_counts) { A.rec_edges = rec.edge_counts + 4 * (size_t)k; A.info = cx->info; }
-    hipError_t e = launch_se3(A, s, guided ? nullptr : &post);
+    hipError_t e;
+    if (fuse_count && !guided && k + 1 < steps) {
+      GraphArgs G = graph_args(ctx, cx, B, pos, sps[k + 1].cross_cutoff);
+      G.prune = forward_prunes(ctx, cx) ? 1 : 0;
+      e = launch_se3_count(A, post, G, s);
+      counted = true;
+    } else {
+      e = launch_se3(A, s, guided ? nullptr : &post);
+    }
     if (e != hipSuccess) return hip_fail(ctx, e, "se3_update launch");
   }
   return DDK_OK;
```

Result: no change. 48.74 (median of 6 runs) (+0.7%).
